# injun-baek/Video-Depth-Normal-v2

Hardware: AMD Instinct MI355X
Metric: depth frames/sec at 518x518, ViT-L (higher is better)
Workload: dtype f16x3; 1 GPU; DepthAnythingV2(vitl) batch=8 518x518 streams/GPU, memory bank full (S=6); replicas per GPU; lanes=2, precision=f16x3, ranks=1, backend=none, attention_pv_products=1

## Files before the change

### include/vdn.h

```cpp
#ifndef VDN_H
#define VDN_H
#include <stddef.h>
#include <stdint.h>

#ifdef __cplusplus
extern "C" {
#endif

typedef void* vdn_stream;

enum vdn_status { VDN_OK = 0, VDN_EINVAL = -1, VDN_EUNSUPPORTED = -2, VDN_EALIGN = -3 };
enum vdn_dtype { VDN_F16 = 0, VDN_BF16 = 1, VDN_F32 = 2, VDN_NONE = 3 };
enum vdn_act { VDN_ACT_NONE = 0, VDN_ACT_GELU = 1, VDN_ACT_RELU = 2,
               VDN_ACT_SILU = 3  };
enum vdn_amode { VDN_A_PLAIN = 0, VDN_A_CONV3X3 = 1,
                 VDN_A_PAD3X3 = 2  };
enum vdn_store {
  VDN_ST_PLAIN = 0,
  VDN_ST_HEADS = 1,
  VDN_ST_CONVT = 2,
  VDN_ST_GEGLU = 3
};

typedef struct vdn_gemm_tuning {
  int force_bm;
  int p8;
  int no_splitk;
  int no_pipe;
  int splitk_p8;
  int cus;
  int splitk_occ;
  int splitk_max;
  int min_tiles;
  float f128, f192;
  int x8;
} vdn_gemm_tuning;
int vdn_gemm_get_tuning(vdn_gemm_tuning* out);

typedef struct vdn_gemm_desc {
  int32_t dt;
  int32_t M, N, K;
  const void* A;
  int32_t a_mode;
  int32_t lda;
  int32_t relu_a;
  int32_t cB, cH, cW, cC, cOH, cOW, cstride;
  const void* W;
  int32_t ldb;
  const float* bias;
  const float* rowadd;
  int32_t act;
  const float* gamma;
  const float* tab;
  int32_t tab_mod, tab_off;
  const void* res1;
  int32_t res1_dt, ldr1;
  const void* res2;
  int32_t res2_dt, ldr2;
  int32_t store;
  void* out;
  int32_t out_dt;
  int32_t ldc;
  int32_t row_group, row_skip;
  void* dst[3];
  int32_t nsplit, heads, tokens, tok_off, tpad;
  int32_t transposed[3];
  int32_t rope[3];
  const float* rope_cs;
  int32_t rope_mod;
  int32_t ck, cout;
  const void* zeros;
  const void* A_lo;
  const void* W_lo;
  void* out_lo;
  void* dst_lo[3];
  const void* res1_lo;
  const void* res2_lo;
  int32_t conv_korder;
  int32_t cu_hint;
  void* splitk_ws;
  int64_t splitk_ws_bytes;
  int32_t ksplit;
  void* dst8[3];
  const void* A8;
  const void* W8;
  void* out8;
  int32_t a_kt, w_kt, out_kt;
  int32_t x8_terms;
  const vdn_gemm_tuning* tuning;
  int32_t subpix;
  const float* subpix_bias;
  void* pad_hi;
} vdn_gemm_desc;

int vdn_gemm(const vdn_gemm_desc* d, vdn_stream stream);

int vdn_layernorm(const void* x, int x_dt, int rows, int C, const float* w, const float* b, float eps,
                  const float* addvec, float alpha, const float* addtab, int tab_div, int tab_mod,
                  int out_group, void* out_h, void* out_h_lo, int h_dt, float* out_f, void* out8, int kt,
                  vdn_stream stream);

int vdn_flash_attn(int dt, const void* Q, const void* K, const void* Vt, void* out, const void* Q_lo,
                   const void* K_lo, const void* Vt_lo, void* out_lo, const void* Q8, const void* K8, void* out8, int out_kt,
                   int B, int H, int nq, int nq_pad, int nk, int nk_pad, float scale, int pv_products, vdn_stream stream);

int vdn_temporal_attn(int dt, const void* qkv, void* out, const void* qkv_lo, void* out_lo, int Bv, int T, int D,
                      int c, int heads, float scale, const float* rope_cs, vdn_stream stream);

int vdn_groupnorm(int dt, const void* x, const void* x_lo, void* y, void* y_lo, int F, int HW, int C, int groups,
                  const float* w, const float* b, float eps, float* partial, int nsplit, vdn_stream stream);

int vdn_upsample_bilinear(int dt, const void* x, const void* x_lo, void* y, void* y_lo, int B, int IH, int IW, int OH,
                          int OW, int C, vdn_stream stream);
int vdn_upsample_bilinear_f32(const float* x, float* y, int B, int IH, int IW, int OH, int OW, int relu,
                              vdn_stream stream);

int vdn_patchify(int dt, const float* img, void* rows, void* rows_lo, int B, int H, int W, int ldk,
                 vdn_stream stream);

int vdn_fill_row(float* x, const float* vec, int B, int rows_per_b, int row, int C, vdn_stream stream);

int vdn_bicubic(const float* src, float* dst, int ih, int iw, int oh, int ow, int C, float scale_rows,
                float scale_cols, vdn_stream stream);

int vdn_preprocess(const uint8_t* frames, int n, int h, int w, int swap_rb, float* out, int H, int W, const float* mean3,
                   const float* std3, vdn_stream stream);

int vdn_add_vec(const float* x, const float* vec, float alpha, float* y, int rows, int C, vdn_stream stream);

int vdn_head_out(int dt, const void* feat, const void* feat_lo, const float* w, float bias, float* depth, int M,
                 int C, int relu, vdn_stream stream);

enum { VDN_OUT_NONE = 0, VDN_OUT_RELU = 1, VDN_OUT_SIGMOID = 2 };

int vdn_head_out_act(int dt, const void* feat, const void* feat_lo, const float* w, float bias, float* depth, int M,
                     int C, int act, float out_scale, vdn_stream stream);

int vdn_mask_down1(const float* depth, float* out, int B, int H, int W, int OH, int OW, const float* w,
                   vdn_stream stream);
int vdn_mask_down2(const float* in, float* out, int B, int H, int W, int OH, int OW, const float* w,
                   vdn_stream stream);

int vdn_dwconv7(const float* x, float* y, int B, int H, int W, int C, const float* w, const float* bias,
                vdn_stream stream);

int vdn_addtab_cast(int dt, const float* x, const float* tab, int tab_div, int tab_mod, void* y, void* y_lo,
                    size_t rows, int C, vdn_stream stream);

int vdn_temporal_attn_last(int dt, const float* pool, size_t slot_stride, const int32_t* slots, int T, int HW, int c,
                           const float* pe_q, const float* pe_k, const float* pe_v, float scale, void* out, void* out_lo,
                           vdn_stream stream);

size_t vdn_stitch_workspace_bytes(void);
int vdn_stitch_fit(const float* pred, const float* target, size_t n, void* workspace, float* coef, vdn_stream stream);
int vdn_stitch_apply(const float* window, const float* coef, float* out_tail, float* out_new, float* ref1, size_t hw,
                     int T, int align_len, int overlap, int ref_frame, vdn_stream stream);

enum vdn_eval_domain { VDN_EVAL_DEPTH = 0, VDN_EVAL_DISP = 1 };
enum vdn_eval_tgm { VDN_EVAL_TGM_ROWS = 0, VDN_EVAL_TGM_FRAMES = 1 };
size_t vdn_eval_workspace_bytes(int frames);
int vdn_eval_fit(const float* pred, const float* gt, const uint8_t* mask, int frames, size_t hw, double dmin, double dmax,
                 int domain, void* workspace, double* coef, vdn_stream stream);
int vdn_eval_metrics(const float* pred, const float* gt, const uint8_t* mask, int frames, int H, int W, double dmin,
                     double dmax, int domain, int tgm, const double* coef, void* workspace, double* out,
                     vdn_stream stream);
int vdn_resize_bilinear_hp(const float* x, float* y, int frames, int IH, int IW, int OH, int OW, vdn_stream stream);

size_t vdn_normal_eval_workspace_bytes(int frames);
int vdn_sobel_ix_iy(const float* depth, float* ix, float* iy, int frames, int H, int W, int normalize_kernel,
                    vdn_stream stream);
int vdn_normal_vector(const float* depth, float* out, int frames, int H, int W, int normalize_kernel, float scale_xy,
                      float scale_z, float eps, vdn_stream stream);
int vdn_erode_mask3(const uint8_t* mask, uint8_t* out, int frames, int H, int W, vdn_stream stream);
int vdn_normal_eval(const float* pred, const float* target, int target_is_depth, const uint8_t* mask, int frames, int H,
                    int W, void* workspace, double* frame_sums, int64_t* frame_counts, double* out, vdn_stream stream);
// ... 128 lines not shown
```

### video-depth-normal-v2_amd/csrc/gemm.hip

```cpp
#include "common.hpp"
#include <stdlib.h>

namespace vdn_gemm_impl {
int launch_f16(const vdn_gemm_desc& d, hipStream_t s);
int launch_bf16(const vdn_gemm_desc& d, hipStream_t s);

static int env_int(const char* name, int dflt) {
  const char* e = getenv(name);
  return e ? atoi(e) : dflt;
}
static float env_float(const char* name, float dflt) {
  const char* e = getenv(name);
  return e ? (float)atof(e) : dflt;
}
static const vdn_gemm_tuning& tuning_defaults() {
  static const vdn_gemm_tuning t = [] {
    vdn_gemm_tuning v;
    v.force_bm = env_int("VDN_GEMM_BM", 0);
    v.p8 = env_int("VDN_GEMM_P8", 1);
    v.no_splitk = getenv("VDN_GEMM_NOSPLITK") != nullptr;
    v.no_pipe = getenv("VDN_GEMM_NOPIPE") != nullptr;
    v.splitk_p8 = env_int("VDN_SPLITK_P8", 0);
    v.cus = env_int("VDN_GEMM_CUS", 0);
    v.splitk_occ = env_int("VDN_SPLITK_OCC", 50);
    v.splitk_max = env_int("VDN_SPLITK_MAX", 8);
    v.min_tiles = env_int("VDN_GEMM_MIN_TILES", 96);
    v.f128 = env_float("VDN_GEMM_F128", 1.3f);
    v.f192 = env_float("VDN_GEMM_F192", 1.2f);
    v.x8 = env_int("VDN_GEMM_X8", 1);
    return v;
  }();
  return t;
}
const vdn_gemm_tuning& tuning(const vdn_gemm_desc& d) { return d.tuning ? *d.tuning : tuning_defaults(); }
}

extern "C" int vdn_gemm_get_tuning(vdn_gemm_tuning* out) {
  if (!out) return VDN_EINVAL;
  vdn_gemm_desc none = {};
  *out = vdn_gemm_impl::tuning(none);
  return VDN_OK;
}

extern "C" int vdn_gemm(const vdn_gemm_desc* dp, vdn_stream stream) {
  if (!dp) return VDN_EINVAL;
  const vdn_gemm_desc& d = *dp;
  if (d.M <= 0 || d.N <= 0 || d.K <= 0 || !d.A || !d.W || !d.zeros) return VDN_EINVAL;
  if (d.tuning) {
    const vdn_gemm_tuning& t = *d.tuning;
    if ((t.force_bm != 0 && t.force_bm != 128 && t.force_bm != 192 && t.force_bm != 256) || t.splitk_occ < 0 || t.splitk_max < 0 ||
        t.min_tiles < 0 || t.cus < 0 || t.cus > 256)
      return VDN_EINVAL;
  }
  if (d.dt != VDN_F16 && d.dt != VDN_BF16) return VDN_EUNSUPPORTED;
  if ((d.K & 7) || (d.ldb & 63) || d.ldb < d.K) return VDN_EALIGN;
  if (((uintptr_t)d.A & 15) || ((uintptr_t)d.W & 15) || ((uintptr_t)d.zeros & 15)) return VDN_EALIGN;
  if (d.subpix) {
    if (d.subpix != 1 || d.a_mode != VDN_A_CONV3X3 || d.store != VDN_ST_CONVT || !d.subpix_bias || d.bias || d.act || d.rowadd ||
        d.gamma || d.tab || d.res1 || d.res2 || d.relu_a || d.K != 4 * d.cC || d.ldb != d.K || d.conv_korder != 1 || d.cstride != 1)
      return VDN_EINVAL;
    if ((d.ck != 2 && d.ck != 4) || d.cout <= 0 || (d.cout & 255) || (d.cC & 63) || !d.A_lo || !d.W_lo || !d.out_lo ||
        d.out_dt != d.dt || d.A8 || d.W8)
      return VDN_EUNSUPPORTED;
    if (((uintptr_t)d.subpix_bias | (uintptr_t)d.out) & 15) return VDN_EALIGN;
  }
  if (d.a_mode == VDN_A_CONV3X3) {
    if ((d.cC & 7) || d.K != (d.subpix ? 4 : 9) * d.cC || d.M != d.cB * d.cOH * d.cOW) return VDN_EINVAL;
    if (d.conv_korder && ((d.cC & 63) || d.conv_korder != 1)) return VDN_EINVAL;
    if (d.cstride != 1 && d.cstride != 2) return VDN_EUNSUPPORTED;
    if (d.cOH != (d.cH + 2 - 3) / d.cstride + 1 || d.cOW != (d.cW + 2 - 3) / d.cstride + 1) return VDN_EINVAL;
  } else if (d.a_mode == VDN_A_PLAIN) {
    if ((d.lda & 7) || d.lda < d.K) return VDN_EALIGN;
  } else if (d.a_mode == VDN_A_PAD3X3) {
    if (d.dt != VDN_F16 || !d.A8 || !d.W8 || !d.a_kt || !d.w_kt || d.relu_a || d.subpix || d.x8_terms) return VDN_EINVAL;
    if (d.cB <= 0 || d.cH <= 0 || d.cW <= 0 || d.cC <= 0 || (d.cC & 63) || d.cC > 4096 || d.K != 9 * d.cC || d.ldb != d.K) return VDN_EINVAL;
    if ((long)d.cB * (d.cH + 2) * (d.cW + 2) != d.M) return VDN_EINVAL;
    if (d.store != VDN_ST_PLAIN || !d.bias || d.rowadd || d.gamma || d.tab || d.row_group > 0 || d.out_dt != VDN_F16 || d.ldc != d.N ||
        (d.N & 63) || !d.out || ((uintptr_t)d.out & 15) || ((uintptr_t)d.bias & 15))
      return VDN_EINVAL;
    if (d.act == VDN_ACT_RELU) {
      if (!d.out_kt || !d.out8 || d.out_lo || d.res1 || d.res2 || d.pad_hi) return VDN_EINVAL;
    } else if (d.act == VDN_ACT_NONE) {
      if (d.out_kt || !d.out_lo || !d.res1 || !d.res1_lo || d.res1_dt != VDN_F16 || (d.ldr1 & 7) || ((uintptr_t)d.res1 | (uintptr_t)d.res1_lo) & 15)
        return VDN_EINVAL;
      if (d.res2 && (!d.res2_lo || d.res2_dt != VDN_F16 || (d.ldr2 & 7) || ((uintptr_t)d.res2 | (uintptr_t)d.res2_lo) & 15)) return VDN_EINVAL;
      if ((d.pad_hi == nullptr) != (d.out8 == nullptr) || ((uintptr_t)d.pad_hi & 15)) return VDN_EINVAL;
    } else {
      return VDN_EINVAL;
    }
  } else {
    return VDN_EUNSUPPORTED;
  }
  if (d.N & 3) return VDN_EALIGN;
  if (d.ksplit != 0 || d.splitk_ws_bytes < 0 || (d.splitk_ws == nullptr) != (d.splitk_ws_bytes == 0)) return VDN_EINVAL;
  if ((uintptr_t)d.splitk_ws & 15) return VDN_EALIGN;
  if (((uintptr_t)d.A_lo | (uintptr_t)d.W_lo | (uintptr_t)d.out_lo) & 15) return VDN_EALIGN;
  if (d.out_lo && (d.out_dt == VDN_F32 || !d.out)) return VDN_EINVAL;
  if ((d.res1 && (d.ldr1 & 3)) || (d.res2 && (d.ldr2 & 3))) return VDN_EALIGN;
  if (((uintptr_t)d.A8 | (uintptr_t)d.W8 | (uintptr_t)d.out8) & 15) return VDN_EALIGN;
  if ((d.A8 || d.W8) && (d.dt != VDN_F16 || (d.a_mode != VDN_A_PLAIN && d.a_mode != VDN_A_PAD3X3) || (d.K & 63) || (d.lda != d.K && !d.a_kt))) return VDN_EINVAL;
  if (d.out8 && (d.dt != VDN_F16 || d.store != VDN_ST_PLAIN || d.out_dt != VDN_F16 || (d.act != VDN_ACT_GELU && d.a_mode != VDN_A_PAD3X3) || d.N != d.ldc || (d.N & 63) || !d.A8 || !d.W8))
    return VDN_EINVAL;
  if ((d.a_kt || d.w_kt || d.out_kt || d.x8_terms) && (!d.A8 || !d.W8)) return VDN_EINVAL;
  if (d.A8 && d.W8 && ((!d.a_kt && (long)d.M * d.lda >= (1L << 31)) || (!d.w_kt && (long)d.N * d.ldb >= (1L << 31)) || d.M >= (1 << 25) || d.N >= (1 << 25)))
    return VDN_EUNSUPPORTED;
  if (d.x8_terms < 0 || d.x8_terms > 2) return VDN_EINVAL;
  if (d.out_kt && (d.store != VDN_ST_PLAIN || d.out_dt != VDN_F16 || d.ldc != d.N || (d.N & 63) || d.res1 || d.res2 || d.tab ||
                   d.rowadd || d.gamma || d.row_group > 0 || (d.act == VDN_ACT_RELU && d.a_mode != VDN_A_PAD3X3))) return VDN_EINVAL;
  if (d.pad_hi && d.a_mode != VDN_A_PAD3X3) return VDN_EINVAL;
  if (((uintptr_t)d.bias | (uintptr_t)d.gamma | (uintptr_t)d.tab | (uintptr_t)d.res1 | (uintptr_t)d.res2) & 7) return VDN_EALIGN;
  switch (d.store) {
    case VDN_ST_PLAIN:
      if (!d.out || d.ldc < d.N) return VDN_EINVAL;
      if ((d.ldc & 3) || ((uintptr_t)d.out & 15)) return VDN_EALIGN;
      break;
    case VDN_ST_GEGLU:
      if (!d.out || (d.N & 31) || d.ldc < d.N / 2 || (d.act && d.act != VDN_ACT_SILU) || d.gamma || d.res1 || d.res2 || d.tab || d.rowadd)
        return VDN_EINVAL;
      if ((d.ldc & 3) || ((uintptr_t)d.out & 15)) return VDN_EALIGN;
      break;
    case VDN_ST_CONVT:
      if (!d.out || d.ck <= 0 || d.cout <= 0 || d.N != d.ck * d.ck * d.cout || d.M != d.cB * d.cH * d.cW || d.res1 ||
          d.res2 || d.tab)
        return VDN_EINVAL;
      if ((d.cout & 3) || ((uintptr_t)d.out & 15)) return VDN_EALIGN;
      break;
    case VDN_ST_HEADS:
      if (d.nsplit < 1 || d.nsplit > 3 || d.heads <= 0 || d.N != d.nsplit * d.heads * 64 || d.tokens <= 0 ||
          d.M % d.tokens || d.tok_off < 0 || d.tok_off + d.tokens > d.tpad || d.act || d.gamma || d.res1 || d.res2 ||
          d.tab || d.rowadd)
        return VDN_EINVAL;
      for (int i = 0; i < d.nsplit; ++i) {
        if (!d.dst[i] || ((uintptr_t)d.dst[i] & 15)) return VDN_EINVAL;
        if (d.rope[i] && (!d.rope_cs || d.rope_mod <= 0)) return VDN_EINVAL;
        if (d.dst8[i] && (d.transposed[i] || (!d.W_lo && !d.W8) || d.dt != VDN_F16 || ((uintptr_t)d.dst8[i] & 15))) return VDN_EINVAL;
      }
      break;
    default:
      return VDN_EUNSUPPORTED;
  }
  hipStream_t s = (hipStream_t)stream;
  return d.dt == VDN_F16 ? vdn_gemm_impl::launch_f16(d, s) : vdn_gemm_impl::launch_bf16(d, s);
}
```

### video-depth-normal-v2_amd/csrc/gemm_kernels.hpp

```cpp
#pragma once
#include "planes.hpp"
#include <stdlib.h>
#include <type_traits>

namespace vdn_gemm_impl {

const vdn_gemm_tuning& tuning(const vdn_gemm_desc& d);

constexpr int BK = 64;


__device__ __forceinline__ void glds16(const void* src, void* dst) {
  __builtin_amdgcn_global_load_lds((const __attribute__((address_space(1))) void*)src, (__attribute__((address_space(3))) void*)dst,
                                   16, 0, 0);
}

__device__ __forceinline__ void tile_mn(int tile, int tiles_m, int tiles_n, int& tm_i, int& tn_i) {
  constexpr int GM = 4;
  const int per_group = GM * tiles_n;
  const int g = tile / per_group, r = tile - g * per_group;
  const int gm = (tiles_m - g * GM) < GM ? (tiles_m - g * GM) : GM;
  tn_i = r / gm;
  tm_i = g * GM + (r - tn_i * gm);
}
// ... 2 lines not shown
__device__ __forceinline__ int frag_off128(int row, int c) { return row * 128 + ((c ^ ((row >> 1) & 7)) << 4); }

template <typename H>
__device__ __forceinline__ f32x4 mma3(typename H::V8 bh, typename H::V8 bl, typename H::V8 ah, typename H::V8 al, f32x4 c) {
  c = H::mfma16(bh, al, c);
  c = H::mfma16(bl, ah, c);
  return H::mfma16(bh, ah, c);
}

struct KStep {
  int k0;
  int tap;
  int off;
};
template <int BKS, bool SUBPIX = false>
__device__ __forceinline__ KStep kstep_decode(int kt, const vdn_gemm_desc& p, unsigned sp_taps = 0, int sp_lg = 0) {
  static_assert(BKS == 32 || BKS == 64, "one or two steps per 64-channel block");
  KStep s = {kt * BKS, 9, 0};
  if (p.conv_korder) {
    const int t2 = BKS == 32 ? kt >> 1 : kt, half = BKS == 32 ? kt & 1 : 0;
    int c64;
    if constexpr (SUBPIX) {
      c64 = t2 >> sp_lg;
      s.tap = (sp_taps >> (4 * (t2 & ((1 << sp_lg) - 1)))) & 15;
    } else {
      c64 = t2 / 9;
      s.tap = t2 - c64 * 9;
    }
    if (c64 * 64 >= p.cC) s.tap = 9;
    const int ky = (s.tap * 11) >> 5, kx = s.tap - ky * 3;
    s.off = ((ky - 1) * p.cW + (kx - 1)) * p.cC + c64 * 64 + half * 32;
  }
  return s;
}

template <typename T, bool CONV>
struct APiece {
  const T* base;
  int iy0, ix0;
  const T* center;
  unsigned ok9;
  __device__ __forceinline__ void setup(int m, int chunk_elems, const vdn_gemm_desc& p) {
    m = m < p.M ? m : p.M - 1;
    if constexpr (CONV) {
      const int hw = p.cOH * p.cOW;
      const int b = m / hw, rem = m - b * hw;
      const int oy = rem / p.cOW, ox = rem - oy * p.cOW;
      base = (const T*)p.A + (size_t)b * p.cH * p.cW * p.cC;
      iy0 = oy * p.cstride - 1;
      ix0 = ox * p.cstride - 1;
      center = base + ((ptrdiff_t)(iy0 + 1) * p.cW + (ix0 + 1)) * p.cC + chunk_elems;
      ok9 = 0;
#pragma unroll
      for (int t = 0; t < 9; ++t) {
        const int iy = iy0 + t / 3, ix = ix0 + t % 3;
        ok9 |= (unsigned)((iy >= 0) & (iy < p.cH) & (ix >= 0) & (ix < p.cW)) << t;
      }
    } else {
      base = (const T*)p.A + (size_t)m * p.lda;
    }
  }
  __device__ __forceinline__ const char* src(const KStep& ks, int chunk_elems, const vdn_gemm_desc& p, bool& ok) const {
    const int k = ks.k0 + chunk_elems;
    if constexpr (!CONV) {
      ok = k < p.K;
      return (const char*)(base + k);
    } else if (p.conv_korder) {
      ok = (ok9 >> ks.tap) & 1;
      return (const char*)(center + ks.off);
    } else {
      const int tap = (int)(((float)(k >> 3) + 0.5f) * (1.0f / (float)(p.cC >> 3)));
      const int ci = k - tap * p.cC;
      const int ky = tap / 3, kx = tap - ky * 3;
      const int iy = iy0 + ky, ix = ix0 + kx;
      ok = (tap < 9) & (iy >= 0) & (iy < p.cH) & (ix >= 0) & (ix < p.cW);
      return (const char*)(base + ((size_t)iy * p.cW + ix) * p.cC + ci);
    }
  }
};


constexpr int VDN_STX_FC1 = 100, VDN_STX_RES = 101, VDN_STX_HEADS = 102, VDN_STX_HALF = 103, VDN_STX_RESHALF1 = 104,
              VDN_STX_RESHALF2 = 105, VDN_STX_SPLITK = 106, VDN_STX_SUBPIX = 107,
              VDN_STX_RCU1 = 108, VDN_STX_RCU2 = 109;

__device__ __forceinline__ void subpix_taps(int phase, int ck, unsigned& taps, int& lg) {
  const int a = phase / ck, b = phase - a * ck;
  const int y0 = a == 0 ? 0 : 1, ny = (a == 0 || a == ck - 1) ? 2 : 1;
  const int x0 = b == 0 ? 0 : 1, nx = (b == 0 || b == ck - 1) ? 2 : 1;
  taps = 0;
  int s = 0;
  for (int yy = 0; yy < ny; ++yy)
    for (int xx = 0; xx < nx; ++xx) taps |= (unsigned)(3 * (y0 + yy) + x0 + xx) << (4 * s++);
  lg = (ny >> 1) + (nx >> 1);
}
__device__ __forceinline__ int subpix_tile(int tn_i, const vdn_gemm_desc& p, unsigned& taps, int& lg) {
  const int tpp = p.cout >> 8;
  const int rank = tn_i / tpp, sub = tn_i - rank * tpp;
  const int phase = p.ck == 4 ? (int)((0xa965edb87421fc30ULL >> (4 * rank)) & 15) : rank;
  subpix_taps(phase, p.ck, taps, lg);
  return phase * p.cout + sub * 256;
}

__host__ __device__ inline int epi_flavour(const vdn_gemm_desc& d) {
  if (d.subpix) return VDN_STX_SUBPIX;
  const bool half_out = d.out_dt != VDN_F32;
  const bool plain_rows = d.store == VDN_ST_PLAIN && !d.rowadd && !d.gamma && !d.tab && d.row_group <= 0;
  if (plain_rows && half_out && d.out_lo && d.act != VDN_ACT_GELU) {
    if (!d.res1 && !d.res2) return VDN_STX_HALF;
    if (d.act == VDN_ACT_NONE && d.res1 && d.res1_lo && d.res1_dt == d.out_dt) {
      if (!d.res2) return VDN_STX_RESHALF1;
      if (d.res2_lo && d.res2_dt == d.out_dt) return VDN_STX_RESHALF2;
    }
  }
  if (d.store == VDN_ST_PLAIN && d.bias && d.act == VDN_ACT_GELU && !d.rowadd && !d.gamma && !d.tab && !d.res1 && !d.res2 &&
      half_out && (d.out_lo || (d.out8 && d.A8 && d.W8)) && d.row_group <= 0)
    return VDN_STX_FC1;
  if (d.store == VDN_ST_PLAIN && d.act == VDN_ACT_NONE && !d.rowadd && !d.tab && d.res1 && d.res1_dt == VDN_F32 && !d.res1_lo &&
      !d.res2 && d.out_dt == VDN_F32 && d.row_group <= 0)
    return VDN_STX_RES;
  if (d.store == VDN_ST_HEADS && !d.rope[0] && !d.rope[1] && !d.rope[2] && d.nsplit >= 1) {
    for (int i = 0; i < d.nsplit; ++i)
      if (!d.dst[i] || (!d.dst_lo[i] && !d.transposed[i] && !d.dst8[i])) return d.store;
    return VDN_STX_HEADS;
  }
  return d.store;
}

template <int DT, int STORE>
__device__ __forceinline__ void emit4(const vdn_gemm_desc& p, int m, int n, f32x4 a, f32x4 b, f32x4 bias_a, f32x4 bias_b,
                                      f32x4 gam) {
  static_assert(STORE == VDN_ST_PLAIN || STORE == VDN_ST_CONVT || STORE == VDN_ST_GEGLU || STORE == VDN_ST_HEADS ||
                STORE == VDN_STX_SPLITK || STORE == VDN_STX_HALF || STORE == VDN_STX_RESHALF1 || STORE == VDN_STX_RESHALF2 ||
                STORE == VDN_STX_RES, "emit4 serves these flavours");
  using H = Half<DT>;
  using T = typename H::T;
  using V4 = typename H::V4;
  if (m >= p.M || n >= p.N) return;
  if constexpr (STORE == VDN_STX_SPLITK) {
    *(f32x4*)((float*)p.out + (size_t)m * p.ldc + n) = a;
    return;
  } else if constexpr (STORE == VDN_STX_HALF || STORE == VDN_STX_RESHALF1 || STORE == VDN_STX_RESHALF2) {
    a += bias_a;
    if constexpr (STORE == VDN_STX_HALF) {
      const float floor_v = p.act == VDN_ACT_RELU ? 0.f : -INFINITY;
#pragma unroll
      for (int e = 0; e < 4; ++e) a[e] = (a[e] < floor_v) ? floor_v : a[e];
    } else {
      const size_t r1 = (size_t)m * p.ldr1 + n;
      const V4 rh = *(const V4*)((const T*)p.res1 + r1), rl = *(const V4*)((const T*)p.res1_lo + r1);
#pragma unroll
      for (int e = 0; e < 4; ++e) a[e] += (float)rh[e] + (float)rl[e];
      if constexpr (STORE == VDN_STX_RESHALF2) {
        const size_t r2 = (size_t)m * p.ldr2 + n;
        const V4 qh = *(const V4*)((const T*)p.res2 + r2), ql = *(const V4*)((const T*)p.res2_lo + r2);
#pragma unroll
        for (int e = 0; e < 4; ++e) a[e] += (float)qh[e] + (float)ql[e];
      }
    }
    V4 h, l;
    split_planes(a, h, l);
    store_out_planes<false, T>(p, (size_t)m * p.ldc + n, h, l);
    return;
  } else if constexpr (STORE == VDN_STX_RES) {
    a = (a + bias_a) * gam + *(const f32x4*)((const float*)p.res1 + (size_t)m * p.ldr1 + n);
    *(f32x4*)((float*)p.out + (size_t)m * p.ldc + n) = a;
    return;
  }
  if constexpr (STORE == VDN_ST_PLAIN || STORE == VDN_ST_CONVT) {
    a += bias_a;
    if (p.rowadd) a += p.rowadd[m];
    if (p.act == VDN_ACT_GELU) {
      a = gelu4(a);
    } else if (p.act == VDN_ACT_RELU) {
#pragma unroll
      for (int e = 0; e < 4; ++e) a[e] = (a[e] < 0.f) ? 0.f : a[e];
    }
    a *= gam;
    if (p.tab) a += *(const f32x4*)(p.tab + (size_t)(m % p.tab_mod + p.tab_off) * p.N + n);
    if (p.res1) {
      a += load4_as_float(p.res1, p.res1_dt, (size_t)m * p.ldr1 + n);
      if (p.res1_lo) a += load4_as_float(p.res1_lo, p.res1_dt, (size_t)m * p.ldr1 + n);
    }
    if (p.res2) {
      a += load4_as_float(p.res2, p.res2_dt, (size_t)m * p.ldr2 + n);
      if (p.res2_lo) a += load4_as_float(p.res2_lo, p.res2_dt, (size_t)m * p.ldr2 + n);
    }
    size_t o;
    if constexpr (STORE == VDN_ST_CONVT) {
      const int hw = p.cH * p.cW;
      const int cb = m / hw, rem = m - cb * hw;
      const int cy = rem / p.cW, cx = rem - cy * p.cW;
      const int kk = n / p.cout, co = n - kk * p.cout;
      const int ky = kk / p.ck, kx = kk - ky * p.ck;
      o = ((((size_t)cb * (p.cH * p.ck) + cy * p.ck + ky) * (p.cW * p.ck)) + cx * p.ck + kx) * p.cout + co;
    } else {
      o = (size_t)(p.row_group > 0 ? m + (m / p.row_group + 1) * p.row_skip : m) * p.ldc + n;
    }
    store_out4<DT>(p, o, a);
  } else if constexpr (STORE == VDN_ST_GEGLU) {
    if ((n & 16) || n + 16 >= p.N) return;
    a += bias_a;
    b += bias_b;
    if (p.act == VDN_ACT_SILU) {
#pragma unroll
      for (int e = 0; e < 4; ++e) a[e] *= b[e] * __builtin_amdgcn_rcpf(1.0f + __builtin_amdgcn_exp2f(-1.44269504088896341f * b[e]));
    } else {
      a = a * gelu4(b);
// ... 176 lines not shown
      return;
    }
#pragma unroll
    for (int i = 0; i < TM; ++i)
#pragma unroll
      for (int j = 0; j < TN; ++j)
        emit4<DT, STORE>(p, mw + i * 16 + fr, nw + j * 16 + fq * 4, acc[i][j], acc[i][j + 1 < TN ? j + 1 : j], bias4[j],
                         bias4[j + 1 < TN ? j + 1 : j], gam4[j]);
  }
}

template <int DT, int TM>
__device__ __forceinline__ void epilogue_subpix(f32x4 (&acc)[TM][4], const vdn_gemm_desc& p, int mw, int nw, int lane) {
  using H = Half<DT>;
  using T = typename H::T;
  using V8 = typename H::V8;
  const int fr = lane & 15, fq = lane >> 4;
  const int phase = nw / p.cout, co0 = nw - phase * p.cout;
  const int ky = phase / p.ck, kx = phase - ky * p.ck;
  unsigned taps;
  int lg;
  subpix_taps(phase, p.ck, taps, lg);
  const int hw = p.cH * p.cW;
  int cy[TM], cx[TM];
  size_t ob[TM];
#pragma unroll
  for (int i = 0; i < TM; ++i) {
    int m = mw + i * 16 + fr;
    m = m < p.M ? m : p.M - 1;
    const int cb = m / hw, rem = m - cb * hw;
    cy[i] = rem / p.cW;
    cx[i] = rem - cy[i] * p.cW;
    ob[i] = ((((size_t)cb * (p.cH * p.ck) + cy[i] * p.ck + ky) * (p.cW * p.ck)) + cx[i] * p.ck + kx) * p.cout + co0 + fq * 8;
  }
  for (int s = 0; s < (1 << lg); ++s) {
    const int tap = (taps >> (4 * s)) & 15;
    const int sy = ((tap * 11) >> 5) - 1, sx = tap - (sy + 1) * 3 - 1;
    const float* bs = p.subpix_bias + (size_t)(phase * 4 + s) * p.cout + co0 + fq * 8;
    f32x4 b4[4];
#pragma unroll
    for (int j = 0; j < 4; ++j) b4[j] = *(const f32x4*)(bs + (j >> 1) * 32 + (j & 1) * 4);
#pragma unroll
    for (int i = 0; i < TM; ++i) {
      const int y = cy[i] + sy, x = cx[i] + sx;
      const float in = ((y >= 0) & (y < p.cH) & (x >= 0) & (x < p.cW)) ? 1.f : 0.f;
#pragma unroll
      for (int j = 0; j < 4; ++j) acc[i][j] += b4[j] * in;
    }
  }
#pragma unroll
  for (int i = 0; i < TM; ++i) {
    if (mw + i * 16 + fr >= p.M) continue;
#pragma unroll
    for (int u = 0; u < 2; ++u) {
      V8 h, l;
      split_planes(acc[i][2 * u], acc[i][2 * u + 1], h, l);
      store_out_planes<false, T>(p, ob[i] + u * 32, h, l);
    }
  }
}

template <int DT, int TM, int STORE>
__device__ __forceinline__ void epilogue_x3(f32x4 (&acc)[TM][4], const vdn_gemm_desc& p, int slice, int mw, int nw, int lane) {
  if constexpr (STORE == VDN_STX_SPLITK) {
    vdn_gemm_desc q = p;
    q.out = (float*)p.splitk_ws + (size_t)slice * p.M * p.N;
    q.ldc = p.N;
    epilogue_regs<DT, TM, 4, STORE, false>(acc, q, mw, nw, lane);
  } else if constexpr (STORE == VDN_STX_SUBPIX) {
    epilogue_subpix<DT, TM>(acc, p, mw, nw, lane);
  } else {
    epilogue_regs<DT, TM, 4, STORE, vdn_pair8<STORE>>(acc, p, mw, nw, lane);
  }
}

template <int DT, int TM, int TN>
__device__ __forceinline__ void epilogue_dispatch(f32x4 (&acc)[TM][TN], const vdn_gemm_desc& p, int mw, int nw, int lane) {
  switch (epi_flavour(p)) {
    case VDN_STX_HALF: epilogue_regs<DT, TM, TN, VDN_STX_HALF>(acc, p, mw, nw, lane); break;
    case VDN_STX_RESHALF1: epilogue_regs<DT, TM, TN, VDN_STX_RESHALF1>(acc, p, mw, nw, lane); break;
    case VDN_STX_RESHALF2: epilogue_regs<DT, TM, TN, VDN_STX_RESHALF2>(acc, p, mw, nw, lane); break;
    case VDN_STX_RES: epilogue_regs<DT, TM, TN, VDN_STX_RES>(acc, p, mw, nw, lane); break;
    case VDN_STX_FC1:
    case VDN_ST_PLAIN: epilogue_regs<DT, TM, TN, VDN_ST_PLAIN>(acc, p, mw, nw, lane); break;
    case VDN_ST_CONVT: epilogue_regs<DT, TM, TN, VDN_ST_CONVT>(acc, p, mw, nw, lane); break;
    case VDN_ST_GEGLU: epilogue_regs<DT, TM, TN, VDN_ST_GEGLU>(acc, p, mw, nw, lane); break;
    default: epilogue_regs<DT, TM, TN, VDN_ST_HEADS>(acc, p, mw, nw, lane); break;
  }
}

template <int DT, int BM, int BN, int WM, int WN, int AMODE >
__global__ __launch_bounds__(256) void gemm_kernel(const vdn_gemm_desc p) {
  using H = Half<DT>;
  using V8 = typename H::V8;
  using T = typename H::T;
  constexpr int A_BYTES = BM * BK * 2, B_BYTES = BN * BK * 2, STAGE = A_BYTES + B_BYTES;
  constexpr int WTM = BM / WM, WTN = BN / WN, TM = WTM / 16, TN = WTN / 16;
  constexpr int A_IT = BM / 32, B_IT = BN / 32;
  constexpr bool CONV = (AMODE == 1 || AMODE == 2);
  constexpr bool RELU_A = (AMODE == 2 || AMODE == 3);
  extern __shared__ __attribute__((aligned(16))) char smem[];

  const int tid = threadIdx.x, lane = tid & 63;
  const int wave = __builtin_amdgcn_readfirstlane(tid >> 6);
  const int tiles_n = (p.N + BN - 1) / BN;
  const int tiles_m = (p.M + BM - 1) / BM;
  const int tile = xcd_remap(blockIdx.x, tiles_m * tiles_n);
  const int m0 = (tile / tiles_n) * BM, n0 = (tile % tiles_n) * BN;

  const int lr = lane >> 3;
  const int chunk = (lane & 7) ^ ((((wave & 1) << 2) + (lr >> 1)) & 7);
  APiece<T, CONV> a_pc[A_IT];
#pragma unroll
  for (int i = 0; i < A_IT; ++i) a_pc[i].setup(m0 + (i * 4 + wave) * 8 + lr, chunk * 8, p);
  const T* b_row[B_IT];
#pragma unroll
  for (int i = 0; i < B_IT; ++i) {
    int n = n0 + (i * 4 + wave) * 8 + lr;
    n = n < p.N ? n : p.N - 1;
    b_row[i] = (const T*)p.W + (size_t)n * p.ldb;
  }
  const char* zeros = (const char*)p.zeros;

  const int nk1 = p.ldb / BK;
  const int seg_wlo = p.W_lo ? 1 : -1;
  const int nseg = 1 + (p.W_lo ? 1 : 0) + (p.A_lo ? 1 : 0);
  const int seg_alo = p.A_lo ? nseg - 1 : -1;
  const ptrdiff_t a_delta = p.A_lo ? (const char*)p.A_lo - (const char*)p.A : 0;
  const ptrdiff_t w_delta = p.W_lo ? (const char*)p.W_lo - (const char*)p.W : 0;

  auto stage = [&](int buf, int kt_all) {
    char* sA = smem + buf * STAGE;
    char* sB = sA + A_BYTES;
    const int seg = kt_all / nk1;
    const int kt = kt_all - seg * nk1;
    const ptrdiff_t ad = (seg == seg_alo) ? a_delta : 0;
    const ptrdiff_t wd = (seg == seg_wlo) ? w_delta : 0;
    const KStep ks = kstep_decode<BK>(kt, p);
    const int k = ks.k0 + chunk * 8;
#pragma unroll
    for (int i = 0; i < A_IT; ++i) {
      bool ok;
      const char* src = a_pc[i].src(ks, chunk * 8, p, ok);
      glds16(ok ? src + ad : zeros, sA + (i * 4 + wave) * 1024);
    }
#pragma unroll
    for (int i = 0; i < B_IT; ++i) glds16((const char*)(b_row[i] + k) + wd, sB + (i * 4 + wave) * 1024);
  };

  const int wm = wave / WN, wn = wave % WN;
  const int fr = lane & 15, fq = lane >> 4;
  int a_off[TM][2], b_off[TN][2];
#pragma unroll
  for (int t = 0; t < TM; ++t) {
    const int row = wm * WTM + t * 16 + fr;
#pragma unroll
    for (int kk = 0; kk < 2; ++kk) a_off[t][kk] = frag_off128(row, kk * 4 + fq);
  }
#pragma unroll
  for (int t = 0; t < TN; ++t) {
    const int row = wn * WTN + t * 16 + fr;
#pragma unroll
    for (int kk = 0; kk < 2; ++kk) b_off[t][kk] = frag_off128(row, kk * 4 + fq);
  }

  f32x4 acc[TM][TN];
// ... 487 lines not shown
  if (wm == 1) __builtin_amdgcn_s_barrier();

  for (int kt = 0; kt + 1 < nk; ++kt) {
    const char* sc = smem + (kt & 1) * STAGE;
    const int nb = (kt + 1) & 1;
    VDN_PHASE((read_a(sc, 0), read_b(sc, 0)), issue(U0, nb, kt + 1), 4, 2, 0, 0);
    VDN_PHASE(read_b(sc, 1), issue(U1, nb, kt + 1), 4, 3, 0, 1);
    VDN_PHASE(read_a(sc, 1), issue(U2, nb, kt + 1), 4, 4, 1, 1);
    VDN_PHASE(read_b(sc, 0), issue(U3, nb, kt + 1), 4, 3, 1, 0);
  }
  {
    const char* sc = smem + ((nk - 1) & 1) * STAGE;
    VDN_PHASE((read_a(sc, 0), read_b(sc, 0)), (void)0, 2, 1, 0, 0);
    VDN_PHASE(read_b(sc, 1), (void)0, 0, 0, 0, 1);
    VDN_PHASE(read_a(sc, 1), (void)0, 0, 0, 1, 1);
    VDN_PHASE(read_b(sc, 0), (void)0, 0, 0, 1, 0);
  }
#undef VDN_PHASE
  if (wm == 0) __builtin_amdgcn_s_barrier();

  epilogue_x3<DT, 2 * TQ, STORE>(acc, p, slice, m0 + wm * (BM / 2), n0 + wn * 64, lane);
  }
}

template <typename F>
void with_amode(const vdn_gemm_desc& d, F&& f) {
  if (d.a_mode == VDN_A_CONV3X3) { if (d.relu_a) f(IC<2>{}); else f(IC<1>{}); }
  else { if (d.relu_a) f(IC<3>{}); else f(IC<0>{}); }
}
template <typename F>
void with_flavour(const vdn_gemm_desc& d, int fl, F&& f) {
  if (d.a_mode == VDN_A_CONV3X3) {
    auto conv = [&](auto st) { if (d.relu_a) f(IC<2>{}, st); else f(IC<1>{}, st); };
    switch (fl) {
      case VDN_STX_HALF: conv(IC<VDN_STX_HALF>{}); break;
      case VDN_STX_RESHALF1: conv(IC<VDN_STX_RESHALF1>{}); break;
      case VDN_STX_RESHALF2: conv(IC<VDN_STX_RESHALF2>{}); break;
      case VDN_STX_SUBPIX: f(IC<1>{}, IC<VDN_STX_SUBPIX>{}); break;
      default: conv(IC<VDN_ST_PLAIN>{}); break;
    }
  } else {
    switch (fl) {
      case VDN_ST_PLAIN: f(IC<0>{}, IC<VDN_ST_PLAIN>{}); break;
      case VDN_STX_HALF: f(IC<0>{}, IC<VDN_STX_HALF>{}); break;
      case VDN_ST_CONVT: f(IC<0>{}, IC<VDN_ST_CONVT>{}); break;
      case VDN_ST_GEGLU: f(IC<0>{}, IC<VDN_ST_GEGLU>{}); break;
      case VDN_STX_FC1: f(IC<0>{}, IC<VDN_STX_FC1>{}); break;
      case VDN_STX_RES: f(IC<0>{}, IC<VDN_STX_RES>{}); break;
      case VDN_STX_HEADS: f(IC<0>{}, IC<VDN_STX_HEADS>{}); break;
      default: f(IC<0>{}, IC<VDN_ST_HEADS>{}); break;
    }
  }
}

template <int DT, int BM, int BN, int WM, int WN>
int launch_tile(const vdn_gemm_desc& d, hipStream_t s) {
  const int tiles = ((d.M + BM - 1) / BM) * ((d.N + BN - 1) / BN);
  const size_t lds = 2 * (size_t)(BM + BN) * BK * 2;
  with_amode(d, [&](auto am) {
    hipLaunchKernelGGL((gemm_kernel<DT, BM, BN, WM, WN, decltype(am)::value>), dim3(tiles), dim3(256), lds, s, d);
  });
  VDN_CHECK_LAUNCH();
  return VDN_OK;
}

template <int DT>
int launch_x3(const vdn_gemm_desc& d, hipStream_t s) {
  const int tiles = ((d.M + 127) / 128) * ((d.N + 127) / 128);
  const size_t lds = 65536;
  with_amode(d, [&](auto am) { hipLaunchKernelGGL((gemm_x3_kernel<DT, decltype(am)::value>), dim3(tiles), dim3(256), lds, s, d); });
  VDN_CHECK_LAUNCH();
  return VDN_OK;
}

template <int DT, int BM>
int launch_x3_big(const vdn_gemm_desc& d, hipStream_t s) {
  const int tiles = ((d.M + BM - 1) / BM) * ((d.N + 255) / 256);
  const size_t lds = 2 * (size_t)(2 * BM * 64 + 2 * 256 * 64);
  const dim3 g(tiles), b(512);
  int fl = epi_flavour(d);
  const bool a8 = !(d.N & 7) && !(d.ldc & 7) && !((uintptr_t)d.out & 15) && !((uintptr_t)d.out_lo & 15) && !(d.ldr1 & 7) &&
                  !(d.ldr2 & 7) && !(((uintptr_t)d.res1 | (uintptr_t)d.res1_lo | (uintptr_t)d.res2 | (uintptr_t)d.res2_lo) & 15);
  if (!a8 && fl != VDN_STX_RES && fl != VDN_STX_HEADS && fl != VDN_STX_SUBPIX) fl = d.store;
  if (d.a_mode == VDN_A_CONV3X3) {
    if (fl != VDN_STX_HALF && fl != VDN_STX_RESHALF1 && fl != VDN_STX_RESHALF2 && fl != VDN_STX_SUBPIX) fl = VDN_ST_PLAIN;
  } else if (fl == VDN_STX_RESHALF1 || fl == VDN_STX_RESHALF2) {
    fl = d.store;
  }
  bool p8 = false;
  if constexpr (BM == 256 || BM == 192) {
    p8 = tuning(d).p8 >= (BM == 256 ? 1 : 2);
    if (p8) with_flavour(d, fl, [&](auto am, auto st) {
      hipLaunchKernelGGL((gemm_x3_p8_kernel<DT, decltype(am)::value, decltype(st)::value, BM>), g, b, lds, s, d);
    });
  }
  if (!p8) with_flavour(d, fl, [&](auto am, auto st) {
    constexpr int AM = decltype(am)::value, ST = decltype(st)::value;
    constexpr bool CAN_PIPE = BM <= 192 && (AM == 0 || BM == 128);
    if (CAN_PIPE && !tuning(d).no_pipe) hipLaunchKernelGGL((gemm_x3_big_kernel<DT, AM, BM, ST, CAN_PIPE>), g, b, lds, s, d);
    else hipLaunchKernelGGL((gemm_x3_big_kernel<DT, AM, BM, ST, false>), g, b, lds, s, d);
  });
  VDN_CHECK_LAUNCH();
  return VDN_OK;
}

template <int DT> int big_entry(const vdn_gemm_desc& d, int bm, hipStream_t s);
int x8_entry(const vdn_gemm_desc& d, hipStream_t s);

template <int DT, int FL>
__global__ __launch_bounds__(256) void splitk_reduce_kernel(const vdn_gemm_desc p) {
  const int n4 = p.N >> 2;
  const size_t total = (size_t)p.M * n4, mn = (size_t)p.M * p.N;
  const float* ws = (const float*)p.splitk_ws;
  const f32x4 one = {1.f, 1.f, 1.f, 1.f};
  for (size_t i = (size_t)blockIdx.x * 256 + threadIdx.x; i < total; i += (size_t)gridDim.x * 256) {
    const int m = (int)(i / n4), n = (int)(i - (size_t)m * n4) * 4;
    f32x4 a = *(const f32x4*)(ws + (size_t)m * p.N + n);
    for (int sl = 1; sl < p.ksplit; ++sl) a += *(const f32x4*)(ws + sl * mn + (size_t)m * p.N + n);
    const f32x4 b4 = p.bias ? *(const f32x4*)(p.bias + n) : f32x4{0.f, 0.f, 0.f, 0.f};
    const f32x4 g4 = p.gamma ? *(const f32x4*)(p.gamma + n) : one;
    emit4<DT, FL>(p, m, n, a, a, b4, b4, g4);
  }
}

template <int DT>
int launch_splitk(const vdn_gemm_desc& d0, int ksplit, int fl, hipStream_t s) {
  vdn_gemm_desc d = d0;
  const bool p8 = ksplit < 0;
  d.ksplit = p8 ? -ksplit : ksplit;
  const int tiles = p8 ? ((d.M + 255) / 256) * ((d.N + 255) / 256) : ((d.M + 127) / 128) * ((d.N + 255) / 256);
  const size_t lds = p8 ? 2 * (size_t)(2 * 256 * 64 + 2 * 256 * 64) : 2 * (size_t)(2 * 128 * 64 + 2 * 256 * 64);
  if (p8) hipLaunchKernelGGL((gemm_x3_p8_kernel<DT, 0, VDN_STX_SPLITK, 256>), dim3(tiles * d.ksplit), dim3(512), lds, s, d);
  else if (d.a_mode != VDN_A_CONV3X3) hipLaunchKernelGGL((gemm_x3_big_kernel<DT, 0, 128, VDN_STX_SPLITK, true>), dim3(tiles * ksplit), dim3(512), lds, s, d);
  else if (d.relu_a) hipLaunchKernelGGL((gemm_x3_big_kernel<DT, 2, 128, VDN_STX_SPLITK, true>), dim3(tiles * ksplit), dim3(512), lds, s, d);
  else hipLaunchKernelGGL((gemm_x3_big_kernel<DT, 1, 128, VDN_STX_SPLITK, true>), dim3(tiles * ksplit), dim3(512), lds, s, d);
  const size_t work = (size_t)d.M * (d.N >> 2);
  const dim3 g((unsigned)((work + 255) / 256 < 4096 ? (work + 255) / 256 : 4096));
  switch (fl) {
    case VDN_STX_HALF: hipLaunchKernelGGL((splitk_reduce_kernel<DT, VDN_STX_HALF>), g, dim3(256), 0, s, d); break;
    case VDN_STX_RESHALF1: hipLaunchKernelGGL((splitk_reduce_kernel<DT, VDN_STX_RESHALF1>), g, dim3(256), 0, s, d); break;
    case VDN_STX_RES: hipLaunchKernelGGL((splitk_reduce_kernel<DT, VDN_STX_RES>), g, dim3(256), 0, s, d); break;
    default: hipLaunchKernelGGL((splitk_reduce_kernel<DT, VDN_STX_RESHALF2>), g, dim3(256), 0, s, d); break;
  }
  VDN_CHECK_LAUNCH();
  return VDN_OK;
}
template <int DT> int splitk_entry(const vdn_gemm_desc& d, int ksplit, int fl, hipStream_t s);

inline int pick_bm(int M, int N, int cu_hint, const vdn_gemm_tuning& tu) {
  const int tn = (N + 255) / 256;
  const int cus = tu.cus > 0 ? tu.cus : (cu_hint > 0 && cu_hint <= 256 ? cu_hint : 256);
  int best = 0;
  double best_cost = 1e30;
  for (int bm : {256, 192, 128}) {
    const long tiles = (long)((M + bm - 1) / bm) * tn;
    const long rounds = (tiles + cus - 1) / cus;
    const double cost = (double)rounds * bm * (bm == 128 ? tu.f128 : (bm == 192 ? tu.f192 : 1.0));
    if (cost < best_cost) { best_cost = cost; best = bm; }
  }
  return best;
}

template <int DT>
int launch_dt(const vdn_gemm_desc& d, hipStream_t s) {
  if constexpr (DT == VDN_F16) {
    if (d.A8 && d.W8) {
      if ((d.a_mode == VDN_A_PLAIN || d.a_mode == VDN_A_PAD3X3) && !d.relu_a && !(d.K & 63) && d.N >= 192 &&
          (long)d.M * d.N >= 1024L * 1024 && tuning(d).x8 != 0)
        return x8_entry(d, s);
      if (d.a_mode == VDN_A_PAD3X3) return VDN_EUNSUPPORTED;
      if (d.a_kt || d.w_kt || d.out_kt || d.out8 || !d.A_lo || !d.W_lo) return VDN_EUNSUPPORTED;
    }
  }
  if (d.subpix) {
    const vdn_gemm_tuning& tu = tuning(d);
    return big_entry<DT>(d, tu.force_bm ? tu.force_bm : pick_bm(d.M, d.N, d.cu_hint, tu), s);
  }
  const bool deep = d.splitk_ws && (d.a_mode == VDN_A_CONV3X3 ? d.ldb : d.K) >= 2048 && (long)d.M * d.N >= 32L * 1024;
  if (d.A_lo && d.W_lo && d.N >= 192 && ((long)d.M * d.N >= 256L * 1024 || deep) &&
      (d.a_mode == VDN_A_CONV3X3 ? d.store == VDN_ST_PLAIN : ((d.K & 31) == 0 && !d.relu_a))) {
    const vdn_gemm_tuning& tu = tuning(d);
    const int force = tu.force_bm;
    if (d.splitk_ws && !force && !(d.N & 3) && !tu.no_splitk) {
      const bool conv = d.a_mode == VDN_A_CONV3X3;
      const int fl = epi_flavour(d);
      const int cus = d.cu_hint > 0 && d.cu_hint <= 256 ? d.cu_hint : 256;
      const long tiles128 = (long)((d.M + 127) / 128) * ((d.N + 255) / 256);
      const int nk_total = conv ? d.ldb / 32 : d.K / 32;
      const bool fl_ok = fl == VDN_STX_HALF || (conv ? (fl == VDN_STX_RESHALF1 || fl == VDN_STX_RESHALF2) : fl == VDN_STX_RES);
      const long occ = tu.splitk_occ, ks_max = tu.splitk_max;
      if (fl_ok && tiles128 * 100 <= cus * occ && nk_total >= (conv ? 64 : 32)) {
        long ks = (cus + tiles128 - 1) / tiles128;
        ks = ks < ks_max ? ks : ks_max;
        ks = ks < nk_total / 16 ? ks : nk_total / 16;
        const long fit = d.splitk_ws_bytes / ((long)d.M * d.N * 4);
        ks = ks < fit ? ks : fit;
        while (ks >= 2 && (ks - 1) * ((nk_total + ks - 1) / ks) >= nk_total) --ks;
        if (ks >= 2) return splitk_entry<DT>(d, (int)ks, fl, s);
      }
    }
    {
      const int ks = tu.splitk_p8;
      if (ks >= 2 && d.splitk_ws && !force && d.a_mode == VDN_A_PLAIN && epi_flavour(d) == VDN_STX_RES && d.K >= 2048 &&
          (long)d.M * d.N * 4 * ks <= d.splitk_ws_bytes)
        return splitk_entry<DT>(d, -ks, VDN_STX_RES, s);
    }
    const int bm = force ? force : pick_bm(d.M, d.N, d.cu_hint, tu);
    const long min_tiles = tu.min_tiles;
    const long tiles128 = (long)((d.M + 127) / 128) * ((d.N + 255) / 256);
    const bool small = !force && ((min_tiles > 0 && tiles128 < min_tiles && d.a_mode != VDN_A_CONV3X3) ||
                                 (long)d.M * d.N < 256L * 1024);
    if (!small && (bm == 256 || bm == 192 || bm == 128)) return big_entry<DT>(d, bm, s);
  }
  if (d.A_lo && d.W_lo && (d.store == VDN_ST_HEADS || d.N > 64)) return launch_x3<DT>(d, s);
  if (d.store == VDN_ST_HEADS || d.N > 64) return launch_tile<DT, 128, 128, 2, 2>(d, s);
  if (d.N > 32) return launch_tile<DT, 128, 64, 2, 2>(d, s);
  return launch_tile<DT, 128, 32, 4, 1>(d, s);
}


}
```

### video-depth-normal-v2_amd/csrc/gemm_x8.hip

```cpp
#include "gemm_kernels.hpp"

namespace vdn_gemm_impl {

typedef int i32x8 __attribute__((ext_vector_type(8)));

constexpr int X8_BN = 256;
constexpr int X8_WH = 256 * 64;
#ifndef VDN_X8_NSLOT
#define VDN_X8_NSLOT 5
#endif
#ifndef VDN_X8_ABL
#define VDN_X8_ABL 0
#endif
constexpr int X8_NSLOT = VDN_X8_NSLOT;
constexpr int x8_unit(int bm) { return bm * 64 + X8_WH; }
constexpr int X8_L = X8_NSLOT - 1;
constexpr int x8_pc(int ph, bool four) {
  const int a = four ? 2 : 1, w = 2;
  return a + w;
}
constexpr int x8_inflight(int newest, int k, bool four) {
  int n = 0;
  for (int t = 0; t < k; ++t) n += x8_pc((newest - t) & 3, four);
  return n;
// ... 163 lines not shown
  auto next = [](int s) { return s + 1 == X8_NSLOT ? 0 : s + 1; };

  {
    int s = 0;
    auto pro = [&](int n, auto phc) {
      if (n < X8_L && n < nunits) { issue(n >> 2, phc, s); s = next(s); }
    };
    pro(0, P0); pro(1, P1); pro(2, P2); pro(3, P3);
    if constexpr (X8_L > 4) pro(4, P0);
  }
  if (nunits >= X8_L) X8_WAIT((X8_L - 1) & 3, X8_L - 1);
  else asm volatile("s_waitcnt vmcnt(0)" ::: "memory");
  __builtin_amdgcn_s_barrier();
  if (wm == 1) __builtin_amdgcn_s_barrier();

#define X8_PHASE(PC, PH)                                                                    \
  do {                                                                                      \
    reads(PC, rd_slot);                                                                     \
    X8_ISSUE(PH);                                                                           \
    X8_WAIT(((PH) + X8_L) & 3, X8_L - 1);                                                   \
    asm volatile("s_waitcnt lgkmcnt(0)" ::: "memory");                                      \
    __builtin_amdgcn_s_barrier();                                                           \
    __builtin_amdgcn_sched_barrier(0);                                                      \
    mfmas(PC);                                                                              \
    __builtin_amdgcn_sched_barrier(0);                                                      \
    __builtin_amdgcn_s_barrier();                                                           \
    rd_slot = next(rd_slot);                                                                \
    wr_slot = next(wr_slot);                                                                \
  } while (0)
#define X8_ISSUE(PH) issue(s + ((PH) + X8_L) / 4, std::integral_constant<int, ((PH) + X8_L) & 3>{}, wr_slot)
  int s = 0;
  for (; 4 * s + 3 + X8_L <= nunits - 1; ++s) {
    X8_PHASE(P0, 0);
    X8_PHASE(P1, 1);
    X8_PHASE(P2, 2);
    X8_PHASE(P3, 3);
  }
  static_assert(X8_L == 4, "the tail below is written for a lead of one slab");
#define X8_TAIL(PC, LEFT)                                                                   \
  do {                                                                                      \
    reads(PC, rd_slot);                                                                     \
    if constexpr ((LEFT) > 0) X8_WAIT(3, (LEFT));                                           \
    else asm volatile("s_waitcnt vmcnt(0)" ::: "memory");                                   \
    asm volatile("s_waitcnt lgkmcnt(0)" ::: "memory");                                      \
    __builtin_amdgcn_s_barrier();                                                           \
    __builtin_amdgcn_sched_barrier(0);                                                      \
    mfmas(PC);                                                                              \
    __builtin_amdgcn_sched_barrier(0);                                                      \
    __builtin_amdgcn_s_barrier();                                                           \
    rd_slot = next(rd_slot);                                                                \
  } while (0)
  for (; s < nslab; ++s) {
    X8_TAIL(P0, 2);
    X8_TAIL(P1, 1);
    X8_TAIL(P2, 0);
    X8_TAIL(P3, 0);
  }
#undef X8_TAIL
#undef X8_ISSUE
#undef X8_PHASE
  if (wm == 0) __builtin_amdgcn_s_barrier();
  __builtin_amdgcn_sched_barrier(0);
#if VDN_X8_ABL & 8
  if (p.splitk_ws && tid == 0 && (blockIdx.x % 37) == 0) {
    unsigned long long* dbg = (unsigned long long*)p.splitk_ws + (blockIdx.x / 37) * 2;
    dbg[0] = __builtin_amdgcn_s_memtime() - st_c0;
    dbg[1] = __builtin_amdgcn_s_memrealtime() - st_r0;
  }
#endif

  const int mw = m0 + wm * (X8_BM / 2), nw = n0 + wn * 64;
  const f32x4 z4 = {0.f, 0.f, 0.f, 0.f}, o4 = {1.f, 1.f, 1.f, 1.f};
  if constexpr (PAIR) {
    f32x4 bias8[2][2][2];
#pragma unroll
    for (int j = 0; j < 2; ++j)
#pragma unroll
      for (int u = 0; u < 2; ++u)
#pragma unroll
        for (int q = 0; q < 2; ++q) {
          const int n = nw + 32 * j + 16 * u + 8 * h + 4 * q;
          bias8[j][u][q] = (p.bias && n < p.N) ? *(const f32x4*)(p.bias + n) : z4;
        }
    if constexpr (STORE == VDN_STX_RCU1 || STORE == VDN_STX_RCU2) {
#pragma unroll
      for (int i = 0; i < NI; ++i)
#pragma unroll
        for (int j = 0; j < 2; ++j)
#pragma unroll
          for (int e = 0; e < 16; ++e) acc[i][j][e] += bias8[j][e >> 3][(e >> 2) & 1][e & 3];
      const int pw = p.cW + 2, fr = (p.cH + 2) * pw;
      auto decode = [&](int m, size_t& mu) {
        const int b = m / fr, rem = m - b * fr, y = rem / pw, x = rem - y * pw;
        mu = (size_t)(b * p.cH + y - 1) * p.cW + (x - 1);
        return m < p.M && y >= 1 && y <= p.cH && x >= 1 && x <= p.cW;
      };
      auto store_pad = [&](_Float16* hip, int m, bool img, const f16x32& hv, const f16x32& lv) {
#pragma unroll
        for (int q = 0; q < 4; ++q) {
          V8 o;
#pragma unroll
          for (int e = 0; e < 8; ++e) o[e] = hv[8 * q + e];
          *(V8*)(hip + kt_half_offset(1, m, nw + 32 * (q >> 1) + 16 * (q & 1) + 8 * h, p.M, p.ldc)) = o;
        }
        const int sb = x6_scale_byte(hv);
        uint8_t* d8 = (uint8_t*)p.out8 + kt_byte_offset(1, m, nw, h, p.M, p.ldc);
        x6_store_half(d8, hv, sb, img);
        x6_store_half(d8 + (size_t)p.M * p.ldc, lv, sb - 10, img);
      };
      if constexpr (STORE == VDN_STX_RCU1) {
#pragma unroll
        for (int i = 0; i < NI; ++i) {
          const int m = mw + 32 * i + r;
          size_t mu;
          const bool img = decode(m, mu);
          f16x32 hv, lv;
#pragma unroll
          for (int j = 0; j < 2; ++j)
#pragma unroll
            for (int u = 0; u < 2; ++u) {
              float v[8];
#pragma unroll
              for (int e = 0; e < 8; ++e) {
                const float a = acc[i][j][8 * u + e];
                v[e] = img ? (a < 0.f ? 0.f : a) : 0.f;
              }
              V8 hh, ll;
              split_planes(v, hh, ll);
#pragma unroll
              for (int e = 0; e < 8; ++e) { hv[16 * j + 8 * u + e] = hh[e]; lv[16 * j + 8 * u + e] = ll[e]; }
            }
          if (m < p.M && nw < p.N) store_pad((_Float16*)p.out, m, img, hv, lv);
        }
      } else {
        using T = _Float16;
        V8 rh[2][2][2] = {}, rl[2][2][2] = {};
        const bool two = p.res2 != nullptr;
        unsigned keep[NI];
        auto load = [&](int i, int rr) {
          size_t mu;
          const bool img = decode(mw + 32 * i + r, mu);
          if (rr == 0) keep[i] = img ? ~0u : 0u;
          if ((rr == 1 && !two) || nw >= p.N) return;
          const T* rp = (const T*)(rr ? p.res2 : p.res1);
          const T* rq = (const T*)(rr ? p.res2_lo : p.res1_lo);
          const size_t o = (img ? mu : 0) * (size_t)(rr ? p.ldr2 : p.ldr1) + nw + 8 * h;
#pragma unroll
          for (int j = 0; j < 2; ++j)
#pragma unroll
            for (int u = 0; u < 2; ++u) {
              rh[rr][j][u] = *(const V8*)(rp + o + 32 * j + 16 * u);
              rl[rr][j][u] = *(const V8*)(rq + o + 32 * j + 16 * u);
            }
        };
        auto add = [&](int i, int rr) {
          if (rr == 1 && !two) return;
          typedef unsigned u32x4v __attribute__((ext_vector_type(4)));
#pragma unroll
          for (int j = 0; j < 2; ++j)
#pragma unroll
            for (int u = 0; u < 2; ++u) {
              const V8 a = __builtin_bit_cast(V8, __builtin_bit_cast(u32x4v, rh[rr][j][u]) & keep[i]);
              const V8 b = __builtin_bit_cast(V8, __builtin_bit_cast(u32x4v, rl[rr][j][u]) & keep[i]);
#pragma unroll
              for (int e = 0; e < 8; ++e) acc[i][j][8 * u + e] += (float)a[e] + (float)b[e];
            }
        };
        load(0, 0);
        load(0, 1);
        __builtin_amdgcn_sched_barrier(0);
#pragma unroll
        for (int i = 0; i < NI; ++i) {
          add(i, 0);
          __builtin_amdgcn_sched_barrier(0);
          if (i + 1 < NI) load(i + 1, 0);
          __builtin_amdgcn_sched_barrier(0);
          add(i, 1);
          __builtin_amdgcn_sched_barrier(0);
          if (i + 1 < NI) load(i + 1, 1);
          __builtin_amdgcn_sched_barrier(0);
        }
#pragma unroll
        for (int i = 0; i < NI; ++i) {
          const int m = mw + 32 * i + r;
          size_t mu;
          const bool img = decode(m, mu);
          f16x32 hv, lv;
#pragma unroll
          for (int j = 0; j < 2; ++j)
#pragma unroll
            for (int u = 0; u < 2; ++u) {
              float v[8];
#pragma unroll
              for (int e = 0; e < 8; ++e) v[e] = img ? acc[i][j][8 * u + e] : 0.f;
              V8 hh, ll;
              split_planes(v, hh, ll);
              const int n = nw + 32 * j + 16 * u + 8 * h;
              if (img && n < p.N) store_out_planes<false, T>(p, mu * p.ldc + n, hh, ll);
              hh = relu8(hh); ll = relu8(ll);
#pragma unroll
              for (int e = 0; e < 8; ++e) { hv[16 * j + 8 * u + e] = hh[e]; lv[16 * j + 8 * u + e] = ll[e]; }
            }
          if (p.out8 && m < p.M && nw < p.N) store_pad((_Float16*)p.pad_hi, m, img, hv, lv);
        }
      }
    } else if (STORE == VDN_STX_FC1 && p.out8) {
#pragma unroll
      for (int i = 0; i < NI; ++i) {
        const int m = mw + 32 * i + r;
        f16x32 hv, lv;
#pragma unroll
        for (int j = 0; j < 2; ++j)
#pragma unroll
          for (int u = 0; u < 2; ++u) {
            const f32x4 g0 = gelu4(f32x4{acc[i][j][8 * u], acc[i][j][8 * u + 1], acc[i][j][8 * u + 2], acc[i][j][8 * u + 3]} + bias8[j][u][0]);
            const f32x4 g1 = gelu4(f32x4{acc[i][j][8 * u + 4], acc[i][j][8 * u + 5], acc[i][j][8 * u + 6], acc[i][j][8 * u + 7]} + bias8[j][u][1]);
            V8 hh, ll;
            split_planes(g0, g1, hh, ll);
#pragma unroll
            for (int e = 0; e < 8; ++e) { hv[16 * j + 8 * u + e] = hh[e]; lv[16 * j + 8 * u + e] = ll[e]; }
            const int n = nw + 32 * j + 16 * u + 8 * h;
            if (m < p.M && n < p.N)
              store_planes((_Float16*)p.out, (_Float16*)p.out_lo, kt_half_offset(p.out_kt, m, n, p.M, p.ldc), hh, ll);
          }
        if (m < p.M && nw < p.N) {
          const int sb = x6_scale_byte(hv);
          uint8_t* d8 = (uint8_t*)p.out8 + kt_byte_offset(p.out_kt, m, nw, h, p.M, p.ldc);
          x6_store_half(d8, hv, sb);
          x6_store_half(d8 + (size_t)p.M * p.ldc, lv, sb - 10);
        }
      }
    } else if ((STORE == VDN_STX_HEADS || STORE == VDN_ST_HEADS) && nw < p.N && !p.transposed[nw / (p.heads * 64)] && p.dst8[nw / (p.heads * 64)]) {
      const int hc = p.heads * 64, split = nw / hc, head = (nw - split * hc) >> 6;
      _Float16* dst = (_Float16*)p.dst[split];
      _Float16* dlo = (_Float16*)p.dst_lo[split];
      if (STORE == VDN_ST_HEADS && p.rope[split]) {
        f32x4 cs[2][2][4];
        auto fetch = [&](int i, f32x4 (&d)[2][4]) {
          const int m = mw + 32 * i + r, mc = m < p.M ? m : p.M - 1;
          const int tl = mc - (mc / p.tokens) * p.tokens;
          const float* t = p.rope_cs + (size_t)(tl % p.rope_mod) * 64 + 16 * h;
#pragma unroll
          for (int j = 0; j < 2; ++j)
#pragma unroll
            for (int q = 0; q < 4; ++q) d[j][q] = *(const f32x4*)(t + 32 * j + 4 * q);
        };
        fetch(0, cs[0]);
#pragma unroll
        for (int i = 0; i < NI; ++i) {
          if (i + 1 < NI) fetch(i + 1, cs[(i + 1) & 1]);
          const int m = mw + 32 * i + r, mc = m < p.M ? m : p.M - 1;
          const int bt = mc / p.tokens, tk = mc - bt * p.tokens + p.tok_off;
          const size_t row = ((size_t)bt * p.heads + head) * p.tpad + tk;
#pragma unroll
          for (int j = 0; j < 2; ++j) {
            float o[16];
#pragma unroll
            for (int e = 0; e < 8; ++e) {
              const float re = acc[i][j][e] + bias8[j][0][e >> 2][e & 3], im = acc[i][j][8 + e] + bias8[j][1][e >> 2][e & 3];
              const float cc = cs[i & 1][j][e >> 1][2 * (e & 1)], ss = cs[i & 1][j][e >> 1][2 * (e & 1) + 1];
              o[2 * e] = re * cc - im * ss;
              o[2 * e + 1] = re * ss + im * cc;
            }
            V8 hh[2], ll[2];
#pragma unroll
            for (int e = 0; e < 16; e += 2) {
              _Float16 h0, h1, l0, l1;
              split2_rtz(o[e], o[e + 1], h0, h1, l0, l1);
              hh[e >> 3][e & 7] = h0; hh[e >> 3][(e & 7) + 1] = h1; ll[e >> 3][e & 7] = l0; ll[e >> 3][(e & 7) + 1] = l1;
            }
            if (m < p.M) {
              const size_t oo = row * 64 + 32 * j + 16 * h;
              *(V8*)(dst + oo) = hh[0];
              *(V8*)(dst + oo + 8) = hh[1];
              if (dlo) { *(V8*)(dlo + oo) = ll[0]; *(V8*)(dlo + oo + 8) = ll[1]; }
              const float k = VDN_LO8_SCALE;
              uint8_t* d8 = (uint8_t*)p.dst8[split] + row * 128 + 32 * j + 16 * h;
              *(u32x4*)d8 = u32x4{pk4_bf8(o[0], o[1], o[2], o[3]), pk4_bf8(o[4], o[5], o[6], o[7]), pk4_bf8(o[8], o[9], o[10], o[11]),
                                  pk4_bf8(o[12], o[13], o[14], o[15])};
              *(u32x4*)(d8 + 64) = u32x4{pk4_bf8(k * (float)ll[0][0], k * (float)ll[0][1], k * (float)ll[0][2], k * (float)ll[0][3]),
                                         pk4_bf8(k * (float)ll[0][4], k * (float)ll[0][5], k * (float)ll[0][6], k * (float)ll[0][7]),
                                         pk4_bf8(k * (float)ll[1][0], k * (float)ll[1][1], k * (float)ll[1][2], k * (float)ll[1][3]),
                                         pk4_bf8(k * (float)ll[1][4], k * (float)ll[1][5], k * (float)ll[1][6], k * (float)ll[1][7])};
            }
          }
        }
// ... 1 lines not shown
#pragma unroll
      for (int i = 0; i < NI; ++i) {
        const int m = mw + 32 * i + r, mc = m < p.M ? m : p.M - 1;
        const int bt = mc / p.tokens, tk = mc - bt * p.tokens + p.tok_off;
        const size_t row = ((size_t)bt * p.heads + head) * p.tpad + tk;
        unsigned hi8[2][2][2], lo8[2][2][2];
#pragma unroll
        for (int j = 0; j < 2; ++j)
#pragma unroll
          for (int u = 0; u < 2; ++u) {
            float v[8];
#pragma unroll
            for (int e = 0; e < 4; ++e) { v[e] = acc[i][j][8 * u + e] + bias8[j][u][0][e]; v[4 + e] = acc[i][j][8 * u + 4 + e] + bias8[j][u][1][e]; }
            V8 hh, ll;
            split_planes(v, hh, ll);
            if (m < p.M) store_planes(dst, dlo, row * 64 + 32 * j + 16 * u + 8 * h, hh, ll);
            pack_bf8<8>(v, hi8[j][u]);
            pack_bf8_lo<8>(ll, lo8[j][u]);
          }
        u32x4 bh[2], bl[2];
#pragma unroll
        for (int u = 0; u < 2; ++u)
#pragma unroll
          for (int w = 0; w < 2; ++w) {
            const auto sh = __builtin_amdgcn_permlane32_swap(hi8[0][u][w], hi8[1][u][w], false, false);
            const auto sl = __builtin_amdgcn_permlane32_swap(lo8[0][u][w], lo8[1][u][w], false, false);
            bh[u][w] = sh[0]; bh[u][2 + w] = sh[1];
            bl[u][w] = sl[0]; bl[u][2 + w] = sl[1];
          }
        if (m < p.M) {
          uint8_t* d8 = (uint8_t*)p.dst8[split] + row * 128 + 32 * h;
          *(u32x4*)d8 = bh[0];
          *(u32x4*)(d8 + 16) = bh[1];
          *(u32x4*)(d8 + 64) = bl[0];
          *(u32x4*)(d8 + 80) = bl[1];
        }
      }
    } else {
#pragma unroll
      for (int i = 0; i < NI; ++i)
#pragma unroll
        for (int j = 0; j < 2; ++j)
#pragma unroll
          for (int u = 0; u < 2; ++u) {
            const f32x4 a0 = {acc[i][j][8 * u], acc[i][j][8 * u + 1], acc[i][j][8 * u + 2], acc[i][j][8 * u + 3]};
            const f32x4 a1 = {acc[i][j][8 * u + 4], acc[i][j][8 * u + 5], acc[i][j][8 * u + 6], acc[i][j][8 * u + 7]};
            emit8<VDN_F16, STORE == VDN_ST_HEADS ? VDN_STX_HEADS : STORE>(p, mw + 32 * i + r, nw + 32 * j + 16 * u + 8 * h, a0, a1, bias8[j][u][0],
                                                                              bias8[j][u][1]);
          }
    }
  } else if constexpr (STORE == VDN_STX_RES) {
    f32x4 bias4[2][4], gam4[2][4];
#pragma unroll
    for (int j = 0; j < 2; ++j)
#pragma unroll
      for (int g = 0; g < 4; ++g) {
        const int n = nw + 32 * j + 8 * g + 4 * h;
        bias4[j][g] = (p.bias && n < p.N) ? *(const f32x4*)(p.bias + n) : z4;
        gam4[j][g] = (p.gamma && n < p.N) ? *(const f32x4*)(p.gamma + n) : o4;
      }
    f32x4 res[2][2][4];
    auto fetch = [&](int i, f32x4 (&dst)[2][4]) {
      const int m = mw + 32 * i + r;
#pragma unroll
      for (int j = 0; j < 2; ++j)
#pragma unroll
        for (int g = 0; g < 4; ++g) {
          const int n = nw + 32 * j + 8 * g + 4 * h;
          dst[j][g] = (m < p.M && n < p.N) ? *(const f32x4*)((const float*)p.res1 + (size_t)m * p.ldr1 + n) : z4;
        }
    };
    fetch(0, res[0]);
#pragma unroll
    for (int i = 0; i < NI; ++i) {
      if (i + 1 < NI) fetch(i + 1, res[(i + 1) & 1]);
      const int m = mw + 32 * i + r;
#pragma unroll
      for (int j = 0; j < 2; ++j)
#pragma unroll
        for (int g = 0; g < 4; ++g) {
          const int n = nw + 32 * j + 8 * g + 4 * h;
          const f32x4 a = {acc[i][j][4 * g], acc[i][j][4 * g + 1], acc[i][j][4 * g + 2], acc[i][j][4 * g + 3]};
          if (m < p.M && n < p.N) *(f32x4*)((float*)p.out + (size_t)m * p.ldc + n) = (a + bias4[j][g]) * gam4[j][g] + res[i & 1][j][g];
        }
    }
  } else {
    f32x4 bias4[2][4], gam4[2][4];
#pragma unroll
    for (int j = 0; j < 2; ++j)
#pragma unroll
      for (int g = 0; g < 4; ++g) {
        const int n = nw + 32 * j + 8 * g + 4 * h;
        bias4[j][g] = (p.bias && n < p.N) ? *(const f32x4*)(p.bias + n) : z4;
        gam4[j][g] = (p.gamma && n < p.N) ? *(const f32x4*)(p.gamma + n) : o4;
      }
#pragma unroll
    for (int j = 0; j < 2; ++j)
#pragma unroll
      for (int g = 0; g < 4; ++g) {
        const int n = nw + 32 * j + 8 * g + 4 * h;
        const int gb = (g + 2) & 3;
#pragma unroll
        for (int i = 0; i < NI; ++i) {
          const f32x4 a = {acc[i][j][4 * g], acc[i][j][4 * g + 1], acc[i][j][4 * g + 2], acc[i][j][4 * g + 3]};
          const f32x4 b = {acc[i][j][4 * gb], acc[i][j][4 * gb + 1], acc[i][j][4 * gb + 2], acc[i][j][4 * gb + 3]};
          emit4<VDN_F16, STORE>(p, mw + 32 * i + r, n, a, b, bias4[j][g], bias4[j][gb], gam4[j][g]);
        }
      }
  }
}
#undef X8_WAIT

template <int BM>
static int x8_launch(const vdn_gemm_desc& d, hipStream_t s) {
  const int tiles = ((d.M + BM - 1) / BM) * ((d.N + X8_BN - 1) / X8_BN);
  const dim3 g(tiles), b(512);
  constexpr int LDS = X8_NSLOT * x8_unit(BM);
#define VDN_X8(ST, PAIR)                                                                                               \
  do {                                                                                                                   \
    static const hipError_t attr = hipFuncSetAttribute((const void*)gemm_x8_kernel<ST, PAIR, BM>,                        \
                                                       hipFuncAttributeMaxDynamicSharedMemorySize, LDS);       \
    if (attr != hipSuccess) return -(1000 + (int)attr);                                                                  \
    hipLaunchKernelGGL((gemm_x8_kernel<ST, PAIR, BM>), g, b, LDS, s, d);                                                 \
  } while (0)
  if (d.a_mode == VDN_A_PAD3X3) {
#define VDN_X8T(ST)                                                                                                      \
  do {                                                                                                                   \
    static const hipError_t attr = hipFuncSetAttribute((const void*)gemm_x8_kernel<ST, true, BM, true>,                  \
                                                       hipFuncAttributeMaxDynamicSharedMemorySize, LDS);       \
    if (attr != hipSuccess) return -(1000 + (int)attr);                                                                  \
    hipLaunchKernelGGL((gemm_x8_kernel<ST, true, BM, true>), g, b, LDS, s, d);                                           \
  } while (0)
    if (d.act == VDN_ACT_RELU) VDN_X8T(VDN_STX_RCU1);
    else VDN_X8T(VDN_STX_RCU2);
#undef VDN_X8T
    VDN_CHECK_LAUNCH();
    return VDN_OK;
  }
  int fl = epi_flavour(d);
  const bool a8 = !(d.N & 7) && !(d.ldc & 7) && !((uintptr_t)d.out & 15) && !((uintptr_t)d.out_lo & 15) && !((uintptr_t)d.out8 & 7);
  if (d.out8 && !(a8 && fl == VDN_STX_FC1 && !(d.N & 63))) return VDN_EUNSUPPORTED;
  if (!a8 && fl != VDN_STX_RES && fl != VDN_STX_HEADS) fl = d.store;
  if (fl == VDN_STX_RESHALF1 || fl == VDN_STX_RESHALF2) fl = d.store;
  switch (fl) {
    case VDN_STX_FC1: VDN_X8(VDN_STX_FC1, true); break;
    case VDN_STX_HALF: VDN_X8(VDN_STX_HALF, true); break;
    case VDN_STX_HEADS: VDN_X8(VDN_STX_HEADS, true); break;
    case VDN_STX_RES: VDN_X8(VDN_STX_RES, false); break;
    case VDN_ST_GEGLU: VDN_X8(VDN_ST_GEGLU, false); break;
    case VDN_ST_HEADS: {
      bool pair = a8 && d.nsplit >= 1 && d.rope_cs && !((uintptr_t)d.rope_cs & 15);
      for (int i = 0; i < d.nsplit && pair; ++i)
        pair = d.dst[i] && (d.transposed[i] ? !d.rope[i] : d.dst8[i] != nullptr);
      if (pair) VDN_X8(VDN_ST_HEADS, true);
      else VDN_X8(VDN_ST_HEADS, false);
      break;
    }
    default: VDN_X8(VDN_ST_PLAIN, false); break;
  }
#undef VDN_X8
  VDN_CHECK_LAUNCH();
  return VDN_OK;
}

int x8_entry(const vdn_gemm_desc& d, hipStream_t s) {
  const vdn_gemm_tuning& tu = tuning(d);
  const int cus = tu.cus > 0 ? tu.cus : (d.cu_hint > 0 && d.cu_hint <= 256 ? d.cu_hint : 256);
  const long tn = (d.N + X8_BN - 1) / X8_BN;
  auto cost = [&](int bm, double f) { const long t = (long)((d.M + bm - 1) / bm) * tn; return (double)((t + cus - 1) / cus) * bm * f; };
  int bm = tu.force_bm == 192 || tu.force_bm == 256 ? tu.force_bm : (cost(192, 1.08) < cost(256, 1.0) ? 192 : 256);
  return bm == 192 ? x8_launch<192>(d, s) : x8_launch<256>(d, s);
}

}
```

### video-depth-normal-v2_amd/csrc/norm.hip

```cpp
#include "planes.hpp"
#include "reduce.hpp"

namespace {

template <typename XT> struct Vec4;
template <> struct Vec4<float> { using V = f32x4; };
template <> struct Vec4<_Float16> { using V = f16x4; };
template <> struct Vec4<__bf16> { using V = bf16x4; };

template <typename XT, int DT, int NV, bool X6>
__global__ __launch_bounds__(256) void layernorm_kernel(const XT* __restrict__ x, int rows, int C,
                                                        const float* __restrict__ w, const float* __restrict__ b,
                                                        float eps, const float* __restrict__ addvec, float alpha,
                                                        const float* __restrict__ addtab, int tab_div, int tab_mod,
                                                        int out_group, typename Half<DT>::T* __restrict__ out_h,
                                                        typename Half<DT>::T* __restrict__ out_l,
                                                        float* __restrict__ out_f, uint8_t* __restrict__ out8, int kt) {
  using T = typename Half<DT>::T;
  using XV = typename Vec4<XT>::V;
  const int lane = threadIdx.x & 63;
  const int nwaves = gridDim.x * 4;
  extern __shared__ __attribute__((aligned(16))) _Float16 stage_all[];
  _Float16* const stage = stage_all + (X6 ? (threadIdx.x >> 6) * 2 * NV * 256 : 0);
  int row = blockIdx.x * 4 + (threadIdx.x >> 6);
  f32x4 wv[NV], bv[NV];
#pragma unroll
  for (int i = 0; i < NV; ++i) {
    const int c = i * 256 + lane * 4;
    if (c < C) {
      wv[i] = *(const f32x4*)(w + c);
      bv[i] = *(const f32x4*)(b + c);
      if (addvec) bv[i] += alpha * *(const f32x4*)(addvec + c);
    }
  }
  auto load = [&](int r, XV (&dst)[NV]) {
    const XT* xr = x + (size_t)r * C;
#pragma unroll
    for (int i = 0; i < NV; ++i) {
      const int c = i * 256 + lane * 4;
      if (c < C) dst[i] = *(const XV*)(xr + c);
    }
  };
  XV cur[NV], nxt[NV];
  if (row < rows) load(row, cur);
  for (; row < rows; row += nwaves) {
    const int nrow = row + nwaves;
    if (nrow < rows) load(nrow, nxt);
    if (!(out_group > 0 && row % out_group == 0)) {
      const size_t orow = out_group > 0 ? (size_t)(row - row / out_group - 1) : (size_t)row;
      f32x4 v[NV];
      float sum = 0.f;
#pragma unroll
      for (int i = 0; i < NV; ++i) {
        if (i * 256 + lane * 4 < C) {
#pragma unroll
          for (int e = 0; e < 4; ++e) v[i][e] = (float)cur[i][e];
          sum += (v[i][0] + v[i][1]) + (v[i][2] + v[i][3]);
        }
      }
      const float mean = wave_sum(sum) / (float)C;
      float sq = 0.f;
#pragma unroll
      for (int i = 0; i < NV; ++i) {
        if (i * 256 + lane * 4 < C) {
          v[i] -= mean;
          sq += (v[i][0] * v[i][0] + v[i][1] * v[i][1]) + (v[i][2] * v[i][2] + v[i][3] * v[i][3]);
        }
      }
      const float rstd = rsqrtf(wave_sum(sq) / (float)C + eps);
      const float* tab = addtab ? addtab + (size_t)((row / tab_div) % tab_mod) * C : nullptr;
#pragma unroll
      for (int i = 0; i < NV; ++i) {
        const int c = i * 256 + lane * 4;
        if (c < C) {
          f32x4 y = v[i] * rstd * wv[i] + bv[i];
          if (tab) y += *(const f32x4*)(tab + c);
          if (out_f) *(f32x4*)(out_f + orow * C + c) = y;
          if (out_h) {
            typename Half<DT>::V4 hv, lv;
            const size_t oh = kt_half_offset(kt, orow, c, rows, C);
            if (out_l || out8) {
#pragma unroll
              for (int e = 0; e < 4; e += 2) {
                T h0, h1, l0, l1;
                split2_rtz(y[e], y[e + 1], h0, h1, l0, l1);
                hv[e] = h0; hv[e + 1] = h1; lv[e] = l0; lv[e + 1] = l1;
              }
              if (out_l) *(typename Half<DT>::V4*)(out_l + oh) = lv;
              if constexpr (X6 && DT == VDN_F16) {
                *(f16x4*)(stage + c) = hv;
                *(f16x4*)(stage + NV * 256 + c) = lv;
              }
            } else {
#pragma unroll
              for (int e = 0; e < 4; ++e) hv[e] = (T)y[e];
            }
            *(typename Half<DT>::V4*)(out_h + oh) = hv;
          }
        }
      }
      if constexpr (X6 && DT == VDN_F16) {
        {
          asm volatile("s_waitcnt lgkmcnt(0)" ::: "memory");
          const int nb = C >> 5;
          for (int t = lane; t < 2 * nb; t += 64) {
            const int plane = t >= nb, hb = t - plane * nb;
            f16x32 hv, xv;
#pragma unroll
            for (int q = 0; q < 4; ++q) {
              const f16x8 a = *(const f16x8*)(stage + hb * 32 + 8 * q);
#pragma unroll
              for (int e = 0; e < 8; ++e) hv[8 * q + e] = a[e];
            }
            const int sb = x6_scale_byte(hv);
            if (plane) {
#pragma unroll
              for (int q = 0; q < 4; ++q) {
                const f16x8 a = *(const f16x8*)(stage + NV * 256 + hb * 32 + 8 * q);
#pragma unroll
                for (int e = 0; e < 8; ++e) xv[8 * q + e] = a[e];
              }
            } else xv = hv;
            uint8_t* d8 = out8 + (size_t)plane * rows * C + kt_byte_offset(kt, orow, (hb >> 1) * 64, hb & 1, rows, C);
            x6_store_half(d8, xv, plane ? sb - 10 : sb);
          }
          asm volatile("s_waitcnt lgkmcnt(0)" ::: "memory");
        }
      }
    }
#pragma unroll
    for (int i = 0; i < NV; ++i) cur[i] = nxt[i];
  }
}

__device__ __forceinline__ int gn_split_begin(int HW, int sp, int nsplit) { return (int)(((long long)HW * sp) / nsplit); }

template <int DT>
__global__ __launch_bounds__(256) void groupnorm_stats_kernel(const typename Half<DT>::T* __restrict__ x,
                                                              const typename Half<DT>::T* __restrict__ xl, int HW,
                                                              int C, int groups, float* __restrict__ partial,
                                                              int nsplit) {
  using V8 = typename Half<DT>::V8;
  extern __shared__ __attribute__((aligned(16))) char smem[];
  const int f = blockIdx.x, sp = blockIdx.y;
  const int cv = C >> 3;
  const int pl = 256 / cv;
  const int tid = threadIdx.x;
  const int my_pl = tid / cv, my_cv = tid - my_pl * cv;
  const int p0 = gn_split_begin(HW, sp, nsplit), p1 = gn_split_begin(HW, sp + 1, nsplit);
  const int cg = C / groups;
  float* col = (float*)smem;
  __shared__ float gmean[64];
  const size_t xo = (size_t)f * HW * C + my_cv * 8;
  const float n = (float)(p1 - p0) * (float)cg;
  for (int pass = 0; pass < 2; ++pass) {
    float s[8], ss[8], m[8];
#pragma unroll
    for (int e = 0; e < 8; ++e) {
      s[e] = ss[e] = 0.f;
      m[e] = (pass && my_pl < pl) ? gmean[(my_cv * 8 + e) / cg] : 0.f;
    }
    if (my_pl < pl) {
      for (int p = p0 + my_pl; p < p1; p += pl) {
        const V8 v = *(const V8*)(x + xo + (size_t)p * C);
        V8 vl;
        if (xl) vl = *(const V8*)(xl + xo + (size_t)p * C);
#pragma unroll
        for (int e = 0; e < 8; ++e) {
          const float d = (xl ? (float)v[e] + (float)vl[e] : (float)v[e]) - m[e];
          s[e] += d;
          ss[e] += d * d;
        }
      }
#pragma unroll
      for (int e = 0; e < 8; ++e) {
        col[((size_t)my_pl * C + my_cv * 8 + e) * 2] = s[e];
        col[((size_t)my_pl * C + my_cv * 8 + e) * 2 + 1] = ss[e];
      }
    }
    __syncthreads();
    for (int g = tid; g < groups; g += 256) {
      float a = 0.f, bq = 0.f;
      for (int k = 0; k < pl; ++k)
        for (int c = g * cg; c < (g + 1) * cg; ++c) {
          a += col[((size_t)k * C + c) * 2];
          bq += col[((size_t)k * C + c) * 2 + 1];
        }
      if (pass == 0) {
        gmean[g] = n > 0.f ? a / n : 0.f;
      } else {
        float* o = partial + (((size_t)f * nsplit + sp) * groups + g) * 2;
        o[0] = n > 0.f ? gmean[g] + a / n : 0.f;
        o[1] = n > 0.f ? fmaxf(bq - a * a / n, 0.f) : 0.f;
      }
    }
    __syncthreads();
  }
}

template <int DT>
__global__ __launch_bounds__(256) void groupnorm_apply_kernel(const typename Half<DT>::T* __restrict__ x,
                                                              const typename Half<DT>::T* __restrict__ xl,
                                                              typename Half<DT>::T* __restrict__ y,
                                                              typename Half<DT>::T* __restrict__ yl, int HW, int C,
                                                              int groups, const float* __restrict__ w,
                                                              const float* __restrict__ b, float eps,
// ... 52 lines not shown
}

template <int DT>
__global__ void addtab_cast_kernel(const float* __restrict__ x, const float* __restrict__ tab, int tab_div, int tab_mod,
                                   typename Half<DT>::T* __restrict__ y, typename Half<DT>::T* __restrict__ yl, size_t rows,
                                   int C) {
  using T = typename Half<DT>::T;
  const int cv = C >> 2;
  const size_t n4 = rows * cv;
  for (size_t i = blockIdx.x * (size_t)blockDim.x + threadIdx.x; i < n4; i += (size_t)gridDim.x * blockDim.x) {
    const size_t row = i / cv;
    const int c = (int)(i - row * cv) * 4;
    f32x4 a = *(const f32x4*)(x + row * C + c);
    if (tab) a += *(const f32x4*)(tab + (size_t)((row / tab_div) % tab_mod) * C + c);
    typename Half<DT>::V4 h, l;
    split_or_round(yl != nullptr, a, h, l);
    store_planes(y, yl, row * C + c, h, l);
  }
}

__global__ void cast_kernel(const void* __restrict__ x, int xdt, void* __restrict__ y, int ydt, size_t n) {
  for (size_t i = blockIdx.x * (size_t)blockDim.x + threadIdx.x; i < n; i += (size_t)gridDim.x * blockDim.x)
    store_from_float(y, ydt, i, load_as_float(x, xdt, i));
}

template <typename XT, int NV>
int ln_launch_nv(const void* x, int rows, int C, const float* w, const float* b, float eps, const float* addvec,
                 float alpha, const float* addtab, int tab_div, int tab_mod, int out_group, void* out_h, void* out_l,
                 int h_dt, float* out_f, void* out8, int kt, hipStream_t s) {
  static const int resident = [] {
    int per_cu = 0, dev = 0;
    hipDeviceProp_t prop;
    if (hipOccupancyMaxActiveBlocksPerMultiprocessor(&per_cu, layernorm_kernel<XT, VDN_F16, NV, false>, 256, 0) != hipSuccess || per_cu <= 0)
      per_cu = 4;
    if (hipGetDevice(&dev) != hipSuccess || hipGetDeviceProperties(&prop, dev) != hipSuccess) return 256 * per_cu;
    return prop.multiProcessorCount * per_cu;
  }();
  constexpr size_t lds6 = (size_t)4 * 2 * NV * 256 * sizeof(_Float16);
  static const int resident6 = [] {
    int per_cu = 0, dev = 0;
    hipDeviceProp_t prop;
    if (hipOccupancyMaxActiveBlocksPerMultiprocessor(&per_cu, layernorm_kernel<XT, VDN_F16, NV, true>, 256, lds6) != hipSuccess || per_cu <= 0)
      per_cu = 3;
    if (hipGetDevice(&dev) != hipSuccess || hipGetDeviceProperties(&prop, dev) != hipSuccess) return 256 * per_cu;
    return prop.multiProcessorCount * per_cu;
  }();
  const int blocks = (rows + 3) / 4;
  const int res = out8 ? resident6 : resident;
  const dim3 grid(blocks < res ? blocks : res);
  if (h_dt == VDN_BF16)
    hipLaunchKernelGGL((layernorm_kernel<XT, VDN_BF16, NV, false>), grid, dim3(256), 0, s, (const XT*)x, rows, C, w, b, eps,
                       addvec, alpha, addtab, tab_div, tab_mod, out_group, (__bf16*)out_h, (__bf16*)out_l, out_f, (uint8_t*)nullptr, 0);
  else if (out8)
    hipLaunchKernelGGL((layernorm_kernel<XT, VDN_F16, NV, true>), grid, dim3(256), lds6, s, (const XT*)x, rows, C, w, b, eps,
                       addvec, alpha, addtab, tab_div, tab_mod, out_group, (_Float16*)out_h, (_Float16*)out_l, out_f, (uint8_t*)out8, kt);
  else
    hipLaunchKernelGGL((layernorm_kernel<XT, VDN_F16, NV, false>), grid, dim3(256), 0, s, (const XT*)x, rows, C, w, b, eps,
                       addvec, alpha, addtab, tab_div, tab_mod, out_group, (_Float16*)out_h, (_Float16*)out_l, out_f, (uint8_t*)nullptr, kt);
  VDN_CHECK_LAUNCH();
  return VDN_OK;
}

template <typename XT>
int ln_launch(const void* x, int rows, int C, const float* w, const float* b, float eps, const float* addvec,
              float alpha, const float* addtab, int tab_div, int tab_mod, int out_group, void* out_h, void* out_l,
              int h_dt, float* out_f, void* out8, int kt, hipStream_t s) {
  if (C <= 512)
    return ln_launch_nv<XT, 2>(x, rows, C, w, b, eps, addvec, alpha, addtab, tab_div, tab_mod, out_group, out_h, out_l, h_dt, out_f, out8, kt, s);
  if (C <= 1024)
    return ln_launch_nv<XT, 4>(x, rows, C, w, b, eps, addvec, alpha, addtab, tab_div, tab_mod, out_group, out_h, out_l, h_dt, out_f, out8, kt, s);
  return ln_launch_nv<XT, 8>(x, rows, C, w, b, eps, addvec, alpha, addtab, tab_div, tab_mod, out_group, out_h, out_l, h_dt, out_f, out8, kt, s);
}

}

extern "C" int vdn_layernorm(const void* x, int x_dt, int rows, int C, const float* w, const float* b, float eps,
                             const float* addvec, float alpha, const float* addtab, int tab_div, int tab_mod,
                             int out_group, void* out_h, void* out_h_lo, int h_dt, float* out_f, void* out8, int kt,
                             vdn_stream stream) {
  if (!x || !w || !b || rows <= 0 || C <= 0 || (!out_h && !out_f)) return VDN_EINVAL;
  if ((C & 3) || C > 2048) return VDN_EALIGN;
  if (addtab && (tab_div <= 0 || tab_mod <= 0)) return VDN_EINVAL;
  if (out_h && h_dt != VDN_F16 && h_dt != VDN_BF16) return VDN_EUNSUPPORTED;
  if ((out8 || kt) && (!out_h || h_dt != VDN_F16 || out_group > 0 || (C & 63) || ((uintptr_t)out8 & 15))) return VDN_EINVAL;
  hipStream_t s = (hipStream_t)stream;
  if (!addtab) { tab_div = 1; tab_mod = 1; }
  switch (x_dt) {
    case VDN_F32: return ln_launch<float>(x, rows, C, w, b, eps, addvec, alpha, addtab, tab_div, tab_mod, out_group, out_h, out_h_lo, h_dt, out_f, out8, kt, s);
    case VDN_F16: return ln_launch<_Float16>(x, rows, C, w, b, eps, addvec, alpha, addtab, tab_div, tab_mod, out_group, out_h, out_h_lo, h_dt, out_f, out8, kt, s);
    case VDN_BF16: return ln_launch<__bf16>(x, rows, C, w, b, eps, addvec, alpha, addtab, tab_div, tab_mod, out_group, out_h, out_h_lo, h_dt, out_f, out8, kt, s);
    default: return VDN_EUNSUPPORTED;
  }
}

extern "C" int vdn_groupnorm(int dt, const void* x, const void* x_lo, void* y, void* y_lo, int F, int HW, int C,
                             int groups, const float* w, const float* b, float eps, float* partial, int nsplit,
                             vdn_stream stream) {
  if (!x || !y || !w || !b || !partial || F <= 0 || HW <= 0 || groups <= 0 || groups > 64 || C % groups || nsplit <= 0)
    return VDN_EINVAL;
  if ((C & 7) || C > 2048) return VDN_EALIGN;
  hipStream_t s = (hipStream_t)stream;
  const int pl = 256 / (C >> 3);
  const size_t lds = (size_t)pl * C * 2 * sizeof(float);
  const int chunks = (int)(((size_t)HW * (C >> 3) + 256 * 8 - 1) / (256 * 8));
  return with_half(dt, [&](auto t) -> int {
    using T = typename Half<decltype(t)::value>::T;
    hipLaunchKernelGGL(groupnorm_stats_kernel<decltype(t)::value>, dim3(F, nsplit), dim3(256), lds, s, (const T*)x, (const T*)x_lo, HW,
                       C, groups, partial, nsplit);
    hipLaunchKernelGGL(groupnorm_apply_kernel<decltype(t)::value>, dim3(F, chunks), dim3(256), 0, s, (const T*)x, (const T*)x_lo, (T*)y,
                       (T*)y_lo, HW, C, groups, w, b, eps, partial, nsplit);
    VDN_CHECK_LAUNCH();
    return VDN_OK;
  });
}

extern "C" int vdn_add_vec(const float* x, const float* vec, float alpha, float* y, int rows, int C,
                           vdn_stream stream) {
  if (!x || !vec || !y || rows <= 0 || C <= 0) return VDN_EINVAL;
  if (C & 3) return VDN_EALIGN;
  const size_t n4 = (size_t)rows * C / 4;
  const int blocks = (int)((n4 + 255) / 256 < 2048 ? (n4 + 255) / 256 : 2048);
  hipLaunchKernelGGL(add_vec_kernel, dim3(blocks), dim3(256), 0, (hipStream_t)stream, x, vec, alpha, y, n4, C);
  VDN_CHECK_LAUNCH();
  return VDN_OK;
}

extern "C" int vdn_addtab_cast(int dt, const float* x, const float* tab, int tab_div, int tab_mod, void* y, void* y_lo,
                               size_t rows, int C, vdn_stream stream) {
  if (!x || !y || rows == 0 || C <= 0 || (tab && (tab_div <= 0 || tab_mod <= 0))) return VDN_EINVAL;
  if (C & 3) return VDN_EALIGN;
  const size_t n4 = rows * (C >> 2);
  const int blocks = (int)((n4 + 255) / 256 < 8192 ? (n4 + 255) / 256 : 8192);
  hipStream_t s = (hipStream_t)stream;
  if (!tab) { tab_div = 1; tab_mod = 1; }
  return with_half(dt, [&](auto t) -> int {
    using T = typename Half<decltype(t)::value>::T;
    hipLaunchKernelGGL(addtab_cast_kernel<decltype(t)::value>, dim3(blocks), dim3(256), 0, s, x, tab, tab_div, tab_mod, (T*)y, (T*)y_lo,
                       rows, C);
    VDN_CHECK_LAUNCH();
    return VDN_OK;
  });
}

extern "C" int vdn_cast(const void* x, int x_dt, void* y, int y_dt, size_t n, vdn_stream stream) {
  if (!x || !y || n == 0) return VDN_EINVAL;
  if (x_dt < 0 || x_dt > VDN_F32 || y_dt < 0 || y_dt > VDN_F32) return VDN_EUNSUPPORTED;
  const int blocks = (int)((n + 255) / 256 < 4096 ? (n + 255) / 256 : 4096);
  hipLaunchKernelGGL(cast_kernel, dim3(blocks), dim3(256), 0, (hipStream_t)stream, x, x_dt, y, y_dt, n);
  VDN_CHECK_LAUNCH();
  return VDN_OK;
}
```

### video-depth-normal-v2_amd/vdn/_abi.py

```python
from __future__ import annotations

import ctypes as C
import os

PKG = os.path.dirname(os.path.dirname(os.path.abspath(__file__)))
LIB_PATH = os.environ.get("VDN_LIB") or os.path.join(PKG, "lib", "libvdn_hip.so")

F16, BF16, F32, NONE = 0, 1, 2, 3
ACT_NONE, ACT_GELU, ACT_RELU, ACT_SILU = 0, 1, 2, 3
OUT_NONE, OUT_RELU, OUT_SIGMOID = 0, 1, 2
A_PLAIN, A_CONV3X3, A_PAD3X3 = 0, 1, 2
ST_PLAIN, ST_HEADS, ST_CONVT, ST_GEGLU = 0, 1, 2, 3
EVAL_DEPTH, EVAL_DISP = 0, 1
EVAL_TGM_ROWS, EVAL_TGM_FRAMES = 0, 1
TAIL_SHIFT, TAIL_MIX = 0, 1
PACK_LINEAR, PACK_CONV3X3, PACK_CONV3X3_TAPS, PACK_CONVT, PACK_GEGLU, PACK_ROPE = 0, 1, 2, 3, 4, 5

i32, vp, fp = C.c_int32, C.c_void_p, C.c_void_p


class GemmDesc(C.Structure):
    _fields_ = [
        ("dt", i32), ("M", i32), ("N", i32), ("K", i32),
        ("A", vp), ("a_mode", i32), ("lda", i32), ("relu_a", i32),
        ("cB", i32), ("cH", i32), ("cW", i32), ("cC", i32), ("cOH", i32), ("cOW", i32), ("cstride", i32),
        ("W", vp), ("ldb", i32),
        ("bias", fp), ("rowadd", fp), ("act", i32), ("gamma", fp), ("tab", fp), ("tab_mod", i32), ("tab_off", i32),
        ("res1", vp), ("res1_dt", i32), ("ldr1", i32),
        ("res2", vp), ("res2_dt", i32), ("ldr2", i32),
        ("store", i32), ("out", vp), ("out_dt", i32), ("ldc", i32), ("row_group", i32), ("row_skip", i32),
        ("dst", vp * 3), ("nsplit", i32), ("heads", i32), ("tokens", i32), ("tok_off", i32), ("tpad", i32),
        ("transposed", i32 * 3), ("rope", i32 * 3),
        ("rope_cs", fp), ("rope_mod", i32),
        ("ck", i32), ("cout", i32), ("zeros", vp),
        ("A_lo", vp), ("W_lo", vp), ("out_lo", vp), ("dst_lo", vp * 3), ("res1_lo", vp), ("res2_lo", vp),
        ("conv_korder", i32), ("cu_hint", i32),
        ("splitk_ws", vp), ("splitk_ws_bytes", C.c_int64), ("ksplit", i32),
        ("dst8", vp * 3),
        ("A8", vp), ("W8", vp), ("out8", vp),
        ("a_kt", i32), ("w_kt", i32), ("out_kt", i32), ("x8_terms", i32),
        ("tuning", vp),
        ("subpix", i32), ("subpix_bias", fp),
        ("pad_hi", vp),
    ]


class GemmTuning(C.Structure):
    _fields_ = [("force_bm", i32), ("p8", i32), ("no_splitk", i32), ("no_pipe", i32), ("splitk_p8", i32),
                ("cus", i32), ("splitk_occ", i32), ("splitk_max", i32), ("min_tiles", i32), ("f128", C.c_float),
                ("f192", C.c_float), ("x8", i32)]


class VdnError(RuntimeError):
    pass


def _load():
    if not os.path.exists(LIB_PATH):
        raise ImportError(
            f"{LIB_PATH} not found: the HIP extension is required (there is no CPU fallback). "
            f"Build it with `python __graft_entry__.py build` (hipcc --offload-arch=gfx950).")
    try:
        return C.CDLL(LIB_PATH)
    except OSError as e:
        raise ImportError(f"cannot load {LIB_PATH}: {e}. Rebuild with `python __graft_entry__.py build`.") from e


lib = _load()

EXPORTS = {
    "vdn_gemm": (C.c_int, [C.POINTER(GemmDesc), vp]),
    "vdn_gemm_get_tuning": (C.c_int, [C.POINTER(GemmTuning)]),
    "vdn_layernorm": (C.c_int, [vp, C.c_int, C.c_int, C.c_int, fp, fp, C.c_float, fp, C.c_float, fp, C.c_int, C.c_int,
                                C.c_int, vp, vp, C.c_int, fp, vp, C.c_int, vp]),
    "vdn_flash_attn": (C.c_int, [C.c_int, vp, vp, vp, vp, vp, vp, vp, vp, vp, vp, vp, C.c_int, C.c_int, C.c_int, C.c_int, C.c_int,
                                 C.c_int, C.c_int, C.c_float, C.c_int, vp]),
    "vdn_temporal_attn": (C.c_int, [C.c_int, vp, vp, vp, vp, C.c_int, C.c_int, C.c_int, C.c_int, C.c_int, C.c_float, fp, vp]),
    "vdn_groupnorm": (C.c_int, [C.c_int, vp, vp, vp, vp, C.c_int, C.c_int, C.c_int, C.c_int, fp, fp, C.c_float, fp,
                                C.c_int, vp]),
    "vdn_upsample_bilinear": (C.c_int, [C.c_int, vp, vp, vp, vp, C.c_int, C.c_int, C.c_int, C.c_int, C.c_int, C.c_int, vp]),
    "vdn_upsample_bilinear_f32": (C.c_int, [fp, fp, C.c_int, C.c_int, C.c_int, C.c_int, C.c_int, C.c_int, vp]),
    "vdn_patchify": (C.c_int, [C.c_int, fp, vp, vp, C.c_int, C.c_int, C.c_int, C.c_int, vp]),
    "vdn_fill_row": (C.c_int, [fp, fp, C.c_int, C.c_int, C.c_int, C.c_int, vp]),
    "vdn_bicubic": (C.c_int, [fp, fp, C.c_int, C.c_int, C.c_int, C.c_int, C.c_int, C.c_float, C.c_float, vp]),
    "vdn_preprocess": (C.c_int, [vp, C.c_int, C.c_int, C.c_int, C.c_int, fp, C.c_int, C.c_int, C.POINTER(C.c_float), C.POINTER(C.c_float), vp]),
    "vdn_add_vec": (C.c_int, [fp, fp, C.c_float, fp, C.c_int, C.c_int, vp]),
    "vdn_head_out": (C.c_int, [C.c_int, vp, vp, fp, C.c_float, fp, C.c_int, C.c_int, C.c_int, vp]),
    "vdn_depth_tail": (C.c_int, [C.c_int, fp, C.c_int, C.c_int, C.c_int, C.c_int, vp, vp, C.c_int, fp, fp, C.c_float, fp,
                                 C.c_int, C.c_int, C.c_int, vp]),
    "vdn_head_out_act": (C.c_int, [C.c_int, vp, vp, fp, C.c_float, fp, C.c_int, C.c_int, C.c_int, C.c_float, vp]),
    "vdn_depth_tail_act": (C.c_int, [C.c_int, fp, C.c_int, C.c_int, C.c_int, C.c_int, vp, vp, C.c_int, fp, fp, C.c_float, fp,
                                     C.c_int, C.c_int, C.c_int, C.c_float, vp]),
    "vdn_depth_to_points": (C.c_int, [fp, vp, C.c_int, C.c_int, C.c_double, C.c_double, vp, vp, vp]),
    "vdn_oc1_combine": (C.c_int, [fp, fp, fp, C.c_int, C.c_int, C.c_int, C.c_int, C.c_int, C.c_int, vp]),
    "vdn_pack_rows": (C.c_int, [C.c_int, C.c_int, C.c_int, C.c_int]),
    "vdn_pack_ldb": (C.c_int, [C.c_int, C.c_int, C.c_int, C.c_int]),
    "vdn_pack_weight": (C.c_int, [C.c_int, C.c_int, fp, C.c_int, C.c_int, C.c_int, vp, vp, C.c_int, vp]),
    "vdn_pack_bias": (C.c_int, [C.c_int, fp, C.c_int, C.c_int, C.c_int, fp, vp]),
    "vdn_pack_x8": (C.c_int, [vp, vp, C.c_int, C.c_int, vp, vp, C.c_int, C.c_int, vp]),
    "vdn_pack_x8_f32": (C.c_int, [fp, C.c_int, C.c_int, vp, vp, vp]),
    "vdn_pack_x8_relu_pad": (C.c_int, [vp, vp, C.c_int, C.c_int, C.c_int, C.c_int, vp, vp, vp]),
    "vdn_gemm_workspace_bytes": (C.c_size_t, [C.POINTER(GemmDesc)]),
    "vdn_groupnorm_workspace_bytes": (C.c_size_t, [C.c_int, C.c_int, C.c_int]),
    "vdn_mask_down1": (C.c_int, [fp, fp, C.c_int, C.c_int, C.c_int, C.c_int, C.c_int, fp, vp]),
    "vdn_mask_down2": (C.c_int, [fp, fp, C.c_int, C.c_int, C.c_int, C.c_int, C.c_int, fp, vp]),
    "vdn_dwconv7": (C.c_int, [fp, fp, C.c_int, C.c_int, C.c_int, C.c_int, fp, fp, vp]),
    "vdn_addtab_cast": (C.c_int, [C.c_int, fp, fp, C.c_int, C.c_int, vp, vp, C.c_size_t, C.c_int, vp]),
    "vdn_cast": (C.c_int, [vp, C.c_int, vp, C.c_int, C.c_size_t, vp]),
    "vdn_temporal_attn_last": (C.c_int, [C.c_int, fp, C.c_size_t, C.POINTER(C.c_int32), C.c_int, C.c_int, C.c_int, fp, fp, fp,
                                         C.c_float, vp, vp, vp]),
    "vdn_frame_median_workspace_bytes": (C.c_size_t, [C.c_int]),
    "vdn_frame_median": (C.c_int, [fp, C.c_int, C.c_size_t, fp, vp, vp]),
    "vdn_refine_scale": (C.c_int, [fp, fp, C.c_int, C.c_size_t, C.c_float, C.c_float, C.c_float, C.c_float, fp, fp, vp]),
    "vdn_refine_pack": (C.c_int, [fp, fp, C.c_int, C.c_int, C.c_int, C.c_int, vp]),
    "vdn_refine_finish": (C.c_int, [fp, fp, C.c_float, C.c_float, C.c_float, C.c_int, fp, C.c_size_t, vp]),
    "vdn_refine_normalize": (C.c_int, [fp, C.c_float, fp, C.c_size_t, vp]),
    "vdn_refine_mix": (C.c_int, [fp, fp, C.c_float, C.c_float, C.c_float, C.c_float, C.c_float, fp, C.c_size_t, vp]),
    "vdn_refine_window_tail_trip": (C.c_int, [C.c_int]),
    "vdn_refine_window_tail": (C.c_int, [fp, C.c_int, C.c_int, fp, C.c_int, C.POINTER(C.c_int32), C.c_int, C.c_int, C.c_int, C.c_int, C.c_int, C.c_float,
                                         C.c_float, C.c_float, C.c_float, C.c_float, fp, vp]),
    "vdn_dn_attn": (C.c_int, [C.c_int, vp, vp, vp, vp, C.c_int, C.c_int, C.c_int, C.c_int, C.c_int, C.c_int, C.c_int, C.c_int,
                              C.c_int, C.c_float, vp]),
    "vdn_dn_prologue": (C.c_int, [C.c_int, fp, fp, C.c_int, C.c_int, C.c_int, fp, C.c_int, fp, vp, vp, vp]),
    "vdn_dn_tail": (C.c_int, [fp, C.c_int, C.c_int, C.c_int, C.c_int, fp, fp, C.c_int, C.c_int, fp, C.c_int, fp, fp, fp, vp]),
    "vdn_hiera_embed": (C.c_int, [C.c_int, fp, vp, vp, C.c_int, C.c_int, vp]),
    "vdn_hiera_attn": (C.c_int, [C.c_int, vp, vp, vp, vp, C.c_int, C.c_int, C.c_int, C.c_int, C.c_int, C.c_float, vp]),
# ... 100 lines not shown
```

### video-depth-normal-v2_amd/vdn/depth_anything_v2.py

```python
from __future__ import annotations

import os

import numpy as np
import torch
import torch.nn as nn

from . import modules, util
from .engine import DPTEngine, EncoderEngine, MemoryEngine, ReadoutEngine
from .runtime import Runtime

_MEAN = (0.485, 0.456, 0.406)
_STD = (0.229, 0.224, 0.225)


PRECISIONS = {"f16x3": (torch.float16, True), "f16": (torch.float16, False),
              "bf16x3": (torch.bfloat16, True), "bf16": (torch.bfloat16, False)}
DEFAULT_PRECISION = "f16x3"


def _precision(name=None):
    name = (name or os.environ.get("VDN_PRECISION", DEFAULT_PRECISION)).lower()
    if name not in PRECISIONS:
        raise ValueError(f"VDN_PRECISION must be one of {sorted(PRECISIONS)}, got {name!r}")
# ... 51 lines not shown
        h, w = raw_image.shape[:2]
        img = torch.from_numpy(np.ascontiguousarray(raw_image)).to(rt.device)[None]
        return self.preprocess(rt, img, input_size, swap_rb=True), (h, w), img

    def image2tensor(self, raw_image: np.ndarray, input_size: int = 518):
        image, hw, _ = self._upload(raw_image, input_size)
        return image, hw

    def _infer_image_device(self, raw_image: np.ndarray, input_size: int, what: str):
        image, (h, w), img = self._upload(raw_image, input_size)
        depth = self.forward(image)
        rt = self._engines()["rt"]
        if tuple(depth.shape[-2:]) != (h, w):
            out = torch.empty((1, h, w), dtype=torch.float32, device=rt.device)
            rt.upsample_f32(depth.contiguous(), out, 1, depth.shape[-2], depth.shape[-1], h, w)
            depth = out
        from .util import check_finite
        check_finite(depth, what)
        return depth, img

    def _infer_image_vis(self, raw_image, input_size, pred_only, grayscale, palette) -> np.ndarray:
        from . import vis
        vis._check(palette, "bgr", "frame", grayscale, 3)
        depth, img = self._infer_image_device(raw_image, input_size, "infer_image_vis")
        with torch.cuda.device(depth.device):
            out = vis._colorize(self._engines()["rt"], depth.contiguous(), palette, "bgr", "frame", grayscale, 3,
                                None if pred_only else img, 50, None)
        return out[0].cpu().numpy()


class DepthAnythingV2(_SingleImage):
    def __init__(self, encoder="vitl", features=256, out_channels=[256, 512, 1024, 1024], use_bn=False,
                 use_clstoken=False, max_memory_length=6):
        super().__init__()
        self.intermediate_layer_idx = {k: v["taps"] for k, v in modules.ENCODERS.items()}
        self.encoder = encoder
        cfg = modules.ENCODERS[encoder]
        self.max_memory_length = max_memory_length
        self.pretrained = modules.dinov2(encoder)
        self.memory_block = modules.memory_block(cfg["dim"], max_memory_length, 4)
        self.depth_head = modules.dpt_head(cfg["dim"], features, out_channels, use_bn, use_clstoken)
        self._features, self._out_channels = features, list(out_channels)

    def _engines(self):
        if self._eng is None:
            rt = self._runtime()
            cfg = modules.ENCODERS[self.encoder]
            self._eng = dict(
                rt=rt, enc=EncoderEngine(rt, self.pretrained, cfg),
                mem=MemoryEngine(rt, self.memory_block, cfg["dim"], self.max_memory_length),
                head=DPTEngine(rt, self.depth_head, cfg["dim"], self._features, self._out_channels, temporal=False))
            if hasattr(self.depth_head, "readout_projects"):
                self._eng["enc"].readout = ReadoutEngine(rt, self.depth_head.readout_projects, cfg["dim"])
            self._lanes = None
        return self._eng

    def _stream_lanes(self, n: int):
        import copy
        e = self._engines()
        if self._lanes is None or len(self._lanes) != n:
            lanes = []
            for i in range(n):
                rt = e["rt"] if i == 0 else Runtime(e["rt"].device, e["rt"].half, e["rt"].split)
                rt.pv_products = e["rt"].pv_products
                enc, mem, head = (copy.copy(e[k]) for k in ("enc", "mem", "head"))
                enc.rt = mem.rt = head.rt = rt
                if getattr(enc, "readout", None) is not None:
                    enc.readout = copy.copy(enc.readout)
                    enc.readout.rt = rt
                mem.lane, mem._nomem = (i, n), {}
                if i > 0:
                    enc._pos_cache = {}
                lanes.append(dict(rt=rt, enc=enc, mem=mem, head=head, stream=torch.cuda.Stream(device=rt.device)))
            self._lanes = lanes
        return self._lanes

    def clear_memory(self):
        if self._eng is not None:
            self._eng["mem"].clear()

    def _forward_lane(self, ln, x, _pre_relu, out):
        rt, enc, mem, head = ln["rt"], ln["enc"], ln["mem"], ln["head"]
        B = x.shape[0]
        taps, last_f32, (ph, pw) = enc.run(x, want_f32_last=True)
        fm = mem.forward(last_f32, B, ph * pw)
        t3 = fm
        if getattr(enc, "readout", None) is not None:
            t3 = enc.readout.apply(3, fm, enc.cls_last, B, ph * pw, rt.hbuf("ro_fm", (B * ph * pw, enc.C)))
        head.run([taps[0], taps[1], taps[2], t3], B, ph, pw, relu=not _pre_relu, out=out)
        mem.update(fm, out.clamp(min=0) if _pre_relu else out, B, ph, pw)

    @torch.no_grad()
    def forward(self, x: torch.Tensor, _pre_relu: bool = False) -> torch.Tensor:
        e = self._engines()
        rt = e["rt"]
        x = x.to(device=rt.device, dtype=torch.float32).contiguous()
        B, _, H, W = x.shape
        e["mem"].prepare(B, (H // 14) * (W // 14))
        out = torch.empty((B, H, W), dtype=torch.float32, device=rt.device)
        nl = int(os.environ.get("VDN_STREAMS", "2"))
        if nl < 2 or B < int(os.environ.get("VDN_LANE_MIN_BATCH", "4")) or B % nl:
            rt.cu_hint = 0
            self._forward_lane(dict(rt=rt, enc=e["enc"], mem=e["mem"], head=e["head"]), x, _pre_relu, out)
            e["mem"].commit()
            return out
        lanes = self._stream_lanes(nl)
        for ln in lanes:
            ln["rt"].cu_hint = 256 // nl
        cur = torch.cuda.current_stream(rt.device)
        for ln, xs, os_ in zip(lanes, x.chunk(nl), out.chunk(nl)):
            ln["stream"].wait_stream(cur)
            with torch.cuda.stream(ln["stream"]):
                self._forward_lane(ln, xs.contiguous(), _pre_relu, os_)
        for ln in lanes:
            cur.wait_stream(ln["stream"])
        e["mem"].commit()
        return out

    @torch.no_grad()
    def infer_image(self, raw_image: np.ndarray, input_size: int = 518) -> np.ndarray:
        return self._infer_image_device(raw_image, input_size, "infer_image")[0][0].cpu().numpy()

    @torch.no_grad()
    def infer_image_vis(self, raw_image: np.ndarray, input_size: int = 518, pred_only: bool = False, grayscale: bool = False,
                        palette: str = "Spectral_r") -> np.ndarray:
        return self._infer_image_vis(raw_image, input_size, pred_only, grayscale, palette)
```

### video-depth-normal-v2_amd/vdn/engine.py

```python
from __future__ import annotations

import math
import os
from typing import List, Optional

import torch

from . import _abi as abi
from . import pack
from .runtime import HL, Runtime, ceil_to

GELU, RELU = abi.ACT_GELU, abi.ACT_RELU
PATCH = 14


class EncoderEngine:

    def __init__(self, rt: Runtime, mod, cfg: dict):
        self.rt, self.cfg = rt, cfg
        self.C, self.heads, self.depth, self.taps = cfg["dim"], cfg["heads"], cfg["depth"], cfg["taps"]
        h = rt.prec
        self.w_patch = pack.patch_embed(mod.patch_embed.proj.weight, h)
        self.b_patch = pack.f32(mod.patch_embed.proj.bias)
        self.cls = pack.f32(mod.cls_token).reshape(-1)
        self.pos = pack.f32(mod.pos_embed).reshape(-1, self.C)
        self.blocks = []
        self.hidden = cfg.get("swiglu") or 4 * self.C
        self.x8 = rt.x8_capable(self.C) and not cfg.get("swiglu")

        def lin(w, order):
            return pack.Linear(pack.linear(w, h), order if self.x8 else None)

        for b in mod.blocks:
            blk = dict(
                n1w=pack.f32(b.norm1.weight), n1b=pack.f32(b.norm1.bias),
                wqkv=lin(b.attn.qkv.weight, pack.ORDER_NATURAL), bqkv=pack.f32(b.attn.qkv.bias),
                wproj=lin(b.attn.proj.weight, pack.ORDER_ATTN), bproj=pack.f32(b.attn.proj.bias),
                ls1=pack.f32(b.ls1.gamma),
                n2w=pack.f32(b.norm2.weight), n2b=pack.f32(b.norm2.bias),
                ls2=pack.f32(b.ls2.gamma))
            if cfg.get("swiglu"):
                Hd = cfg["swiglu"]
                w12, b12 = b.mlp.w12.weight, b.mlp.w12.bias
                blk["wfc1"], blk["bfc1"] = pack.geglu(torch.cat([w12[Hd:], w12[:Hd]]), torch.cat([b12[Hd:], b12[:Hd]]), h)
                blk["wfc2"], blk["bfc2"] = pack.linear(b.mlp.w3.weight, h), pack.f32(b.mlp.w3.bias)
            else:
                blk["wfc1"], blk["bfc1"] = lin(b.mlp.fc1.weight, pack.ORDER_NATURAL), pack.f32(b.mlp.fc1.bias)
                blk["wfc2"], blk["bfc2"] = lin(b.mlp.fc2.weight, pack.ORDER_GEMM), pack.f32(b.mlp.fc2.bias)
            self.blocks.append(blk)
        self.nw, self.nb = pack.f32(mod.norm.weight), pack.f32(mod.norm.bias)
        self._pos_cache = {}
        self.x8_terms = [dict(qkv=0, proj=0, fc1=0, fc2=0) for _ in self.blocks]
        for item in filter(None, os.environ.get("VDN_X8_TERMS", "").split(",")):
            name, val = item.split("=")
            val, _, rng = val.partition("@")
            a, b = (int(v) for v in rng.split("-")) if rng else (0, len(self.blocks) - 1)
            for L in range(a, b + 1):
                self.x8_terms[L][name] = int(val)

    def _pos_for(self, ph: int, pw: int):
        key = (ph, pw)
        if key not in self._pos_cache:
            rt, C = self.rt, self.C
            gs = int(math.sqrt(self.pos.shape[0] - 1))
            if ph * pw == gs * gs and ph == pw:
                table = self.pos
            else:
                table = torch.empty((1 + ph * pw, C), dtype=torch.float32, device=rt.device)
                table[0].copy_(self.pos[0])
                sx, sy = float(ph + 0.1) / gs, float(pw + 0.1) / gs
                rt.bicubic(self.pos[1:], table[1:], gs, gs, ph, pw, C, sx, sy)
            self._pos_cache[key] = (table, (self.cls + table[0]).contiguous())
        return self._pos_cache[key]

    def run(self, x: torch.Tensor, want_f32_last: bool = False, tap_out=None):
        rt, C, Hh = self.rt, self.C, self.heads
        Bf, _, H, W = x.shape
        assert H % PATCH == 0 and W % PATCH == 0, "input sides must be multiples of 14 (patch_embed.py:73-74)"
        ph, pw = H // PATCH, W // PATCH
        P, N = ph * pw, ph * pw + 1
        M = Bf * N
        table, cls_row = self._pos_for(ph, pw)
        rows = rt.hbuf("patch_rows", (Bf * P, 640))
        rt.patchify(x, rows, Bf, H, W, 640)
        tok = rt.fbuf("tokens", (M, C))
        rt.fill_row(tok, cls_row, Bf, N, 0, C)
        rt.gemm(rows, self.w_patch, Bf * P, C, 640, out=tok, bias=self.b_patch, tab=table, tab_mod=P, tab_off=1,
                row_group=P, row_skip=1)
        npad = ceil_to(N, 64)
        q = rt.hbuf("enc_q", (Bf * Hh, npad, 64), zero=True)
        k = rt.hbuf("enc_k", (Bf * Hh, npad, 64), zero=True)
        vt = rt.hbuf("enc_vt", (Bf * Hh, 64, npad), zero=True)
        q8, k8 = rt.qk8("enc_q8", Bf * Hh, npad), rt.qk8("enc_k8", Bf * Hh, npad)
        Hd = self.hidden
        heads = rt.head_split([(q, q8), (k, k8)], vt, Hh, N, npad)
        outs, last_f32 = [], None
        readout = getattr(self, "readout", None)
        probe = getattr(self, "probe", None)
        if probe is not None:
            probe(-1, tok)
        use8 = self.x8 and rt.x8_rows(M) and q8 is not None and rt.pv_products != 3
        hn, att, f1 = rt.operand("enc_ln", (M, C), use8), rt.operand("enc_att", (M, C), use8), rt.operand("enc_fc1", (M, Hd), use8)
        for i, b in enumerate(self.blocks):
            xt = self.x8_terms[i]
            rt.layernorm(tok, M, C, b["n1w"], b["n1b"], 1e-6, out_h=hn)
            rt.gemm(hn, b["wqkv"], M, 3 * C, C, bias=b["bqkv"], store=abi.ST_HEADS, heads=heads, tag="enc_linear", x8_terms=xt["qkv"])
            rt.flash_attn(q, k, vt, att, Bf, Hh, N, npad, N, npad, 64 ** -0.5, tag="enc_attn", q8=q8, k8=k8)
            rt.gemm(att, b["wproj"], M, C, C, bias=b["bproj"], gamma=b["ls1"], res1=tok, out=tok, tag="enc_linear", x8_terms=xt["proj"])
            rt.layernorm(tok, M, C, b["n2w"], b["n2b"], 1e-6, out_h=hn)
            if self.cfg.get("swiglu"):
                rt.gemm(hn, b["wfc1"], M, 2 * Hd, C, bias=b["bfc1"], store=abi.ST_GEGLU, act=abi.ACT_SILU, out=f1, tag="enc_linear")
            else:
                rt.gemm(hn, b["wfc1"], M, Hd, C, bias=b["bfc1"], act=GELU, out=f1, tag="enc_linear", x8_terms=xt["fc1"])
            rt.gemm(f1, b["wfc2"], M, C, Hd, bias=b["bfc2"], gamma=b["ls2"], res1=tok, out=tok, tag="enc_linear", x8_terms=xt["fc2"])
            if probe is not None:
                probe(i, tok)
            if i in self.taps:
                j = self.taps.index(i)
                t = tap_out[j] if tap_out is not None else rt.hbuf(f"tap{j}", (Bf * P, C))
                f = None
                if want_f32_last and j == len(self.taps) - 1:
                    f = last_f32 = rt.fbuf("tap_last_f32", (Bf * P, C))
                if readout is None:
                    rt.layernorm(tok, M, C, self.nw, self.nb, 1e-6, out_h=t, out_f=f, out_group=N)
                else:
                    last = want_f32_last and j == len(self.taps) - 1
                    raw = t if last else rt.hbuf("tap_raw", (Bf * P, C))
                    rt.layernorm(tok, M, C, self.nw, self.nb, 1e-6, out_h=raw, out_f=f, out_group=N)
                    cls = rt.fbuf("cls_norm_last" if last else "cls_norm", (Bf, C))
                    rt.layernorm(tok.view(Bf, N, C)[:, 0].contiguous(), Bf, C, self.nw, self.nb, 1e-6, out_f=cls)
                    if last:
                        self.cls_last = cls
                    else:
                        readout.apply(j, raw, cls, Bf, P, t)
                outs.append(t)
        return outs, last_f32, (ph, pw)


class ReadoutEngine:

    def __init__(self, rt: Runtime, mods, C: int):
        self.rt, self.C = rt, C
        h = rt.prec
        self.w1 = [pack.linear(m[0].weight[:, :C].contiguous(), h) for m in mods]
        self.w2 = [pack.linear(m[0].weight[:, C:].contiguous(), h) for m in mods]
        self.b = [pack.f32(m[0].bias) for m in mods]

    def apply(self, j: int, x, cls_f32: torch.Tensor, Bf: int, P: int, out):
        rt, C = self.rt, self.C
        cb = rt.fbuf("ro_cb", (Bf, C))
        rt.gemm(rt.to_half(cls_f32), self.w2[j], Bf, C, C, bias=self.b[j], out=cb)
        for b in range(Bf):
            rt.gemm(x.narrow0(b * P, P), self.w1[j], P, C, C, bias=cb[b], act=GELU, out=out.narrow0(b * P, P))
        return out


class TemporalEngine:

    def __init__(self, rt: Runtime, mod, c: int, idx: int):
        self.rt, self.c, self.idx = rt, c, idx
        h = rt.prec
        tt = mod.temporal_transformer
        blk = tt.transformer_blocks[0]
        self.gnw, self.gnb = pack.f32(tt.norm.weight), pack.f32(tt.norm.bias)
        self.w_in, self.b_in = pack.linear(tt.proj_in.weight, h), pack.f32(tt.proj_in.bias)
        self.x8 = rt.x8_capable(c)
        x8_order = pack.ORDER_NATURAL if self.x8 else None
        self.att = []
        for i in range(2):
            a = blk.attention_blocks[i]
            wqkv, _ = pack.cat_proj([a.to_q.weight, a.to_k.weight, a.to_v.weight], [None, None, None], [0, 0, 0], h)
            wqkv = pack.Linear(wqkv, x8_order)
            rope = not hasattr(a, "pos_encoder")
            if rope:
                Tm = a.max_len
                pe64 = torch.zeros((Tm, c), dtype=torch.float64, device=a.to_q.weight.device)
                fr = 1.0 / (10000.0 ** (torch.arange(0, c, 2, dtype=torch.float32)[: c // 2] / c))
                ang = torch.outer(torch.arange(Tm, dtype=torch.float32), fr)
                rope_cs = torch.stack([ang.cos(), ang.sin()], dim=-1).contiguous().to(a.to_q.weight.device)
            else:
                pe64 = a.pos_encoder.pe.detach().double().reshape(-1, c)
                rope_cs = None
            self.att.append(dict(
                nw=pack.f32(blk.norms[i].weight), nb=pack.f32(blk.norms[i].bias), wqkv=wqkv,
                pe=None if rope else pack.f32(a.pos_encoder.pe).reshape(-1, c), rope_cs=rope_cs, max_len=pe64.shape[0],
                pe_q=(pe64 @ a.to_q.weight.detach().double().t()).float().contiguous(),
                pe_k=(pe64 @ a.to_k.weight.detach().double().t()).float().contiguous(),
                pe_v=(pe64 @ a.to_v.weight.detach().double().t()).float().contiguous(),
                wo=pack.linear(a.to_out[0].weight, h), bo=pack.f32(a.to_out[0].bias)))
        self.fnw, self.fnb = pack.f32(blk.ff_norm.weight), pack.f32(blk.ff_norm.bias)
        wg, self.bg = pack.geglu(blk.ff.net[0].proj.weight, blk.ff.net[0].proj.bias, h)
        self.wg = pack.Linear(wg, x8_order)
        self.wf2, self.bf2 = pack.linear(blk.ff.net[2].weight, h), pack.f32(blk.ff.net[2].bias)
        self.w_out, self.b_out = pack.linear(tt.proj_out.weight, h), pack.f32(tt.proj_out.bias)

    def gn(self, x, F: int, HW: int):
        g = self.rt.hbuf("tm_gn", (F * HW, self.c))
        self.rt.groupnorm(x, g, F, HW, self.c, 32, self.gnw, self.gnb, 1e-6)
        return g

    def core(self, g, B: int, T: int, D: int):
        rt, c = self.rt, self.c
        M = B * T * D
        assert T <= self.att[0]["max_len"], "clip longer than temporal_max_len (motion_module.py:200-213)"
        hs = rt.fbuf("tm_h", (M, c))
        rt.gemm(g, self.w_in, M, c, c, bias=self.b_in, out=hs)
        n = rt.operand("tm_n", (M, c), self.x8 and rt.x8_rows(M) and M * 3 * c >= (1 << 20))
        qkv = rt.hbuf("tm_qkv", (M, 3 * c))
        a = rt.hbuf("tm_a", (M, c))
        for at in self.att:
            rt.layernorm(hs, M, c, at["nw"], at["nb"], 1e-5, out_h=n, addtab=at["pe"], tab_div=D, tab_mod=T)
            rt.gemm(n, at["wqkv"], M, 3 * c, c, out=qkv)
            rt.temporal_attn(qkv, a, B, T, D, c, 8, (c // 8) ** -0.5, rope_cs=at["rope_cs"])
            rt.gemm(a, at["wo"], M, c, c, bias=at["bo"], res1=hs, out=hs)
        gg = rt.hbuf("tm_gg", (M, 4 * c))
        rt.layernorm(hs, M, c, self.fnw, self.fnb, 1e-5, out_h=n)
        rt.gemm(n, self.wg, M, 8 * c, c, bias=self.bg, store=abi.ST_GEGLU, out=gg)
        hh = rt.hbuf("tm_hh", (M, c))
        rt.gemm(gg, self.wf2, M, c, 4 * c, bias=self.bf2, res1=hs, out=hh)
        return hh

    def out(self, hh, x, M: int):
        y = self.rt.hbuf(f"tm_out{self.idx}", (M, self.c))
        self.rt.gemm(hh, self.w_out, M, self.c, self.c, bias=self.b_out, res1=x, out=y)
        return y

    def run(self, x, B: int, T: int, HW: int):
        return self.out(self.core(self.gn(x, B * T, HW), B, T, HW), x, B * T * HW)

    STREAM_SLOTS = 44

    def run_stream(self, x, HW: int, window_slots, new_slot: int):
        rt, c = self.rt, self.c
        g = self.gn(x, 1, HW)
        hs = rt.fbuf("ts_h", (HW, c))
        rt.gemm(g, self.w_in, HW, c, c, bias=self.b_in, out=hs)
        nh = rt.hbuf("ts_nh", (HW, c))
        a = rt.hbuf("ts_a", (HW, c))
        slots = list(window_slots) + [new_slot]
        for j, at in enumerate(self.att):
            pool = rt.fbuf(f"ts_pool{self.idx}_{j}", (self.STREAM_SLOTS, HW, 3 * c))
            rt.layernorm(hs, HW, c, at["nw"], at["nb"], 1e-5, out_h=nh)
            rt.gemm(nh, at["wqkv"], HW, 3 * c, c, out=pool[new_slot])
            rt.temporal_attn_last(pool, slots, at["pe_q"], at["pe_k"], at["pe_v"], a, HW, c, (c // 8) ** -0.5)
            rt.gemm(a, at["wo"], HW, c, c, bias=at["bo"], res1=hs, out=hs)
        n = rt.hbuf("ts_n", (HW, c))
        rt.layernorm(hs, HW, c, self.fnw, self.fnb, 1e-5, out_h=n)
        gg = rt.hbuf("ts_gg", (HW, 4 * c))
        rt.gemm(n, self.wg, HW, 8 * c, c, bias=self.bg, store=abi.ST_GEGLU, out=gg)
        hh = rt.hbuf("ts_hh", (HW, c))
        rt.gemm(gg, self.wf2, HW, c, 4 * c, bias=self.bf2, res1=hs, out=hh)
        return self.out(hh, x, HW)

    def run_sharded(self, x, exch, HW: int):
        from .dist import shard_core
        Tl = exch.Tl
        g = self.gn(x, Tl, HW)

        def core(planes, D):
            hh = self.core(HL(planes[0], planes[1] if len(planes) > 1 else None), 1, exch.T, D)
            return [hh.hi] + ([hh.lo] if hh.lo is not None else [])

        back = shard_core(exch, [g.hi] + ([g.lo] if g.lo is not None else []), HW, core)
        return self.out(HL(back[0], back[1] if len(back) > 1 else None), x, Tl * HW)


class DPTEngine:

    def __init__(self, rt: Runtime, mod, in_ch: int, features: int, out_channels, temporal: bool):
        self.rt, self.C, self.F, self.oc = rt, in_ch, features, list(out_channels)
        h = rt.prec
        self.proj = [(pack.conv1x1(p.weight, h), pack.f32(p.bias)) for p in mod.projects]
        self.rt0 = pack.conv_transpose(mod.resize_layers[0].weight, mod.resize_layers[0].bias, h)
        self.rt1 = pack.conv_transpose(mod.resize_layers[1].weight, mod.resize_layers[1].bias, h)
        self.rs3 = (pack.conv3x3(mod.resize_layers[3].weight, h), pack.f32(mod.resize_layers[3].bias))
        s = mod.scratch
        self.rn = [pack.conv3x3(getattr(s, f"layer{i + 1}_rn").weight, h) for i in range(4)]

        def fold(conv, bn):
            w, b = conv.weight.detach().float(), conv.bias.detach().float()
            if bn is None:
                return w, b
            sc = bn.weight.detach().float() / torch.sqrt(bn.running_var.detach().float() + 1e-5)
            return w * sc[:, None, None, None], (b - bn.running_mean.detach().float()) * sc + bn.bias.detach().float()

        self.rcu_x8 = rt.x8_capable(features) and features % 256 == 0 and not os.environ.get("VDN_RCU_X3")
        self.rcu_path = {}
        self._rcu_x8_ok = True

        def rcu(r, x8):
            w1, b1 = fold(r.conv1, getattr(r, "bn1", None))
            w2, b2 = fold(r.conv2, getattr(r, "bn2", None))
            d = dict(w1=pack.conv3x3(w1, h), b1=pack.f32(b1), w2=pack.conv3x3(w2, h), b2=pack.f32(b2))
            if x8:
                d.update(x1=pack.conv3x3_x8(w1, h), x2=pack.conv3x3_x8(w2, h))
            return d

        self.ref = {}
        for i in range(1, 5):
            f = getattr(s, f"refinenet{i}")
            x8 = self.rcu_x8 and i in (1, 2)
            self.ref[i] = dict(r1=rcu(f.resConfUnit1, x8), r2=rcu(f.resConfUnit2, x8),
                               wo=pack.conv1x1(f.out_conv.weight, h), bo=pack.f32(f.out_conv.bias))
        self.oc1 = (pack.conv3x3(s.output_conv1.weight, h), pack.f32(s.output_conv1.bias))
        self.oc2 = (pack.conv3x3(s.output_conv2[0].weight, h), pack.f32(s.output_conv2[0].bias))
        w2 = s.output_conv2[0].weight
        fused = h.split and w2.shape[0] == 32 and w2.shape[1] % 32 == 0 and not os.environ.get("VDN_TAIL_UNFUSED")
        self.oc2_taps = pack.conv3x3_taps(w2, h) if fused else None
        self.oc1_low = None
        if fused and (features // 2) % 16 == 0 and not os.environ.get("VDN_OC1_HIRES"):
            f1 = s.refinenet1.out_conv
            self.oc1_low = pack.lowres_oc1(s.output_conv1.weight, f1.weight, f1.bias, h)
        self.rn_low = [None, None]
        if not os.environ.get("VDN_RN_HIRES"):
            for i, k in enumerate((4, 2)):
                if pack.subpixel_conv_ok(self.oc[i], features, k, h):
                    rl = mod.resize_layers[i]
                    self.rn_low[i] = pack.subpixel_conv(rl.weight, rl.bias, getattr(s, f"layer{i + 1}_rn").weight, h)
        self.w_last = pack.f32(s.output_conv2[2].weight).reshape(-1)
        self.b_last = float(s.output_conv2[2].bias.detach().float().item())
        self.temporal = None
        if temporal:
            chans = [self.oc[2], self.oc[3], features, features]
            self.temporal = [TemporalEngine(rt, mod.motion_modules[i], chans[i], i) for i in range(4)]

    def _conv3(self, x, w, Bf, H, W, Cin, Cout, name, *, stride=1, bias=None, relu_a=False, act=0, res1=None, res2=None,
               f32_out=False):
        OH, OW = (H + 2 - 3) // stride + 1, (W + 2 - 3) // stride + 1
        out = (self.rt.fbuf if f32_out else self.rt.hbuf)(name, (Bf * OH * OW, Cout))
        self.rt.gemm(x, w, Bf * OH * OW, Cout, 9 * Cin, out=out, bias=bias, act=act, relu_a=relu_a, res1=res1, res2=res2,
                     conv=dict(B=Bf, H=H, W=W, C=Cin, OH=OH, OW=OW, stride=stride))
        return out

    def _rcu(self, r, x, Bf, H, W, name, extra=None):
        F = self.F
        t = self._conv3(x, r["w1"], Bf, H, W, F, F, "rcu_t", bias=r["b1"], relu_a=True, act=RELU)
        return self._conv3(t, r["w2"], Bf, H, W, F, F, name, bias=r["b2"], res1=x, res2=extra)

    def _fusion(self, i, Bf, size_in, size_out, prev, skip=None):
        rt, F = self.rt, self.F
        H, W = size_in
        f = self.ref[i]
        x = prev
        M = Bf * H * W
        if self.rcu_x8 and self._rcu_x8_ok and i in (1, 2) and rt.x8_rows(Bf * (H + 2) * (W + 2)):
            self.rcu_path[i] = "x8"
            pa, pb = rt.pad_operand("rcu_pa", Bf, H, W, F), rt.pad_operand("rcu_pb", Bf, H, W, F)
            rt.pack_x8_relu_pad(skip if skip is not None else x, pa)
            if skip is not None:
                r = f["r1"]
                rt.conv3x3_pad(pa, r["x1"], F, r["b1"], out_pad=pb)
                x = rt.conv3x3_pad(pb, r["x2"], F, r["b2"], out=rt.hbuf(f"ff{i}_s", (M, F)), res1=skip, res2=prev, out_pad=pa)
            r = f["r2"]
            rt.conv3x3_pad(pa, r["x1"], F, r["b1"], out_pad=pb)
            u = rt.conv3x3_pad(pb, r["x2"], F, r["b2"], out=rt.hbuf(f"ff{i}_u", (M, F)), res1=x)
        else:
            self.rcu_path[i] = "x3"
            if skip is not None:
                x = self._rcu(f["r1"], skip, Bf, H, W, f"ff{i}_s", extra=prev)
            u = self._rcu(f["r2"], x, Bf, H, W, f"ff{i}_u")
        if size_out is None:
            return u
        v = rt.hbuf(f"ff{i}_v", (Bf * H * W, F))
        rt.gemm(u, f["wo"], Bf * H * W, F, F, bias=f["bo"], out=v)
        OH, OW = size_out
        p = rt.hbuf(f"path{i}", (Bf * OH * OW, F))
        rt.upsample(v, p, Bf, H, W, OH, OW, F)
        return p

    def run(self, taps: List[torch.Tensor], Bf: int, ph: int, pw: int, T: Optional[int] = None, relu: bool = True,
            exch=None, stream=None, out: Optional[torch.Tensor] = None, act: Optional[int] = None, out_scale: float = 1.0):
        rt, C, F, oc = self.rt, self.C, self.F, self.oc
        self._rcu_x8_ok = exch is None and stream is None
        P = ph * pw
        pr = []
        for i in range(4):
            o = rt.hbuf(f"proj{i}", (Bf * P, oc[i]))
            rt.gemm(taps[i], self.proj[i][0], Bf * P, oc[i], C, bias=self.proj[i][1], out=o)
            pr.append(o)
        s1, s2, s3 = (4 * ph, 4 * pw), (2 * ph, 2 * pw), (ph, pw)
        s4 = ((ph + 2 - 3) // 2 + 1, (pw + 2 - 3) // 2 + 1)

        def level(i, k, size, wT, name):
            if self.rn_low[i] is not None:
                r = rt.hbuf(name + "_rn", (Bf * size[0] * size[1], F))
                return rt.gemm(pr[i], self.rn_low[i][0], Bf * P, k * k * F, 4 * oc[i], store=abi.ST_CONVT, out=r,
                               conv=dict(B=Bf, H=ph, W=pw, C=oc[i], OH=ph, OW=pw, stride=1, korder=1),
                               convt=dict(k=k, cout=F, B=Bf, H=ph, W=pw), subpix_bias=self.rn_low[i][1])
            l = rt.hbuf(name, (Bf * size[0] * size[1], oc[i]))
            rt.gemm(pr[i], wT[0], Bf * P, k * k * oc[i], oc[i], bias=wT[1], store=abi.ST_CONVT, out=l,
                    convt=dict(k=k, cout=oc[i], B=Bf, H=ph, W=pw))
            return self._conv3(l, self.rn[i], Bf, size[0], size[1], oc[i], F, name + "_rn")

        r1 = level(0, 4, s1, self.rt0, "l1")
        r2 = level(1, 2, s2, self.rt1, "l2")
        l3 = pr[2]
        l4 = self._conv3(pr[3], self.rs3[0], Bf, ph, pw, oc[3], oc[3], "l4", stride=2, bias=self.rs3[1])
        def tm(i, x, hw):
            if stream is not None:
                return self.temporal[i].run_stream(x, hw, stream["window"], stream["new"])
            if exch is not None:
                return self.temporal[i].run_sharded(x, exch, hw)
            return self.temporal[i].run(x, Bf // T, T, hw)

        if self.temporal is not None:
            l3 = tm(0, l3, s3[0] * s3[1])
            l4 = tm(1, l4, s4[0] * s4[1])
        r3 = self._conv3(l3, self.rn[2], Bf, s3[0], s3[1], oc[2], F, "l3_rn")
        r4 = self._conv3(l4, self.rn[3], Bf, s4[0], s4[1], oc[3], F, "l4_rn")
        p4 = self._fusion(4, Bf, s4, s3, r4)
        if self.temporal is not None:
            p4 = tm(2, p4, s3[0] * s3[1])
        p3 = self._fusion(3, Bf, s3, s2, p4, r3)
        if self.temporal is not None:
            p3 = tm(3, p3, s2[0] * s2[1])
        p2 = self._fusion(2, Bf, s2, s1, p3, r2)
        s0 = (2 * s1[0], 2 * s1[1])
        H, W = ph * PATCH, pw * PATCH
        if out is not None:
            assert out.shape == (Bf, H, W) and out.dtype == torch.float32 and out.is_contiguous(), (out.shape, out.dtype)
        depth = out if out is not None else rt.fbuf("depth", (Bf, H, W))
        sy, sx = (s0[0] - 1) / max(H - 1, 1), (s0[1] - 1) / max(W - 1, 1)
        fused = self.oc2_taps is not None and int(17 * sy) + 3 <= 13 and int(17 * sx) + 3 <= 13
        if fused and self.oc1_low is not None and rt.lowres_oc1_rows(Bf * s0[0] * s0[1]):
            u = self._fusion(1, Bf, s1, None, p2, r1)
            M1 = Bf * s1[0] * s1[1]
            z = rt.fbuf("oc1_z", (M1, 9 * (F // 2)))
            rt.gemm(u, self.oc1_low[0], M1, 9 * (F // 2), F, bias=self.oc1_low[1], out=z)
            o1 = rt.fbuf("out1_f32", (Bf * s0[0] * s0[1], F // 2))
            rt.oc1_combine(z, self.oc1[1], o1, Bf, s1[0], s1[1], s0[0], s0[1], F // 2)
            rt.depth_tail(o1, self.oc2_taps, self.oc2[1], self.w_last, self.b_last, depth, Bf, s0[0], s0[1], F // 2, H, W, relu, act, out_scale)
            return depth
        p1 = self._fusion(1, Bf, s1, s0, p2, r1)
        if fused:
            o1 = self._conv3(p1, self.oc1[0], Bf, s0[0], s0[1], F, F // 2, "out1_f32", bias=self.oc1[1], f32_out=True)
            rt.depth_tail(o1, self.oc2_taps, self.oc2[1], self.w_last, self.b_last, depth, Bf, s0[0], s0[1], F // 2, H, W, relu, act, out_scale)
            return depth
        o1 = self._conv3(p1, self.oc1[0], Bf, s0[0], s0[1], F, F // 2, "out1", bias=self.oc1[1])
        up = rt.hbuf("out_up", (Bf * H * W, F // 2))
        rt.upsample(o1, up, Bf, s0[0], s0[1], H, W, F // 2)
        o2 = self._conv3(up, self.oc2[0], Bf, H, W, F // 2, 32, "out2", bias=self.oc2[1], act=RELU)
        rt.head_out(o2, self.w_last, self.b_last, depth, Bf * H * W, 32, relu, act, out_scale)
        return depth


class MemoryEngine:

    def __init__(self, rt: Runtime, mod, C: int, max_len: int):
        self.rt, self.C, self.heads, self.max_len = rt, C, C // 64, max_len
        h = rt.prec
        ma = mod.memory_attention
        self.x8 = rt.x8_capable(C)

        def lin(w, order):
            return pack.Linear(w, order if self.x8 else None)

        NAT, GEMM, ATTN = pack.ORDER_NATURAL, pack.ORDER_GEMM, pack.ORDER_ATTN
        self.layers = []
        for l in ma.layers:
            sa, ca = l.self_attn, l.cross_attn_image
            wqkv, bqkv = pack.cat_proj([sa.q_proj.weight, sa.k_proj.weight, sa.v_proj.weight],
                                       [sa.q_proj.bias, sa.k_proj.bias, sa.v_proj.bias], [1, 1, 0], h)
            wq, bq = pack.cat_proj([ca.q_proj.weight], [ca.q_proj.bias], [1], h)
            wkv, bkv = pack.cat_proj([ca.k_proj.weight, ca.v_proj.weight], [ca.k_proj.bias, ca.v_proj.bias], [1, 0], h)
            self.layers.append(dict(
                n1w=pack.f32(l.norm1.weight), n1b=pack.f32(l.norm1.bias),
                n2w=pack.f32(l.norm2.weight), n2b=pack.f32(l.norm2.bias),
                n3w=pack.f32(l.norm3.weight), n3b=pack.f32(l.norm3.bias),
                wqkv=lin(wqkv, NAT), bqkv=bqkv, wso=lin(pack.linear(sa.out_proj.weight, h), ATTN), bso=pack.f32(sa.out_proj.bias),
                wq=lin(wq, NAT), bq=bq, wkv=lin(wkv, NAT), bkv=bkv,
                wco=lin(pack.linear(ca.out_proj.weight, h), ATTN), bco=pack.f32(ca.out_proj.bias),
                w1=lin(pack.linear(l.linear1.weight, h), NAT), b1=pack.f32(l.linear1.bias),
                w2=lin(pack.linear(l.linear2.weight, h), GEMM), b2=pack.f32(l.linear2.bias)))
        self.nw, self.nb = pack.f32(ma.norm.weight), pack.f32(ma.norm.bias)
        self.curr_pos = pack.f32(mod.curr_pos_enc).reshape(-1)
        self.no_mem = mod.no_mem_embed.detach().float().reshape(1, -1)
        me = mod.memory_encoder

        def flat(*ts):
            return torch.cat([t.detach().float().reshape(-1) for t in ts]).contiguous()

        e0, e1 = me.mask_downsampler[0].encoder, me.mask_downsampler[1].encoder
        self.md1 = flat(e0[0].weight, e0[0].bias, e0[1].weight, e0[1].bias, e0[3].weight, e0[3].bias)
        self.md2 = flat(e1[0].weight, e1[0].bias, e1[1].weight, e1[1].bias, e1[3].weight, e1[3].bias)
        assert self.md1.numel() == 53 and self.md2.numel() == 2598
        self.wpix, self.bpix = pack.conv1x1(me.pix_feat_proj.weight, h), pack.f32(me.pix_feat_proj.bias)
        self.cx = []
        for b in me.fuser.layers:
            self.cx.append(dict(
                wdw=b.dwconv.weight.detach().float().reshape(C, 49).t().contiguous(), bdw=pack.f32(b.dwconv.bias),
                nw=pack.f32(b.norm.weight), nb=pack.f32(b.norm.bias),
                w1=lin(pack.linear(b.pwconv1.weight, h), NAT), b1=pack.f32(b.pwconv1.bias),
                w2=lin(pack.linear(b.pwconv2.weight, h), GEMM), b2=pack.f32(b.pwconv2.bias), g=pack.f32(b.gamma)))
        self.state = {"count": 0, "shape": None}
        self.lane = (0, 1)
        self.bank_rt = rt
        self._rope = {}
        self._nomem = {}

    def clear(self):
        self.state["count"] = 0
        self.state["shape"] = None

    @property
    def S(self):
        return min(self.state["count"], self.max_len)

    def _rope_for(self, side):
        if side not in self._rope:
            self._rope[side] = pack.rope_table(side, side, 64, device=self.rt.device)
        return self._rope[side]

    def prepare(self, B: int, P: int):
        st = self.state
        if st["shape"] != (B, P):
            if st["count"] > 0:
                raise RuntimeError(f"memory bank holds {self.S} frame(s) of batch/grid {st['shape']} but the new frame is "
                                   f"{(B, P)}: call clear_memory() before changing the batch size or resolution")
            st["shape"] = (B, P)
        side = int(math.sqrt(P))
        assert side * side == P, "MemoryBlock assumes square inputs (memory_block.py:85)"
        self._rope_for(side)
        self._bank_full(B, P)

    def commit(self):
        self.state["count"] += 1

    def _bank_full(self, B, P):
        rt, Hh = self.bank_rt, self.heads
        tp = ceil_to(self.max_len * P, 64)
        ks = [rt.hbuf(f"mem_k{l}", (B * Hh, tp, 64), zero=True) for l in range(len(self.layers))]
        vs = [rt.hbuf(f"mem_vt{l}", (B * Hh, 64, tp), zero=True) for l in range(len(self.layers))]
        k8 = [rt.qk8(f"mem_k8{l}", B * Hh, tp) for l in range(len(self.layers))]
        return ks, vs, k8, tp

    def _bank(self, B, P):
        i, n = self.lane
        ks, vs, k8, tp = self._bank_full(B * n, P)
        r0, nr = i * B * self.heads, B * self.heads
        return ([k.narrow0(r0, nr) for k in ks], [v.narrow0(r0, nr) for v in vs],
                [None if t is None else t.narrow(0, r0, nr) for t in k8], tp)

    def forward(self, feat_f32: torch.Tensor, B: int, P: int) -> torch.Tensor:
        rt, C, Hh = self.rt, self.C, self.heads
        assert self.state["shape"] == (B * self.lane[1], P), "MemoryEngine.prepare() not called for this batch"
        side = int(math.sqrt(P))
        M = B * P
        cs = self._rope_for(side)
        pp = ceil_to(P, 64)
        x = rt.fbuf("ma_x", (M, C))
        rt.add_vec(feat_f32, self.curr_pos, 0.1, x, M, C)
        q = rt.hbuf("ma_q", (B * Hh, pp, 64), zero=True)
        k = rt.hbuf("ma_k", (B * Hh, pp, 64), zero=True)
        vt = rt.hbuf("ma_vt", (B * Hh, 64, pp), zero=True)
        q8, k8 = rt.qk8("ma_q8", B * Hh, pp), rt.qk8("ma_k8", B * Hh, pp)
        ks, vs, k8s, tp = self._bank(B, P)
        S = self.S
        if S == 0:
            nk, nk_pad = P, pp
            if M not in self._nomem:
                self._nomem[M] = rt.to_half(self.no_mem.expand(M, C).contiguous())
            a_nm = self._nomem[M]
            ks = [rt.hbuf(f"nomem_k{l}", (B * Hh, pp, 64), zero=True) for l in range(len(self.layers))]
            vs = [rt.hbuf(f"nomem_vt{l}", (B * Hh, 64, pp), zero=True) for l in range(len(self.layers))]
            k8s = [rt.qk8(f"nomem_k8{l}", B * Hh, pp) for l in range(len(self.layers))]
            for l, L in enumerate(self.layers):
                rt.gemm(a_nm, L["wkv"], M, 2 * C, C, bias=L["bkv"], store=abi.ST_HEADS,
                        heads=rt.head_split([(ks[l], k8s[l])], vs[l], Hh, P, pp, rope_cs=cs, rope_mod=P))
        else:
            nk, nk_pad = S * P, tp
        sh = rt.head_split([(q, q8), (k, k8)], vt, Hh, P, pp, rope_cs=cs, rope_mod=P)
        qh = rt.head_split([(q, q8)], None, Hh, P, pp, rope_cs=cs, rope_mod=P)
        use8 = self.x8 and rt.x8_rows(M) and q8 is not None and rt.pv_products != 3
        n, att, h2 = rt.operand("ma_n", (M, C), use8), rt.operand("ma_att", (M, C), use8), rt.operand("ma_h2", (M, 2 * C), use8)
        for l, L in enumerate(self.layers):
            rt.layernorm(x, M, C, L["n1w"], L["n1b"], 1e-5, out_h=n)
            rt.gemm(n, L["wqkv"], M, 3 * C, C, bias=L["bqkv"], store=abi.ST_HEADS, heads=sh)
            rt.flash_attn(q, k, vt, att, B, Hh, P, pp, P, pp, 0.125, q8=q8, k8=k8)
            rt.gemm(att, L["wso"], M, C, C, bias=L["bso"], res1=x, out=x)
            rt.layernorm(x, M, C, L["n2w"], L["n2b"], 1e-5, out_h=n, addvec=self.curr_pos, alpha=1.0)
            rt.gemm(n, L["wq"], M, C, C, bias=L["bq"], store=abi.ST_HEADS, heads=qh)
            rt.flash_attn(q, ks[l], vs[l], att, B, Hh, P, pp, nk, nk_pad, 0.125, q8=q8, k8=k8s[l])
            rt.gemm(att, L["wco"], M, C, C, bias=L["bco"], res1=x, out=x)
            rt.layernorm(x, M, C, L["n3w"], L["n3b"], 1e-5, out_h=n)
            rt.gemm(n, L["w1"], M, 2 * C, C, bias=L["b1"], act=GELU, out=h2)
            rt.gemm(h2, L["w2"], M, C, 2 * C, bias=L["b2"], res1=x, out=x)
        out = rt.hbuf("mem_out", (M, C))
        rt.layernorm(x, M, C, self.nw, self.nb, 1e-5, out_h=out)
        return out

    def update(self, mem_out: torch.Tensor, depth: torch.Tensor, B: int, ph: int, pw: int):
        rt, C, Hh = self.rt, self.C, self.heads
        P, M = ph * pw, B * ph * pw
        H, W = depth.shape[-2], depth.shape[-1]
        h1, w1 = (H + 2 - 3) // 2 + 1, (W + 2 - 3) // 2 + 1
        h2, w2 = (h1 - 7) // 7 + 1, (w1 - 7) // 7 + 1
        assert (h2, w2) == (ph, pw), "mask downsampler output must match the feature grid (memory_encoder.py:173)"
        m1 = rt.fbuf("me_m1", (B, h1, w1))
        rt.mask_down1(depth, m1, B, H, W, h1, w1, self.md1)
        m2 = rt.fbuf("me_m2", (M,))
        rt.mask_down2(m1, m2, B, h1, w1, h2, w2, self.md2)
        x = rt.fbuf("me_x", (M, C))
        rt.gemm(mem_out, self.wpix, M, C, C, bias=self.bpix, rowadd=m2, out=x)
        d = rt.fbuf("me_dw", (M, C))
        use8 = self.x8 and rt.x8_rows(M)
        n, h4, feat = rt.operand("me_n", (M, C), use8), rt.operand("me_h4", (M, 4 * C), use8), rt.operand("mem_feat", (M, C), use8)
        for cx in self.cx:
            rt.dwconv7(x, d, B, ph, pw, C, cx["wdw"], cx["bdw"])
            rt.layernorm(d, M, C, cx["nw"], cx["nb"], 1e-6, out_h=n)
            rt.gemm(n, cx["w1"], M, 4 * C, C, bias=cx["b1"], act=GELU, out=h4)
            rt.gemm(h4, cx["w2"], M, C, 4 * C, bias=cx["b2"], gamma=cx["g"], res1=x,
                    out=(feat if cx is self.cx[-1] and not use8 else x))
        if use8:
            rt.pack_x8_f32(x, feat.hi, feat.p8)
        ks, vs, k8s, tp = self._bank(B, P)
        slot = self.state["count"] % self.max_len
        cs = self._rope_for(int(math.sqrt(P)))
        for l, L in enumerate(self.layers):
            rt.gemm(feat, L["wkv"], M, 2 * C, C, bias=L["bkv"], store=abi.ST_HEADS,
                    heads=rt.head_split([(ks[l], k8s[l])], vs[l], Hh, P, tp, rope_cs=cs, rope_mod=P, tok_off=slot * P))
```

### video-depth-normal-v2_amd/vdn/runtime.py

```python
from __future__ import annotations

import os

import ctypes as C
from typing import Dict, List, Optional, Sequence, Tuple

import torch

from . import _abi as abi
from ._abi import F16, BF16, F32
from .pack import Linear, Prec

_TDT = {torch.float16: F16, torch.bfloat16: BF16, torch.float32: F32}
_POISON = bool(int(__import__("os").environ.get("VDN_POISON", "0")))


def ceil_to(x: int, m: int) -> int:
    return (x + m - 1) // m * m


class HL:
    __slots__ = ("hi", "lo")

    def __init__(self, hi: torch.Tensor, lo: Optional[torch.Tensor] = None):
# ... 108 lines not shown
            if not zero and _POISON and t.is_floating_point():
                t.fill_(float("nan"))
            self._bufs[key] = t
        return t

    def hbuf(self, name, shape, zero=False) -> HL:
        hi = self.buf(name, shape, self.half, zero)
        return HL(hi, self.buf(name + "#lo", shape, self.half, zero) if self.split else None)

    def operand(self, name: str, shape, x8: bool = False):
        if not x8:
            return self.hbuf(name, shape)
        return KT(self.buf(name + "_kt", shape, self.half), self.buf(name + "8", (2, *shape), torch.uint8))

    def pad_operand(self, name: str, B: int, H: int, W: int, C: int) -> PadKT:
        assert C % 64 == 0 and self.half == torch.float16, (C, self.half)
        Mp, g = B * (H + 2) * (W + 2), W + 3
        return PadKT(self.buf(name + "_pkt", (C * Mp + 64 * g,), self.half, zero=True),
                     self.buf(name + "_p8", (2 * C * Mp + 128 * g,), torch.uint8, zero=True), B, H, W, C)

    def x8_capable(self, Cn: int) -> bool:
        return self.split and self.half == torch.float16 and Cn % 64 == 0 and os.environ.get("VDN_X8", "1") != "0"

    @staticmethod
    def x8_rows(M: int) -> bool:
        return M >= int(os.environ.get("VDN_X8_MIN_ROWS", "4096"))

    def to_half(self, x: torch.Tensor) -> HL:
        return HL.from_float(x, self.half, self.split)

    def qk8(self, name: str, bh: int, tpad: int) -> Optional[torch.Tensor]:
        if not (self.split and self.half == torch.float16) or os.environ.get("VDN_ATTN_QK8", "1") == "0":
            return None
        return self.buf(name, (bh, tpad, 128), torch.uint8, zero=True)

    def v_dst(self, vt: HL) -> HL:
        if (vt.lo is not None and self.half == torch.float16 and os.environ.get("VDN_ATTN_QK8", "1") != "0"
                and self.pv_products == 1):
            return HL(vt.hi, None)
        return vt

    def qk_dst(self, t: HL, t8) -> HL:
        if self.pv_products == 3:
            return t
        return HL(t.hi, None) if (t8 is not None and t.lo is not None) else t

    def head_split(self, qk, vt, heads: int, tokens: int, tpad: int, rope_cs=None, rope_mod: int = 0, tok_off: int = 0) -> dict:
        nv = int(vt is not None)
        return dict(dst=[self.qk_dst(t, t8) for t, t8 in qk] + [self.v_dst(vt) for _ in range(nv)], dst8=[t8 for _, t8 in qk] + [None] * nv,
                    transposed=[0] * len(qk) + [1] * nv, rope=[int(rope_cs is not None)] * len(qk) + [0] * nv, rope_cs=rope_cs,
                    rope_mod=rope_mod, heads=heads, tokens=tokens, tok_off=tok_off, tpad=tpad)

    def fbuf(self, name, shape, zero=False):
        return self.buf(name, shape, torch.float32, zero)

    def workspace_bytes(self) -> int:
        return sum(t.numel() * t.element_size() for t in self._bufs.values())

    def _ws(self, name: str, nbytes: int) -> torch.Tensor:
        return self.buf(name, ((nbytes + 7) // 8,), torch.float64)

    def _launch(self, fn, *args, tag: Optional[str] = None, flop: float = 0.0):
        if tag is not None and self.timing is not None:
            s, e = torch.cuda.Event(enable_timing=True), torch.cuda.Event(enable_timing=True)
            s.record()
            rc = fn(*args, torch.cuda.current_stream(self.device).cuda_stream)
            e.record()
            self.timing.append((tag, s, e, flop))
        else:
            rc = fn(*args, torch.cuda.current_stream(self.device).cuda_stream)
        abi.check(rc, fn.__name__)

    @staticmethod
    def _p(t: Optional[torch.Tensor]):
        return None if t is None else t.data_ptr()

    def gemm(self, A: torch.Tensor, W: torch.Tensor, M: int, N: int, K: int, *, lda: Optional[int] = None,
             out: Optional[torch.Tensor] = None, ldc: Optional[int] = None, bias=None, act: int = 0, gamma=None,
             rowadd=None, tab=None, tab_mod: int = 0, tab_off: int = 0, res1=None, ldr1=None, res2=None, ldr2=None,
             conv: Optional[dict] = None, relu_a: bool = False, store: int = abi.ST_PLAIN, row_group: int = 0,
             row_skip: int = 0, heads: Optional[dict] = None, convt: Optional[dict] = None, tag: Optional[str] = None,
             a8: Optional[torch.Tensor] = None, w8: Optional[torch.Tensor] = None, out8: Optional[torch.Tensor] = None,
             a_kt: bool = False, w_kt: bool = False, out_kt: bool = False, x8_terms: int = 0,
             subpix_bias: Optional[torch.Tensor] = None, pad: Optional[PadKT] = None, pad_out: Optional[PadKT] = None):
        if isinstance(W, Linear):
            if not isinstance(A, KT):
                W, x8_terms = W.hl, 0
            elif W.x8 is None:
                raise abi.VdnError("vdn_gemm: a cross-term (KT) activation needs a weight packed with X8 planes")
            else:
                a8, w8, a_kt, w_kt, W = A.p8, W.x8.p8, True, True, W.x8.hi
        elif isinstance(A, KT):
            raise abi.VdnError("vdn_gemm: a cross-term (KT) activation needs a pack.Linear weight")
        if isinstance(out, KT):
            out8, out_kt = out.p8, True
        d = abi.GemmDesc()
        d.dt = self.dt
        d.M, d.N, d.K = M, N, K
        A, d.A_lo = _hl(A)
        W, d.W_lo = _hl(W)
        d.A = A.data_ptr()
        d.relu_a = 1 if relu_a else 0
        if conv is not None:
            d.a_mode = abi.A_CONV3X3
            d.cB, d.cH, d.cW, d.cC = conv["B"], conv["H"], conv["W"], conv["C"]
            d.cOH, d.cOW, d.cstride = conv["OH"], conv["OW"], conv["stride"]
            d.lda = conv["C"]
            d.conv_korder = conv.get("korder", 1 if conv["C"] % 64 == 0 else 0)
        elif pad is not None:
            d.a_mode = abi.A_PAD3X3
            d.cB, d.cH, d.cW, d.cC = pad.B, pad.H, pad.W, pad.C
        else:
            d.a_mode = abi.A_PLAIN
            d.lda = lda if lda is not None else K
        d.W = W.data_ptr()
        d.ldb = W.shape[1]
        assert W.shape[0] == N and W.dtype == self.half and A.dtype == self.half, (W.shape, N, W.dtype, A.dtype)
        assert W.is_contiguous()
        d.bias = self._p(bias)
        d.rowadd = self._p(rowadd)
        d.act = act
        d.gamma = self._p(gamma)
        d.tab = self._p(tab)
        d.tab_mod, d.tab_off = tab_mod, tab_off
        if res1 is not None:
            r1, d.res1_lo = _hl(res1)
            d.res1, d.res1_dt, d.ldr1 = r1.data_ptr(), _TDT[r1.dtype], (ldr1 if ldr1 is not None else N)
        if res2 is not None:
            r2, d.res2_lo = _hl(res2)
            d.res2, d.res2_dt, d.ldr2 = r2.data_ptr(), _TDT[r2.dtype], (ldr2 if ldr2 is not None else N)
        d.store = store
        if out is not None:
            oh, d.out_lo = _hl(out)
            d.out = oh.data_ptr()
            d.out_dt = _TDT[oh.dtype]
            d.ldc = ldc if ldc is not None else (N // 2 if store == abi.ST_GEGLU else N)
        d.row_group, d.row_skip = row_group, row_skip
        if heads is not None:
            dst = heads["dst"]
            d.nsplit = len(dst)
            for i, t in enumerate(dst):
                th, d.dst_lo[i] = _hl(t)
                d.dst[i] = th.data_ptr()
                d.transposed[i] = int(heads["transposed"][i])
                d.rope[i] = int(heads.get("rope", (0, 0, 0))[i])
                t8 = (heads.get("dst8") or (None, None, None))[i]
                if t8 is not None:
                    d.dst8[i] = t8.data_ptr()
            d.heads, d.tokens, d.tok_off, d.tpad = heads["heads"], heads["tokens"], heads.get("tok_off", 0), heads["tpad"]
            if heads.get("rope_cs") is not None:
                d.rope_cs, d.rope_mod = heads["rope_cs"].data_ptr(), heads["rope_mod"]
        if convt is not None:
            d.ck, d.cout = convt["k"], convt["cout"]
            d.cB, d.cH, d.cW = convt["B"], convt["H"], convt["W"]
        d.zeros = self.zeros.data_ptr()
        if a8 is not None and w8 is not None:
            d.A8, d.W8 = a8.data_ptr(), w8.data_ptr()
        if out8 is not None:
            d.out8 = out8.data_ptr()
        if pad_out is not None:
            d.pad_hi, d.out8 = pad_out.hi.data_ptr(), pad_out.p8.data_ptr()
        d.a_kt, d.w_kt, d.out_kt = int(a_kt), int(w_kt), int(out_kt)
        d.x8_terms = int(x8_terms)
        if subpix_bias is not None:
            assert subpix_bias.dtype == torch.float32 and subpix_bias.is_contiguous() and subpix_bias.numel() == 4 * N, subpix_bias.shape
            d.subpix, d.subpix_bias = 1, subpix_bias.data_ptr()
        d.cu_hint = self.cu_hint
        if abi.OVERRIDE is not None:
            d.tuning = C.addressof(abi.OVERRIDE)
        if self.split:
            ws = self.buf("splitk_ws", (32 * 1024 * 1024,), torch.float32)
            d.splitk_ws, d.splitk_ws_bytes = ws.data_ptr(), ws.numel() * 4
        self._launch(abi.lib.vdn_gemm, C.byref(d), tag=tag, flop=2.0 * M * N * K)
        return out

    def layernorm(self, x: torch.Tensor, rows: int, Cn: int, w, b, eps: float, *, out_h=None, out_f=None, addvec=None,
                  alpha: float = 1.0, addtab=None, tab_div: int = 1, tab_mod: int = 1, out_group: int = 0, out8=None,
                  kt: bool = False):
        if isinstance(out_h, KT):
            out8, kt = out_h.p8, True
        oh, ol = _hl(out_h) if out_h is not None else (None, None)
        self._launch(abi.lib.vdn_layernorm, x.data_ptr(), _TDT[x.dtype], rows, Cn, w.data_ptr(), b.data_ptr(), eps,
                     self._p(addvec), alpha, self._p(addtab), tab_div, tab_mod, out_group, self._p(oh), ol, self.dt,
                     self._p(out_f), self._p(out8), int(kt))

    def flash_attn(self, Q, K, Vt, out, B: int, H: int, nq: int, nq_pad: int, nk: int, nk_pad: int, scale: float,
                   tag: Optional[str] = None, q8: Optional[torch.Tensor] = None, k8: Optional[torch.Tensor] = None,
                   out8: Optional[torch.Tensor] = None, out_kt: bool = False):
        if isinstance(out, KT):
            out8, out_kt = out.p8, True
        (Q, ql), (K, kl), (Vt, vl), (out, ol) = _hl(Q), _hl(K), _hl(Vt), _hl(out)
        self._launch(abi.lib.vdn_flash_attn, self.dt, Q.data_ptr(), K.data_ptr(), Vt.data_ptr(), out.data_ptr(), ql, kl,
                     vl, ol, self._p(q8), self._p(k8), self._p(out8), int(out_kt), B, H, nq, nq_pad, nk, nk_pad, scale, self.pv_products, tag=tag,
                     flop=4.0 * B * H * nq * nk * 64)

    def temporal_attn(self, qkv, out, Bv: int, T: int, D: int, c: int, heads: int, scale: float, rope_cs=None):
        (qkv, ql), (out, ol) = _hl(qkv), _hl(out)
        self._launch(abi.lib.vdn_temporal_attn, self.dt, qkv.data_ptr(), out.data_ptr(), ql, ol, Bv, T, D, c, heads, scale,
                     self._p(rope_cs))

    def temporal_attn_last(self, pool: torch.Tensor, slots, pe_q, pe_k, pe_v, out, HW: int, c: int, scale: float):
        T = len(slots)
        tab = (C.c_int32 * T)(*slots)
        (out, ol) = _hl(out)
        self._launch(abi.lib.vdn_temporal_attn_last, self.dt, pool.data_ptr(), pool.stride(0), tab, T, HW, c, pe_q.data_ptr(),
                     pe_k.data_ptr(), pe_v.data_ptr(), scale, out.data_ptr(), ol)

    def groupnorm(self, x, y, F: int, HW: int, Cn: int, groups: int, w, b, eps: float):
        nsplit = 16 if HW >= 1024 else 4
        part = self.fbuf("gn_partial", (F, nsplit, groups, 2))
        (x, xl), (y, yl) = _hl(x), _hl(y)
        self._launch(abi.lib.vdn_groupnorm, self.dt, x.data_ptr(), xl, y.data_ptr(), yl, F, HW, Cn, groups, w.data_ptr(),
                     b.data_ptr(), eps, part.data_ptr(), nsplit)

    def upsample(self, x, y, B: int, IH: int, IW: int, OH: int, OW: int, Cn: int):
        (x, xl), (y, yl) = _hl(x), _hl(y)
        self._launch(abi.lib.vdn_upsample_bilinear, self.dt, x.data_ptr(), xl, y.data_ptr(), yl, B, IH, IW, OH, OW, Cn)

    def upsample_f32(self, x, y, B: int, IH: int, IW: int, OH: int, OW: int, relu: bool = False):
        dev = self.device
        self._launch(abi.lib.vdn_upsample_bilinear_f32, checked_ptr("upsample_f32: x", x, dev, _f32, count=B * IH * IW),
                     checked_ptr("upsample_f32: y", y, dev, _f32, count=B * OH * OW), B, IH, IW, OH, OW, int(relu))

    def stitch_fit(self, pred: torch.Tensor, target: torch.Tensor, coef: torch.Tensor):
        dev = self.device
        p = checked_ptr("stitch_fit: pred", pred, dev, _f32)
        n = pred.numel()
        self._launch(abi.lib.vdn_stitch_fit, p, checked_ptr("stitch_fit: target", target, dev, _f32, count=n), n,
                     self._ws("stitch_ws", abi.lib.vdn_stitch_workspace_bytes()).data_ptr(),
                     checked_ptr("stitch_fit: coef", coef, dev, _f32, count=2))

    def stitch_apply(self, window: torch.Tensor, coef: torch.Tensor, out_tail: torch.Tensor, out_new: torch.Tensor,
                     ref1: torch.Tensor, align_len: int, overlap: int, ref_frame: int):
        dev = self.device
        w = checked_ptr("stitch_apply: window", window, dev, _f32)
        T, frame = window.shape[0], tuple(window.shape[1:])
        self._launch(abi.lib.vdn_stitch_apply, w, checked_ptr("stitch_apply: coef", coef, dev, _f32, count=2),
                     checked_ptr("stitch_apply: out_tail", out_tail, dev, _f32, (overlap - align_len,) + frame),
                     checked_ptr("stitch_apply: out_new", out_new, dev, _f32, (T - overlap,) + frame),
                     checked_ptr("stitch_apply: ref1", ref1, dev, _f32, frame),
                     window[0].numel(), T, align_len, overlap, ref_frame)

    def _eval_args(self, what: str, pred, gt, mask):
        p = checked_ptr(what + ": pred", pred, self.device, _f32, 3)
# ... 297 lines not shown

    def fill_row(self, x, vec, B: int, rows_per_b: int, row: int, Cn: int):
        self._launch(abi.lib.vdn_fill_row, x.data_ptr(), vec.data_ptr(), B, rows_per_b, row, Cn)

    def bicubic(self, src, dst, ih: int, iw: int, oh: int, ow: int, Cn: int, scale_rows: float, scale_cols: float):
        self._launch(abi.lib.vdn_bicubic, src.data_ptr(), dst.data_ptr(), ih, iw, oh, ow, Cn, scale_rows, scale_cols)

    def preprocess_u8(self, frames_u8: torch.Tensor, H: int, W: int, mean, std, swap_rb: bool = False,
                      out: Optional[torch.Tensor] = None) -> torch.Tensor:
        src = checked_ptr("preprocess_u8: frames_u8", frames_u8, self.device, _u8, (None, None, None, 3))
        n, h, w, _ = frames_u8.shape
        if out is None:
            out = torch.empty((n, 3, H, W), dtype=torch.float32, device=self.device)
        m3, s3 = (C.c_float * 3)(*mean), (C.c_float * 3)(*std)
        self._launch(abi.lib.vdn_preprocess, src, n, h, w, int(swap_rb),
                     checked_ptr("preprocess_u8: out", out, self.device, _f32, (n, 3, H, W)), H, W, m3, s3)
        return out

    def add_vec(self, x, vec, alpha: float, y, rows: int, Cn: int):
        self._launch(abi.lib.vdn_add_vec, x.data_ptr(), vec.data_ptr(), alpha, y.data_ptr(), rows, Cn)

    @staticmethod
    def _out_act(relu: bool, act: Optional[int]) -> int:
        if act is None:
            return abi.OUT_RELU if relu else abi.OUT_NONE
        if act not in (abi.OUT_NONE, abi.OUT_RELU, abi.OUT_SIGMOID):
            raise ValueError(f"act must be one of OUT_NONE, OUT_RELU, OUT_SIGMOID (0, 1, 2), got {act!r}")
        return act

    def depth_tail(self, x: torch.Tensor, w: HL, bias2, w1, b1: float, depth, B: int, IH: int, IW: int, Cn: int, OH: int,
                   OW: int, relu: bool = False, act: Optional[int] = None, out_scale: float = 1.0):
        assert x.dtype == torch.float32 and x.is_contiguous() and w.lo is not None and w.hi.shape[0] == 32
        self._launch(abi.lib.vdn_depth_tail_act, self.dt, x.data_ptr(), B, IH, IW, Cn, w.hi.data_ptr(), w.lo.data_ptr(),
                     w.hi.shape[1], bias2.data_ptr(), w1.data_ptr(), b1, depth.data_ptr(), OH, OW, self._out_act(relu, act),
                     float(out_scale))

    @staticmethod
    def lowres_oc1_rows(M: int) -> bool:
        return M >= int(os.environ.get("VDN_OC1_LOWRES_MIN_ROWS", "65536"))

    def oc1_combine(self, z: torch.Tensor, bias, out: torch.Tensor, B: int, IH: int, IW: int, OH: int, OW: int, Cn: int):
        assert z.dtype == torch.float32 and z.is_contiguous() and z.numel() == B * IH * IW * 9 * Cn, (z.shape, z.dtype)
        assert out.dtype == torch.float32 and out.is_contiguous() and out.numel() == B * OH * OW * Cn, (out.shape, out.dtype)
        self._launch(abi.lib.vdn_oc1_combine, z.data_ptr(), bias.data_ptr(), out.data_ptr(), B, IH, IW, OH, OW, Cn)

    def head_out(self, feat, w, bias: float, depth, M: int, Cn: int, relu: bool = False, act: Optional[int] = None,
                 out_scale: float = 1.0):
        feat, fl = _hl(feat)
        self._launch(abi.lib.vdn_head_out_act, self.dt, feat.data_ptr(), fl, w.data_ptr(), bias, depth.data_ptr(), M, Cn,
                     self._out_act(relu, act), float(out_scale))

    def depth_to_points(self, depth: torch.Tensor, rgb: torch.Tensor, fx: float, fy: float, points: torch.Tensor,
                        colors: torch.Tensor):
        dev = self.device
        d = checked_ptr("depth_to_points: depth", depth, dev, _f32, 2)
        h, w = depth.shape
        self._launch(abi.lib.vdn_depth_to_points, d, checked_ptr("depth_to_points: rgb", rgb, dev, _u8, (h, w, 3)), h, w, float(fx), float(fy),
                     checked_ptr("depth_to_points: points", points, dev, _f64, (h * w, 3)),
                     checked_ptr("depth_to_points: colors", colors, dev, _f64, (h * w, 3)))

    def mask_down1(self, depth, out, B, H, W, OH, OW, w):
        self._launch(abi.lib.vdn_mask_down1, depth.data_ptr(), out.data_ptr(), B, H, W, OH, OW, w.data_ptr())

    def mask_down2(self, x, out, B, H, W, OH, OW, w):
        self._launch(abi.lib.vdn_mask_down2, x.data_ptr(), out.data_ptr(), B, H, W, OH, OW, w.data_ptr())

    def dwconv7(self, x, y, B, H, W, Cn, w, bias):
        self._launch(abi.lib.vdn_dwconv7, x.data_ptr(), y.data_ptr(), B, H, W, Cn, w.data_ptr(), bias.data_ptr())

    def addtab_cast(self, x, tab, tab_div: int, tab_mod: int, y, rows: int, Cn: int):
        yh, yl = _hl(y)
        self._launch(abi.lib.vdn_addtab_cast, self.dt, x.data_ptr(), self._p(tab), tab_div, tab_mod, yh.data_ptr(), yl, rows, Cn)

    def pack_x8(self, t: HL, hi_kt: torch.Tensor, planes8: torch.Tensor, order: int = 0):
        rows, ld = t.hi.shape
        self._launch(abi.lib.vdn_pack_x8, t.hi.data_ptr(), t.lo.data_ptr(), rows, ld, hi_kt.data_ptr(), planes8.data_ptr(), 1, order)

    def pack_x8_relu_pad(self, x: HL, out: PadKT):
        assert x.lo is not None and tuple(x.hi.shape) == (out.B * out.H * out.W, out.C) and x.hi.dtype == torch.float16, x.hi.shape
        self._launch(abi.lib.vdn_pack_x8_relu_pad, x.hi.data_ptr(), x.lo.data_ptr(), out.B, out.H, out.W, out.C, out.hi.data_ptr(),
                     out.p8.data_ptr())

    def conv3x3_pad(self, a: PadKT, w, N: int, bias: torch.Tensor, *, out_pad: Optional[PadKT] = None, out: Optional[HL] = None,
                    res1: Optional[HL] = None, res2: Optional[HL] = None, tag: Optional[str] = None):
        kw = dict(a8=a.p8, w8=w.p8, a_kt=True, w_kt=True, bias=bias, pad=a, tag=tag)
        if out is None:
            assert out_pad is not None and res1 is None and res2 is None and (out_pad.B, out_pad.H, out_pad.W, out_pad.C) == (a.B, a.H, a.W, N)
            self.gemm(HL(a.hi), HL(w.hi), a.rows, N, 9 * a.C, out=HL(out_pad.hi.view(-1, N)), out8=out_pad.p8, out_kt=True, act=abi.ACT_RELU, **kw)
            return out_pad
        assert res1 is not None and tuple(out.hi.shape) == (a.B * a.H * a.W, N)
        assert out_pad is None or (out_pad.B, out_pad.H, out_pad.W, out_pad.C) == (a.B, a.H, a.W, N)
        self.gemm(HL(a.hi), HL(w.hi), a.rows, N, 9 * a.C, out=out, res1=res1, res2=res2, pad_out=out_pad, **kw)
        return out

    def pack_x8_f32(self, x: torch.Tensor, hi_kt: torch.Tensor, planes8: torch.Tensor):
        rows, ld = x.shape
        self._launch(abi.lib.vdn_pack_x8_f32, x.data_ptr(), rows, ld, hi_kt.data_ptr(), planes8.data_ptr())

    def cast(self, x, y):
        self._launch(abi.lib.vdn_cast, x.data_ptr(), _TDT[x.dtype], y.data_ptr(), _TDT[y.dtype], x.numel())
```

Measured before the change: 294.6 frames/s.

## Route DPT head projections and memory output through x8 packed GEMM path

Encoder tap layernorms and the memory-bank output layernorm now write KT/x8-packed operands directly, so the head's 1x1 projections and pix-feature projection can run on the x8 GEMM path instead of the x3 split path. A new RCU2U epilogue lets the last fusion conv emit a packed unpadded output for the low-res oc1 GEMM (opt-in via env), and an F32-store x8 epilogue is added. Layernorm is extended to support kt/x8 output with out_group row dropping. The aim is to cut the extra GEMM terms and separate packing passes in the head, at the cost of more epilogue variants and relying on x8 precision holding up.

```diff
diff --git a/include/vdn.h b/include/vdn.h
--- a/include/vdn.h
+++ b/include/vdn.h
@@ -91,6 +91,8 @@
   int32_t subpix;
   const float* subpix_bias;
   void* pad_hi;
+  void* u_hi;
+  void* u8;
 } vdn_gemm_desc;
 
 int vdn_gemm(const vdn_gemm_desc* d, vdn_stream stream);
diff --git a/video-depth-normal-v2_amd/csrc/gemm.hip b/video-depth-normal-v2_amd/csrc/gemm.hip
--- a/video-depth-normal-v2_amd/csrc/gemm.hip
+++ b/video-depth-normal-v2_amd/csrc/gemm.hip
@@ -79,12 +79,13 @@
         (d.N & 63) || !d.out || ((uintptr_t)d.out & 15) || ((uintptr_t)d.bias & 15))
       return VDN_EINVAL;
     if (d.act == VDN_ACT_RELU) {
-      if (!d.out_kt || !d.out8 || d.out_lo || d.res1 || d.res2 || d.pad_hi) return VDN_EINVAL;
+      if (!d.out_kt || !d.out8 || d.out_lo || d.res1 || d.res2 || d.pad_hi || d.u_hi || d.u8) return VDN_EINVAL;
     } else if (d.act == VDN_ACT_NONE) {
       if (d.out_kt || !d.out_lo || !d.res1 || !d.res1_lo || d.res1_dt != VDN_F16 || (d.ldr1 & 7) || ((uintptr_t)d.res1 | (uintptr_t)d.res1_lo) & 15)
         return VDN_EINVAL;
       if (d.res2 && (!d.res2_lo || d.res2_dt != VDN_F16 || (d.ldr2 & 7) || ((uintptr_t)d.res2 | (uintptr_t)d.res2_lo) & 15)) return VDN_EINVAL;
       if ((d.pad_hi == nullptr) != (d.out8 == nullptr) || ((uintptr_t)d.pad_hi & 15)) return VDN_EINVAL;
+      if ((d.u_hi == nullptr) != (d.u8 == nullptr) || (d.u_hi && d.pad_hi) || (((uintptr_t)d.u_hi | (uintptr_t)d.u8) & 15)) return VDN_EINVAL;
     } else {
       return VDN_EINVAL;
     }
@@ -107,7 +108,7 @@
   if (d.x8_terms < 0 || d.x8_terms > 2) return VDN_EINVAL;
   if (d.out_kt && (d.store != VDN_ST_PLAIN || d.out_dt != VDN_F16 || d.ldc != d.N || (d.N & 63) || d.res1 || d.res2 || d.tab ||
                    d.rowadd || d.gamma || d.row_group > 0 || (d.act == VDN_ACT_RELU && d.a_mode != VDN_A_PAD3X3))) return VDN_EINVAL;
-  if (d.pad_hi && d.a_mode != VDN_A_PAD3X3) return VDN_EINVAL;
+  if ((d.pad_hi || d.u_hi || d.u8) && d.a_mode != VDN_A_PAD3X3) return VDN_EINVAL;
   if (((uintptr_t)d.bias | (uintptr_t)d.gamma | (uintptr_t)d.tab | (uintptr_t)d.res1 | (uintptr_t)d.res2) & 7) return VDN_EALIGN;
   switch (d.store) {
     case VDN_ST_PLAIN:
diff --git a/video-depth-normal-v2_amd/csrc/gemm_kernels.hpp b/video-depth-normal-v2_amd/csrc/gemm_kernels.hpp
--- a/video-depth-normal-v2_amd/csrc/gemm_kernels.hpp
+++ b/video-depth-normal-v2_amd/csrc/gemm_kernels.hpp
@@ -108,7 +108,9 @@
 
 constexpr int VDN_STX_FC1 = 100, VDN_STX_RES = 101, VDN_STX_HEADS = 102, VDN_STX_HALF = 103, VDN_STX_RESHALF1 = 104,
               VDN_STX_RESHALF2 = 105, VDN_STX_SPLITK = 106, VDN_STX_SUBPIX = 107,
-              VDN_STX_RCU1 = 108, VDN_STX_RCU2 = 109;
+              VDN_STX_RCU1 = 108, VDN_STX_RCU2 = 109,
+              VDN_STX_RCU2U = 111,
+              VDN_STX_F32 = 110;
 
 __device__ __forceinline__ void subpix_taps(int phase, int ck, unsigned& taps, int& lg) {
   const int a = phase / ck, b = phase - a * ck;
@@ -150,6 +152,9 @@
       if (!d.dst[i] || (!d.dst_lo[i] && !d.transposed[i] && !d.dst8[i])) return d.store;
     return VDN_STX_HEADS;
   }
+  if (d.store == VDN_ST_PLAIN && d.act == VDN_ACT_NONE && !d.gamma && !d.tab && !d.res1 && !d.res2 && d.out_dt == VDN_F32 &&
+      !d.out_lo && d.row_group <= 0)
+    return VDN_STX_F32;
   return d.store;
 }
 
@@ -492,6 +497,7 @@
     case VDN_STX_RESHALF2: epilogue_regs<DT, TM, TN, VDN_STX_RESHALF2>(acc, p, mw, nw, lane); break;
     case VDN_STX_RES: epilogue_regs<DT, TM, TN, VDN_STX_RES>(acc, p, mw, nw, lane); break;
     case VDN_STX_FC1:
+    case VDN_STX_F32:
     case VDN_ST_PLAIN: epilogue_regs<DT, TM, TN, VDN_ST_PLAIN>(acc, p, mw, nw, lane); break;
     case VDN_ST_CONVT: epilogue_regs<DT, TM, TN, VDN_ST_CONVT>(acc, p, mw, nw, lane); break;
     case VDN_ST_GEGLU: epilogue_regs<DT, TM, TN, VDN_ST_GEGLU>(acc, p, mw, nw, lane); break;
@@ -1145,6 +1151,7 @@
   const bool a8 = !(d.N & 7) && !(d.ldc & 7) && !((uintptr_t)d.out & 15) && !((uintptr_t)d.out_lo & 15) && !(d.ldr1 & 7) &&
                   !(d.ldr2 & 7) && !(((uintptr_t)d.res1 | (uintptr_t)d.res1_lo | (uintptr_t)d.res2 | (uintptr_t)d.res2_lo) & 15);
   if (!a8 && fl != VDN_STX_RES && fl != VDN_STX_HEADS && fl != VDN_STX_SUBPIX) fl = d.store;
+  if (fl == VDN_STX_F32) fl = d.store;
   if (d.a_mode == VDN_A_CONV3X3) {
     if (fl != VDN_STX_HALF && fl != VDN_STX_RESHALF1 && fl != VDN_STX_RESHALF2 && fl != VDN_STX_SUBPIX) fl = VDN_ST_PLAIN;
   } else if (fl == VDN_STX_RESHALF1 || fl == VDN_STX_RESHALF2) {
@@ -1229,7 +1236,7 @@
   if constexpr (DT == VDN_F16) {
     if (d.A8 && d.W8) {
       if ((d.a_mode == VDN_A_PLAIN || d.a_mode == VDN_A_PAD3X3) && !d.relu_a && !(d.K & 63) && d.N >= 192 &&
-          (long)d.M * d.N >= 1024L * 1024 && tuning(d).x8 != 0)
+          ((long)d.M * d.N >= 1024L * 1024 || tuning(d).x8 == 2) && tuning(d).x8 != 0)
         return x8_entry(d, s);
       if (d.a_mode == VDN_A_PAD3X3) return VDN_EUNSUPPORTED;
       if (d.a_kt || d.w_kt || d.out_kt || d.out8 || !d.A_lo || !d.W_lo) return VDN_EUNSUPPORTED;
diff --git a/video-depth-normal-v2_amd/csrc/gemm_x8.hip b/video-depth-normal-v2_amd/csrc/gemm_x8.hip
--- a/video-depth-normal-v2_amd/csrc/gemm_x8.hip
+++ b/video-depth-normal-v2_amd/csrc/gemm_x8.hip
@@ -269,7 +269,7 @@
           const int n = nw + 32 * j + 16 * u + 8 * h + 4 * q;
           bias8[j][u][q] = (p.bias && n < p.N) ? *(const f32x4*)(p.bias + n) : z4;
         }
-    if constexpr (STORE == VDN_STX_RCU1 || STORE == VDN_STX_RCU2) {
+    if constexpr (STORE == VDN_STX_RCU1 || STORE == VDN_STX_RCU2 || STORE == VDN_STX_RCU2U) {
 #pragma unroll
       for (int i = 0; i < NI; ++i)
 #pragma unroll
@@ -384,11 +384,28 @@
               split_planes(v, hh, ll);
               const int n = nw + 32 * j + 16 * u + 8 * h;
               if (img && n < p.N) store_out_planes<false, T>(p, mu * p.ldc + n, hh, ll);
-              hh = relu8(hh); ll = relu8(ll);
+              if constexpr (STORE == VDN_STX_RCU2) { hh = relu8(hh); ll = relu8(ll); }
 #pragma unroll
               for (int e = 0; e < 8; ++e) { hv[16 * j + 8 * u + e] = hh[e]; lv[16 * j + 8 * u + e] = ll[e]; }
             }
-          if (p.out8 && m < p.M && nw < p.N) store_pad((_Float16*)p.pad_hi, m, img, hv, lv);
+          if constexpr (STORE == VDN_STX_RCU2U) {
+            if (img && nw < p.N) {
+              const int mr = p.cB * p.cH * p.cW;
+#pragma unroll
+              for (int q = 0; q < 4; ++q) {
+                V8 o;
+#pragma unroll
+                for (int e = 0; e < 8; ++e) o[e] = hv[8 * q + e];
+                *(V8*)((_Float16*)p.u_hi + kt_half_offset(1, mu, nw + 32 * (q >> 1) + 16 * (q & 1) + 8 * h, mr, p.ldc)) = o;
+              }
+              const int sb = x6_scale_byte(hv);
+              uint8_t* d8 = (uint8_t*)p.u8 + kt_byte_offset(1, mu, nw, h, mr, p.ldc);
+              x6_store_half(d8, hv, sb);
+              x6_store_half(d8 + (size_t)mr * p.ldc, lv, sb - 10);
+            }
+          } else {
+            if (p.out8 && m < p.M && nw < p.N) store_pad((_Float16*)p.pad_hi, m, img, hv, lv);
+          }
         }
       }
     } else if (STORE == VDN_STX_FC1 && p.out8) {
@@ -556,6 +573,35 @@
           const int n = nw + 32 * j + 8 * g + 4 * h;
           const f32x4 a = {acc[i][j][4 * g], acc[i][j][4 * g + 1], acc[i][j][4 * g + 2], acc[i][j][4 * g + 3]};
           if (m < p.M && n < p.N) *(f32x4*)((float*)p.out + (size_t)m * p.ldc + n) = (a + bias4[j][g]) * gam4[j][g] + res[i & 1][j][g];
+        }
+    }
+  } else if constexpr (STORE == VDN_STX_F32) {
+    f32x4 bias4[2][4];
+#pragma unroll
+    for (int j = 0; j < 2; ++j)
+#pragma unroll
+      for (int g = 0; g < 4; ++g) {
+        const int n = nw + 32 * j + 8 * g + 4 * h;
+        bias4[j][g] = (p.bias && n < p.N) ? *(const f32x4*)(p.bias + n) : z4;
+      }
+    const bool radd = p.rowadd != nullptr;
+    float ra[NI];
+#pragma unroll
+    for (int i = 0; i < NI; ++i) {
+      const int m = mw + 32 * i + r;
+      ra[i] = (radd && m < p.M) ? p.rowadd[m] : 0.f;
+    }
+#pragma unroll
+    for (int i = 0; i < NI; ++i) {
+      const int m = mw + 32 * i + r;
+#pragma unroll
+      for (int j = 0; j < 2; ++j)
+#pragma unroll
+        for (int g = 0; g < 4; ++g) {
+          const int n = nw + 32 * j + 8 * g + 4 * h;
+          f32x4 a = f32x4{acc[i][j][4 * g], acc[i][j][4 * g + 1], acc[i][j][4 * g + 2], acc[i][j][4 * g + 3]} + bias4[j][g];
+          if (radd) a += ra[i];
+          if (m < p.M && n < p.N) *(f32x4*)((float*)p.out + (size_t)m * p.ldc + n) = a;
         }
     }
   } else {
@@ -606,6 +652,7 @@
     hipLaunchKernelGGL((gemm_x8_kernel<ST, true, BM, true>), g, b, LDS, s, d);                                           \
   } while (0)
     if (d.act == VDN_ACT_RELU) VDN_X8T(VDN_STX_RCU1);
+    else if (d.u_hi) VDN_X8T(VDN_STX_RCU2U);
     else VDN_X8T(VDN_STX_RCU2);
 #undef VDN_X8T
     VDN_CHECK_LAUNCH();
@@ -621,6 +668,7 @@
     case VDN_STX_HALF: VDN_X8(VDN_STX_HALF, true); break;
     case VDN_STX_HEADS: VDN_X8(VDN_STX_HEADS, true); break;
     case VDN_STX_RES: VDN_X8(VDN_STX_RES, false); break;
+    case VDN_STX_F32: VDN_X8(VDN_STX_F32, false); break;
     case VDN_ST_GEGLU: VDN_X8(VDN_ST_GEGLU, false); break;
     case VDN_ST_HEADS: {
       bool pair = a8 && d.nsplit >= 1 && d.rope_cs && !((uintptr_t)d.rope_cs & 15);
diff --git a/video-depth-normal-v2_amd/csrc/norm.hip b/video-depth-normal-v2_amd/csrc/norm.hip
--- a/video-depth-normal-v2_amd/csrc/norm.hip
+++ b/video-depth-normal-v2_amd/csrc/norm.hip
@@ -23,6 +23,7 @@
   extern __shared__ __attribute__((aligned(16))) _Float16 stage_all[];
   _Float16* const stage = stage_all + (X6 ? (threadIdx.x >> 6) * 2 * NV * 256 : 0);
   int row = blockIdx.x * 4 + (threadIdx.x >> 6);
+  const int orows = out_group > 0 ? rows - (rows + out_group - 1) / out_group : rows;
   f32x4 wv[NV], bv[NV];
 #pragma unroll
   for (int i = 0; i < NV; ++i) {
@@ -78,7 +79,7 @@
           if (out_f) *(f32x4*)(out_f + orow * C + c) = y;
           if (out_h) {
             typename Half<DT>::V4 hv, lv;
-            const size_t oh = kt_half_offset(kt, orow, c, rows, C);
+            const size_t oh = kt_half_offset(kt, orow, c, orows, C);
             if (out_l || out8) {
 #pragma unroll
               for (int e = 0; e < 4; e += 2) {
@@ -121,7 +122,7 @@
                 for (int e = 0; e < 8; ++e) xv[8 * q + e] = a[e];
               }
             } else xv = hv;
-            uint8_t* d8 = out8 + (size_t)plane * rows * C + kt_byte_offset(kt, orow, (hb >> 1) * 64, hb & 1, rows, C);
+            uint8_t* d8 = out8 + (size_t)plane * orows * C + kt_byte_offset(kt, orow, (hb >> 1) * 64, hb & 1, orows, C);
             x6_store_half(d8, xv, plane ? sb - 10 : sb);
           }
           asm volatile("s_waitcnt lgkmcnt(0)" ::: "memory");
@@ -340,7 +341,7 @@
   if ((C & 3) || C > 2048) return VDN_EALIGN;
   if (addtab && (tab_div <= 0 || tab_mod <= 0)) return VDN_EINVAL;
   if (out_h && h_dt != VDN_F16 && h_dt != VDN_BF16) return VDN_EUNSUPPORTED;
-  if ((out8 || kt) && (!out_h || h_dt != VDN_F16 || out_group > 0 || (C & 63) || ((uintptr_t)out8 & 15))) return VDN_EINVAL;
+  if ((out8 || kt) && (!out_h || h_dt != VDN_F16 || (C & 63) || ((uintptr_t)out8 & 15))) return VDN_EINVAL;
   hipStream_t s = (hipStream_t)stream;
   if (!addtab) { tab_div = 1; tab_mod = 1; }
   switch (x_dt) {
diff --git a/video-depth-normal-v2_amd/vdn/_abi.py b/video-depth-normal-v2_amd/vdn/_abi.py
--- a/video-depth-normal-v2_amd/vdn/_abi.py
+++ b/video-depth-normal-v2_amd/vdn/_abi.py
@@ -41,7 +41,7 @@
         ("a_kt", i32), ("w_kt", i32), ("out_kt", i32), ("x8_terms", i32),
         ("tuning", vp),
         ("subpix", i32), ("subpix_bias", fp),
-        ("pad_hi", vp),
+        ("pad_hi", vp), ("u_hi", vp), ("u8", vp),
     ]
 
 
diff --git a/video-depth-normal-v2_amd/vdn/depth_anything_v2.py b/video-depth-normal-v2_amd/vdn/depth_anything_v2.py
--- a/video-depth-normal-v2_amd/vdn/depth_anything_v2.py
+++ b/video-depth-normal-v2_amd/vdn/depth_anything_v2.py
@@ -157,8 +157,11 @@
     def _forward_lane(self, ln, x, _pre_relu, out):
         rt, enc, mem, head = ln["rt"], ln["enc"], ln["mem"], ln["head"]
         B = x.shape[0]
-        taps, last_f32, (ph, pw) = enc.run(x, want_f32_last=True)
-        fm = mem.forward(last_f32, B, ph * pw)
+        hx = head.tap_x8(B * (x.shape[2] // 14) * (x.shape[3] // 14))
+        if getattr(enc, "readout", None) is not None:
+            hx = [False] * 4
+        taps, last_f32, (ph, pw) = enc.run(x, want_f32_last=True, tap_x8=hx)
+        fm = mem.forward(last_f32, B, ph * pw, out_x8=hx[3])
         t3 = fm
         if getattr(enc, "readout", None) is not None:
             t3 = enc.readout.apply(3, fm, enc.cls_last, B, ph * pw, rt.hbuf("ro_fm", (B * ph * pw, enc.C)))
diff --git a/video-depth-normal-v2_amd/vdn/engine.py b/video-depth-normal-v2_amd/vdn/engine.py
--- a/video-depth-normal-v2_amd/vdn/engine.py
+++ b/video-depth-normal-v2_amd/vdn/engine.py
@@ -8,7 +8,7 @@
 
 from . import _abi as abi
 from . import pack
-from .runtime import HL, Runtime, ceil_to
+from .runtime import HL, KT, Runtime, ceil_to
 
 GELU, RELU = abi.ACT_GELU, abi.ACT_RELU
 PATCH = 14
@@ -73,7 +73,7 @@
             self._pos_cache[key] = (table, (self.cls + table[0]).contiguous())
         return self._pos_cache[key]
 
-    def run(self, x: torch.Tensor, want_f32_last: bool = False, tap_out=None):
+    def run(self, x: torch.Tensor, want_f32_last: bool = False, tap_out=None, tap_x8=(False,) * 4):
         rt, C, Hh = self.rt, self.C, self.heads
         Bf, _, H, W = x.shape
         assert H % PATCH == 0 and W % PATCH == 0, "input sides must be multiples of 14 (patch_embed.py:73-74)"
@@ -100,6 +100,7 @@
         if probe is not None:
             probe(-1, tok)
         use8 = self.x8 and rt.x8_rows(M) and q8 is not None and rt.pv_products != 3
+        tap8 = [bool(t) and self.x8 and tap_out is None and readout is None and rt.x8_rows(Bf * P) for t in tap_x8]
         hn, att, f1 = rt.operand("enc_ln", (M, C), use8), rt.operand("enc_att", (M, C), use8), rt.operand("enc_fc1", (M, Hd), use8)
         for i, b in enumerate(self.blocks):
             xt = self.x8_terms[i]
@@ -117,10 +118,12 @@
                 probe(i, tok)
             if i in self.taps:
                 j = self.taps.index(i)
-                t = tap_out[j] if tap_out is not None else rt.hbuf(f"tap{j}", (Bf * P, C))
+                t = tap_out[j] if tap_out is not None else rt.operand(f"tap{j}", (Bf * P, C), tap8[j])
                 f = None
                 if want_f32_last and j == len(self.taps) - 1:
                     f = last_f32 = rt.fbuf("tap_last_f32", (Bf * P, C))
+                    if tap8[j]:
+                        t = None
                 if readout is None:
                     rt.layernorm(tok, M, C, self.nw, self.nb, 1e-6, out_h=t, out_f=f, out_group=N)
                 else:
@@ -270,7 +273,11 @@
     def __init__(self, rt: Runtime, mod, in_ch: int, features: int, out_channels, temporal: bool):
         self.rt, self.C, self.F, self.oc = rt, in_ch, features, list(out_channels)
         h = rt.prec
-        self.proj = [(pack.conv1x1(p.weight, h), pack.f32(p.bias)) for p in mod.projects]
+        self.head_x8 = [rt.x8_capable(in_ch) and o >= 1024 and o % 8 == 0 and not os.environ.get("VDN_HEAD_X3") for o in self.oc]
+        self.head_path = {}
+        self.oc1_x8 = False
+        self.proj = [(pack.Linear(pack.conv1x1(p.weight, h), pack.ORDER_NATURAL if x8 else None), pack.f32(p.bias))
+                     for p, x8 in zip(mod.projects, self.head_x8)]
         self.rt0 = pack.conv_transpose(mod.resize_layers[0].weight, mod.resize_layers[0].bias, h)
         self.rt1 = pack.conv_transpose(mod.resize_layers[1].weight, mod.resize_layers[1].bias, h)
         self.rs3 = (pack.conv3x3(mod.resize_layers[3].weight, h), pack.f32(mod.resize_layers[3].bias))
@@ -311,6 +318,8 @@
         if fused and (features // 2) % 16 == 0 and not os.environ.get("VDN_OC1_HIRES"):
             f1 = s.refinenet1.out_conv
             self.oc1_low = pack.lowres_oc1(s.output_conv1.weight, f1.weight, f1.bias, h)
+            self.oc1_x8 = self.rcu_x8 and os.environ.get("VDN_OC1_X8") == "1" and not os.environ.get("VDN_HEAD_X3")
+            self.oc1_low = (pack.Linear(self.oc1_low[0], pack.ORDER_GEMM if self.oc1_x8 else None), self.oc1_low[1])
         self.rn_low = [None, None]
         if not os.environ.get("VDN_RN_HIRES"):
             for i, k in enumerate((4, 2)):
@@ -324,6 +333,9 @@
             chans = [self.oc[2], self.oc[3], features, features]
             self.temporal = [TemporalEngine(rt, mod.motion_modules[i], chans[i], i) for i in range(4)]
 
+    def tap_x8(self, rows: int) -> list:
+        return [x8 and self.rt.x8_rows(rows) for x8 in self.head_x8]
+
     def _conv3(self, x, w, Bf, H, W, Cin, Cout, name, *, stride=1, bias=None, relu_a=False, act=0, res1=None, res2=None,
                f32_out=False):
         OH, OW = (H + 2 - 3) // stride + 1, (W + 2 - 3) // stride + 1
@@ -337,7 +349,7 @@
         t = self._conv3(x, r["w1"], Bf, H, W, F, F, "rcu_t", bias=r["b1"], relu_a=True, act=RELU)
         return self._conv3(t, r["w2"], Bf, H, W, F, F, name, bias=r["b2"], res1=x, res2=extra)
 
-    def _fusion(self, i, Bf, size_in, size_out, prev, skip=None):
+    def _fusion(self, i, Bf, size_in, size_out, prev, skip=None, u_x8=False):
         rt, F = self.rt, self.F
         H, W = size_in
         f = self.ref[i]
@@ -353,7 +365,10 @@
                 x = rt.conv3x3_pad(pb, r["x2"], F, r["b2"], out=rt.hbuf(f"ff{i}_s", (M, F)), res1=skip, res2=prev, out_pad=pa)
             r = f["r2"]
             rt.conv3x3_pad(pa, r["x1"], F, r["b1"], out_pad=pb)
-            u = rt.conv3x3_pad(pb, r["x2"], F, r["b2"], out=rt.hbuf(f"ff{i}_u", (M, F)), res1=x)
+            ukt = rt.operand(f"ff{i}_u", (M, F), True) if u_x8 and size_out is None else None
+            u = rt.conv3x3_pad(pb, r["x2"], F, r["b2"], out=rt.hbuf(f"ff{i}_u", (M, F)), res1=x, out_u=ukt)
+            if ukt is not None:
+                return ukt
         else:
             self.rcu_path[i] = "x3"
             if skip is not None:
@@ -375,6 +390,7 @@
         P = ph * pw
         pr = []
         for i in range(4):
+            self.head_path[f"proj{i}"] = "x8" if isinstance(taps[i], KT) else "x3"
             o = rt.hbuf(f"proj{i}", (Bf * P, oc[i]))
             rt.gemm(taps[i], self.proj[i][0], Bf * P, oc[i], C, bias=self.proj[i][1], out=o)
             pr.append(o)
@@ -423,7 +439,8 @@
         sy, sx = (s0[0] - 1) / max(H - 1, 1), (s0[1] - 1) / max(W - 1, 1)
         fused = self.oc2_taps is not None and int(17 * sy) + 3 <= 13 and int(17 * sx) + 3 <= 13
         if fused and self.oc1_low is not None and rt.lowres_oc1_rows(Bf * s0[0] * s0[1]):
-            u = self._fusion(1, Bf, s1, None, p2, r1)
+            u = self._fusion(1, Bf, s1, None, p2, r1, u_x8=self.oc1_x8)
+            self.head_path["oc1_z"] = "x8" if isinstance(u, KT) else "x3"
             M1 = Bf * s1[0] * s1[1]
             z = rt.fbuf("oc1_z", (M1, 9 * (F // 2)))
             rt.gemm(u, self.oc1_low[0], M1, 9 * (F // 2), F, bias=self.oc1_low[1], out=z)
@@ -484,7 +501,9 @@
         self.md1 = flat(e0[0].weight, e0[0].bias, e0[1].weight, e0[1].bias, e0[3].weight, e0[3].bias)
         self.md2 = flat(e1[0].weight, e1[0].bias, e1[1].weight, e1[1].bias, e1[3].weight, e1[3].bias)
         assert self.md1.numel() == 53 and self.md2.numel() == 2598
-        self.wpix, self.bpix = pack.conv1x1(me.pix_feat_proj.weight, h), pack.f32(me.pix_feat_proj.bias)
+        self.wpix = lin(pack.conv1x1(me.pix_feat_proj.weight, h), None if os.environ.get("VDN_HEAD_X3") else NAT)
+        self.bpix = pack.f32(me.pix_feat_proj.bias)
+        self.out_path = None
         self.cx = []
         for b in me.fuser.layers:
             self.cx.append(dict(
@@ -541,7 +560,7 @@
         return ([k.narrow0(r0, nr) for k in ks], [v.narrow0(r0, nr) for v in vs],
                 [None if t is None else t.narrow(0, r0, nr) for t in k8], tp)
 
-    def forward(self, feat_f32: torch.Tensor, B: int, P: int) -> torch.Tensor:
+    def forward(self, feat_f32: torch.Tensor, B: int, P: int, out_x8: bool = False):
         rt, C, Hh = self.rt, self.C, self.heads
         assert self.state["shape"] == (B * self.lane[1], P), "MemoryEngine.prepare() not called for this batch"
         side = int(math.sqrt(P))
@@ -585,7 +604,9 @@
             rt.layernorm(x, M, C, L["n3w"], L["n3b"], 1e-5, out_h=n)
             rt.gemm(n, L["w1"], M, 2 * C, C, bias=L["b1"], act=GELU, out=h2)
             rt.gemm(h2, L["w2"], M, C, 2 * C, bias=L["b2"], res1=x, out=x)
-        out = rt.hbuf("mem_out", (M, C))
+        out8 = out_x8 and self.wpix.x8 is not None and rt.x8_rows(M)
+        self.out_path = "x8" if out8 else "x3"
+        out = rt.operand("mem_out", (M, C), out8)
         rt.layernorm(x, M, C, self.nw, self.nb, 1e-5, out_h=out)
         return out
 
diff --git a/video-depth-normal-v2_amd/vdn/runtime.py b/video-depth-normal-v2_amd/vdn/runtime.py
--- a/video-depth-normal-v2_amd/vdn/runtime.py
+++ b/video-depth-normal-v2_amd/vdn/runtime.py
@@ -214,7 +214,8 @@
              row_skip: int = 0, heads: Optional[dict] = None, convt: Optional[dict] = None, tag: Optional[str] = None,
              a8: Optional[torch.Tensor] = None, w8: Optional[torch.Tensor] = None, out8: Optional[torch.Tensor] = None,
              a_kt: bool = False, w_kt: bool = False, out_kt: bool = False, x8_terms: int = 0,
-             subpix_bias: Optional[torch.Tensor] = None, pad: Optional[PadKT] = None, pad_out: Optional[PadKT] = None):
+             subpix_bias: Optional[torch.Tensor] = None, pad: Optional[PadKT] = None, pad_out: Optional[PadKT] = None,
+             u_out: Optional[KT] = None):
         if isinstance(W, Linear):
             if not isinstance(A, KT):
                 W, x8_terms = W.hl, 0
@@ -292,6 +293,8 @@
             d.out8 = out8.data_ptr()
         if pad_out is not None:
             d.pad_hi, d.out8 = pad_out.hi.data_ptr(), pad_out.p8.data_ptr()
+        if u_out is not None:
+            d.u_hi, d.u8 = u_out.hi.data_ptr(), u_out.p8.data_ptr()
         d.a_kt, d.w_kt, d.out_kt = int(a_kt), int(w_kt), int(out_kt)
         d.x8_terms = int(x8_terms)
         if subpix_bias is not None:
@@ -755,7 +758,7 @@
                      out.p8.data_ptr())
 
     def conv3x3_pad(self, a: PadKT, w, N: int, bias: torch.Tensor, *, out_pad: Optional[PadKT] = None, out: Optional[HL] = None,
-                    res1: Optional[HL] = None, res2: Optional[HL] = None, tag: Optional[str] = None):
+                    res1: Optional[HL] = None, res2: Optional[HL] = None, tag: Optional[str] = None, out_u: Optional[KT] = None):
         kw = dict(a8=a.p8, w8=w.p8, a_kt=True, w_kt=True, bias=bias, pad=a, tag=tag)
         if out is None:
             assert out_pad is not None and res1 is None and res2 is None and (out_pad.B, out_pad.H, out_pad.W, out_pad.C) == (a.B, a.H, a.W, N)
@@ -763,7 +766,8 @@
             return out_pad
         assert res1 is not None and tuple(out.hi.shape) == (a.B * a.H * a.W, N)
         assert out_pad is None or (out_pad.B, out_pad.H, out_pad.W, out_pad.C) == (a.B, a.H, a.W, N)
-        self.gemm(HL(a.hi), HL(w.hi), a.rows, N, 9 * a.C, out=out, res1=res1, res2=res2, pad_out=out_pad, **kw)
+        assert out_u is None or (out_pad is None and tuple(out_u.hi.shape) == tuple(out.hi.shape) and tuple(out_u.p8.shape) == (2, *out.hi.shape))
+        self.gemm(HL(a.hi), HL(w.hi), a.rows, N, 9 * a.C, out=out, res1=res1, res2=res2, pad_out=out_pad, u_out=out_u, **kw)
         return out
 
     def pack_x8_f32(self, x: torch.Tensor, hi_kt: torch.Tensor, planes8: torch.Tensor):
```

Result: no change. 295.9 frames/s, median of 6 (+0.5%).
